# nihaomiao/WACV23_TSNet

Hardware: AMD Instinct MI355X
Metric: retargeted frames/sec at bs=4, 256x256, n_source=3; max-abs delta vs ref (higher is better)
Workload: dtype f32 (convolutions: fp16 x 2 split of the scaled fp32 operands, 3 exact MFMA products, two-level fp32 accumulate; fp32-class accuracy); 1 GPU; TSNet(label_nc=2,n_blocks=0,n_downsampling=3,n_source=3) forward, fp32, B=4 per GPU, 256x256 (BASELINE.json configs[1]); global_batch=4, parallelism=replicas x1 (batch-sharded, weights broadcast once)

## Files before the change

include/tsnet_abi.h:

```cpp
#ifndef TSNET_ABI_H
#define TSNET_ABI_H

#include <stddef.h>
#include <stdint.h>

#ifdef __cplusplus
extern "C" {
#endif

#define TSNET_ABI_VERSION 5
#define TSNET_MAX_SOURCES 8

enum {
    TSNET_OK = 0,
    TSNET_ERR_ARG = -1,
    TSNET_ERR_WEIGHT = -2,
    TSNET_ERR_HIP = -3,
    TSNET_ERR_NOMEM = -4
};

typedef struct tsnet_engine* tsnet_handle;

typedef struct tsnet_cfg {
    int label_nc;
    int n_blocks;
    int n_downsampling;
    int n_source;
    int ngf;
    int enc_blocks;
    int addcoords;
    int pose_composite;
    float pose_mean[3];
    int height, width;
    int max_batch;
    int operand_mode;
} tsnet_cfg;

int tsnet_abi_version(void);
int tsnet_create(const tsnet_cfg* cfg, tsnet_handle* out);
int tsnet_load_weights(tsnet_handle h, const char* name, const float* data, const int64_t* shape, int rank);
int tsnet_finalize(tsnet_handle h, void* stream);
void tsnet_destroy(tsnet_handle h);
const char* tsnet_last_error(tsnet_handle h);

int tsnet_num_params(tsnet_handle h);
int tsnet_param_info(tsnet_handle h, int index, const char** name, int64_t shape_out[4], int* rank);

int tsnet_packed_weights(tsnet_handle h, void** dev_ptr, size_t* bytes);

int tsnet_forward(tsnet_handle h,
                  const float* const* src_img, const float* const* src_lbl, const float* const* src_bbox,
                  const float* tar_lbl, const float* tar_bbox,
                  float* out_rgb, float* out_flow, int B, void* stream);

int tsnet_set_source_divisors(tsnet_handle h, const float* div, int n);

int tsnet_set_sources(tsnet_handle h, const float* const* src_img, const float* const* src_lbl,
                      const float* const* src_bbox, int B, void* stream);
int tsnet_forward_target(tsnet_handle h, const float* tar_lbl, const float* tar_bbox,
                         float* out_rgb, float* out_flow, int B, void* stream);

int tsnet_train_extras(tsnet_handle h, const float* const* src_img, const float* tar_img, int B,
                       float* warp_src_img, float* losses, void* stream);

int tsnet_stage_ptr(tsnet_handle h, const char* name, const float** dev_ptr, size_t* count);

double tsnet_forward_macs(tsnet_handle h, int B);

#define TSNET_TIMING_CLASSES 9
enum { TSNET_T_CONV = 0, TSNET_T_STATS = 1, TSNET_T_ELEMWISE = 2, TSNET_T_FLOW = 3, TSNET_T_WARP = 4,
       TSNET_T_PACK = 5, TSNET_T_UPSAMPLE = 6, TSNET_T_OTHER = 7,
       TSNET_T_CONV_RES = 8  };
int tsnet_timing_enable(tsnet_handle h, int on);
int tsnet_timing_read(tsnet_handle h, double ms_out[TSNET_TIMING_CLASSES], int64_t launches_out[TSNET_TIMING_CLASSES], int reset);

int tsnet_op_conv2d(const float* x, int N, int H, int W, int Cin,
                    const float* w_oihw, const float* bias, int Cout, int ksize, int stride, int pad, int pad_mode,
                    const float* in_alpha, const float* in_beta, int in_relu, float bound, int nprod, int kernel, int tile,
                    float* y, void* stream);
int tsnet_op_conv2d_cat(const float* x, const float* x2, int N, int H, int W, int C1, int C2, int x2_nmod,
                        const float* w_oihw, const float* bias, int Cout, int ksize, int stride, int pad, int pad_mode,
                        float bound, int nprod, float* y, void* stream);
int tsnet_op_head(const float* x, int N, int H, int W, int C, const float* in_alpha, const float* in_beta,
                  const float* w_oihw, const float* bias, int composite, const float* bg, float* y, void* stream);
int tsnet_op_instnorm_stats(const float* x, int N, int HW, int C, float* alpha, float* beta, void* stream);
int tsnet_op_norm_act(const float* x, const float* alpha, const float* beta, int relu, const float* resid,
                      int N, int HW, int C, float* y, void* stream);
int tsnet_op_upsample2x(const float* x, const float* alpha, const float* beta, int relu,
                        int N, int H, int W, int C, float* y, void* stream);
int tsnet_op_flow(const float* tar_fea, const float* src_fea, const float* tar_bbox, const float* src_bbox,
                  int B, int h, int w, int C, int H, int W, float* flow, void* stream);
int tsnet_op_flow_k(const float* tar_fea, const float* src_fea, const float* tar_bbox, const float* src_bbox,
                    int B, int K, int h, int w, int C, int H, int W, float* flow, int variant, int repeat, float* ms_out, void* stream);
int tsnet_flow_plan(int B, int h, int w, int C);
int tsnet_op_warp(const float* src_fea, const float* flow, int B, int h, int w, int C, float* out, void* stream);
int tsnet_op_warp_k(const float* src_fea, const float* flow, int B, int K, int h, int w, int C, float* out, int repeat, float* ms_out, void* stream);
const char* tsnet_op_last_error(void);

int tsnet_frame_stats(const float* x, int B, int C, int HW, float div, float* mean, float* std_unbiased, void* stream);
int tsnet_demo_postprocess(const float* rec, int B, int H, int W, const float* gen_mean, const float* gen_std,
                           const float* ref_mean, const float* ref_std, const float* img_mean_over_255,
                           unsigned char* out_rgb, void* stream);

int tsnet_fit_face_curves(const double* keypoints, int F, double* curves);
int tsnet_raster_face(const double* keypoints, const double* curves, int F, int h, int w, int bw, unsigned char* edges, unsigned char* bbox, void* stream);
int tsnet_vl2ch(const float* labels, int B, int HW, int num_classes, float* out, void* stream);

int tsnet_resize_label(const unsigned char* in, int F, int h, int w, int OH, int OW, const double* wts_rows, int lw_rows,
                       const double* wts_cols, int lw_cols, float* out, void* stream);
int tsnet_fit_pose_curves(const double* pts, int F, int flags, double* curves);
int tsnet_raster_pose(const double* pts, const double* curves, int F, int h, int w, int win_x0, int win_y0, int win_x1, int win_y1, int flags,
                      unsigned char* labels, void* stream);
int tsnet_label_bbox(const unsigned char* labels, int F, int h, int w, unsigned char* bbox, void* stream);
int tsnet_resize_pad(const unsigned char* in, int F, int h, int w, const int* ytab, const int* xtab, int oh, int ow,
                     int pad_top, int pad_left, int OH, int OW, int binarise, float* out, void* stream);

int tsnet_bench_conv(int N, int H, int W, int Cin, int Cout, int ksize, int stride, int pad, int pad_mode, int norm,
                     int variant, int iters, float* ms_out, void* stream);

void tsnet_debug_counters(int64_t out[4], int reset);

void tsnet_linspace(int n, float* out);
void tsnet_coord_table(int H, int W, float* out);

int tsnet_bicubic_taps(int n_in, int n_out);
int tsnet_bicubic_table(int n_in, int n_out, int* first, int* count, int* coef);
int tsnet_prepare_frames(const unsigned char* frames, int F, int h, int w, int x0, int y0, int x1, int y1,
                         const int* xfirst, const int* xcount, const int* xcoef, int xtaps,
                         const int* yfirst, const int* ycount, const int* ycoef, int ytaps,
                         int oh, int ow, int pad_top, int pad_left, int OH, int OW, const float* mean_bgr, float* out, void* stream);

#ifdef __cplusplus
}
#endif
#endif
```

wacv23_tsnet_amd/_lib.py:

```python
from __future__ import annotations

import ctypes as C
import os

import torch

_HERE = os.path.dirname(os.path.abspath(__file__))
LIB_PATH = os.path.join(_HERE, "lib", "libtsnet_hip.so")
MAX_SOURCES = 8
TIMING_CLASSES = 9
TIMING_NAMES = ("conv", "stats", "elementwise", "flow", "warp", "pack", "upsample", "other", "conv_res")

ABI_SYMBOLS = (
    "tsnet_abi_version", "tsnet_create", "tsnet_load_weights", "tsnet_finalize", "tsnet_destroy",
    "tsnet_last_error", "tsnet_num_params", "tsnet_param_info", "tsnet_packed_weights",
    "tsnet_forward", "tsnet_set_source_divisors", "tsnet_set_sources", "tsnet_forward_target", "tsnet_train_extras", "tsnet_stage_ptr",
    "tsnet_forward_macs", "tsnet_timing_enable", "tsnet_timing_read",
    "tsnet_op_conv2d", "tsnet_op_conv2d_cat", "tsnet_op_head", "tsnet_op_instnorm_stats", "tsnet_op_norm_act", "tsnet_op_upsample2x",
    "tsnet_op_flow", "tsnet_op_flow_k", "tsnet_flow_plan", "tsnet_op_warp", "tsnet_op_warp_k", "tsnet_op_last_error", "tsnet_frame_stats", "tsnet_demo_postprocess", "tsnet_fit_face_curves", "tsnet_raster_face", "tsnet_vl2ch", "tsnet_fit_pose_curves", "tsnet_raster_pose", "tsnet_label_bbox", "tsnet_resize_pad", "tsnet_resize_label", "tsnet_bench_conv", "tsnet_debug_counters", "tsnet_linspace", "tsnet_coord_table",
    "tsnet_bicubic_taps", "tsnet_bicubic_table", "tsnet_prepare_frames",
)


class TsnetCfg(C.Structure):
    _fields_ = [
        ("label_nc", C.c_int), ("n_blocks", C.c_int), ("n_downsampling", C.c_int), ("n_source", C.c_int),
        ("ngf", C.c_int), ("enc_blocks", C.c_int), ("addcoords", C.c_int), ("pose_composite", C.c_int),
        ("pose_mean", C.c_float * 3), ("height", C.c_int), ("width", C.c_int), ("max_batch", C.c_int), ("operand_mode", C.c_int),
    ]


_fp = C.POINTER(C.c_float)
_vp = C.c_void_p


def bind(lib: C.CDLL) -> C.CDLL:
    lib.tsnet_abi_version.restype = C.c_int
    lib.tsnet_create.argtypes = [C.POINTER(TsnetCfg), C.POINTER(_vp)]
    lib.tsnet_load_weights.argtypes = [_vp, C.c_char_p, _vp, C.POINTER(C.c_int64), C.c_int]
    lib.tsnet_finalize.argtypes = [_vp, _vp]
    lib.tsnet_destroy.argtypes = [_vp]
    lib.tsnet_destroy.restype = None
    lib.tsnet_last_error.argtypes = [_vp]
    lib.tsnet_last_error.restype = C.c_char_p
    lib.tsnet_num_params.argtypes = [_vp]
    lib.tsnet_param_info.argtypes = [_vp, C.c_int, C.POINTER(C.c_char_p), C.POINTER(C.c_int64), C.POINTER(C.c_int)]
    lib.tsnet_packed_weights.argtypes = [_vp, C.POINTER(_vp), C.POINTER(C.c_size_t)]
    pp = C.POINTER(_vp)
    lib.tsnet_forward.argtypes = [_vp, pp, pp, pp, _vp, _vp, _vp, _vp, C.c_int, _vp]
    lib.tsnet_set_source_divisors.argtypes = [_vp, _fp, C.c_int]
    lib.tsnet_set_sources.argtypes = [_vp, pp, pp, pp, C.c_int, _vp]
    lib.tsnet_forward_target.argtypes = [_vp, _vp, _vp, _vp, _vp, C.c_int, _vp]
    lib.tsnet_train_extras.argtypes = [_vp, pp, _vp, C.c_int, _vp, _vp, _vp]
    lib.tsnet_stage_ptr.argtypes = [_vp, C.c_char_p, C.POINTER(_vp), C.POINTER(C.c_size_t)]
    lib.tsnet_forward_macs.argtypes = [_vp, C.c_int]
    lib.tsnet_forward_macs.restype = C.c_double
    lib.tsnet_timing_enable.argtypes = [_vp, C.c_int]
    lib.tsnet_timing_read.argtypes = [_vp, C.POINTER(C.c_double), C.POINTER(C.c_int64), C.c_int]
    lib.tsnet_op_conv2d.argtypes = [_vp, C.c_int, C.c_int, C.c_int, C.c_int, _vp, _vp, C.c_int, C.c_int, C.c_int,
                                    C.c_int, C.c_int, _vp, _vp, C.c_int, C.c_float, C.c_int, C.c_int, C.c_int, _vp, _vp]
    lib.tsnet_op_conv2d_cat.argtypes = [_vp, _vp] + [C.c_int] * 6 + [_vp, _vp] + [C.c_int] * 5 + [C.c_float, C.c_int, _vp, _vp]
    lib.tsnet_op_head.argtypes = [_vp, C.c_int, C.c_int, C.c_int, C.c_int, _vp, _vp, _vp, _vp, C.c_int, _fp, _vp, _vp]
    lib.tsnet_op_instnorm_stats.argtypes = [_vp, C.c_int, C.c_int, C.c_int, _vp, _vp, _vp]
    lib.tsnet_op_norm_act.argtypes = [_vp, _vp, _vp, C.c_int, _vp, C.c_int, C.c_int, C.c_int, _vp, _vp]
    lib.tsnet_op_upsample2x.argtypes = [_vp, _vp, _vp, C.c_int, C.c_int, C.c_int, C.c_int, C.c_int, _vp, _vp]
    lib.tsnet_resize_label.argtypes = [_vp, C.c_int, C.c_int, C.c_int, C.c_int, C.c_int, _vp, C.c_int, _vp, C.c_int, _vp, _vp]
    lib.tsnet_op_flow.argtypes = [_vp, _vp, _vp, _vp, C.c_int, C.c_int, C.c_int, C.c_int, C.c_int, C.c_int, _vp, _vp]
    lib.tsnet_op_flow_k.argtypes = [_vp, _vp, _vp, _vp] + [C.c_int] * 7 + [_vp, C.c_int, C.c_int, _fp, _vp]
    lib.tsnet_flow_plan.argtypes = [C.c_int] * 4
    lib.tsnet_op_warp.argtypes = [_vp, _vp, C.c_int, C.c_int, C.c_int, C.c_int, _vp, _vp]
    if hasattr(lib, "tsnet_op_warp_k"):
        lib.tsnet_op_warp_k.argtypes = [_vp, _vp] + [C.c_int] * 5 + [_vp, C.c_int, _fp, _vp]
    lib.tsnet_op_last_error.restype = C.c_char_p
    lib.tsnet_frame_stats.argtypes = [_vp, C.c_int, C.c_int, C.c_int, C.c_float, _vp, _vp, _vp]
    lib.tsnet_demo_postprocess.argtypes = [_vp, C.c_int, C.c_int, C.c_int, _vp, _vp, _vp, _vp, _fp, _vp, _vp]
    lib.tsnet_fit_face_curves.argtypes = [_vp, C.c_int, _vp]
    lib.tsnet_fit_pose_curves.argtypes = [_vp, C.c_int, C.c_int, _vp]
    lib.tsnet_raster_face.argtypes = [_vp, _vp, C.c_int, C.c_int, C.c_int, C.c_int, _vp, _vp, _vp]
    lib.tsnet_vl2ch.argtypes = [_vp, C.c_int, C.c_int, C.c_int, _vp, _vp]
    lib.tsnet_raster_pose.argtypes = [_vp, _vp] + [C.c_int] * 8 + [_vp, _vp]
    lib.tsnet_label_bbox.argtypes = [_vp, C.c_int, C.c_int, C.c_int, _vp, _vp]
    lib.tsnet_resize_pad.argtypes = [_vp, C.c_int, C.c_int, C.c_int, _vp, _vp] + [C.c_int] * 7 + [_vp, _vp]
    lib.tsnet_bench_conv.argtypes = [C.c_int] * 12 + [_fp, _vp]
    lib.tsnet_debug_counters.argtypes = [C.POINTER(C.c_int64), C.c_int]
    lib.tsnet_debug_counters.restype = None
    lib.tsnet_linspace.argtypes = [C.c_int, _fp]
    lib.tsnet_linspace.restype = None
    lib.tsnet_coord_table.argtypes = [C.c_int, C.c_int, _fp]
    lib.tsnet_coord_table.restype = None
    if hasattr(lib, "tsnet_prepare_frames"):
        lib.tsnet_bicubic_taps.argtypes = [C.c_int, C.c_int]
        lib.tsnet_bicubic_table.argtypes = [C.c_int, C.c_int, _vp, _vp, _vp]
        lib.tsnet_prepare_frames.argtypes = [_vp] + [C.c_int] * 7 + [_vp, _vp, _vp, C.c_int, _vp, _vp, _vp, C.c_int] + [C.c_int] * 6 + [_fp, _vp, _vp]
    return lib


_cached = None


def load_tools() -> C.CDLL:
    from . import build as _b
    if not os.path.exists(_b.OUT_TOOLS):
        raise RuntimeError(f"{_b.OUT_TOOLS} is missing: run `python -m wacv23_tsnet_amd.build --tools`")
    return bind(C.CDLL(_b.OUT_TOOLS))


def load() -> C.CDLL:
    global _cached
    if _cached is not None:
        return _cached
    if not os.path.exists(LIB_PATH):
        raise RuntimeError(
            f"{LIB_PATH} is missing: the HIP extension is not built. Run "
            "`python -c 'import __graft_entry__ as g; g.build()'` (needs hipcc). "
            "There is no CPU fallback for the TS-Net forward path.")
    try:
        _cached = bind(C.CDLL(LIB_PATH))
    except OSError as e:
        raise RuntimeError(f"failed to load {LIB_PATH}: {e}") from e
    if _cached.tsnet_abi_version() != 5:
        raise RuntimeError("libtsnet_hip.so ABI version mismatch; rebuild")
    return _cached
```

wacv23_tsnet_amd/csrc/conv_common.hpp:

```cpp
#pragma once
#include <hip/hip_runtime.h>

namespace tsnet {

typedef float f32x16 __attribute__((ext_vector_type(16)));
struct alignas(16) F4 { float v[4]; };

constexpr unsigned kOOB = 0x80000000u;
constexpr int kPatchCols = 32;
constexpr int kPatchRows = 4;

#ifndef TSNET_BUF_LOAD16
typedef __amdgpu_buffer_rsrc_t tsnet_brsrc_t;
__device__ __forceinline__ tsnet_brsrc_t tsnet_make_brsrc(const void* p, unsigned bytes) {
    return __builtin_amdgcn_make_buffer_rsrc(const_cast<void*>(p), 0, (int)bytes, 0x00020000);
}
#define TSNET_BUF_LOAD16(rsrc, voff, soff) __builtin_bit_cast(F4, __builtin_amdgcn_raw_buffer_load_b128((rsrc), (int)(voff), (int)(soff), 0))
#endif
#ifndef TSNET_BUF_LOAD8
struct alignas(8) F2 { float v[2]; };
#define TSNET_BUF_LOAD8(rsrc, voff, soff) __builtin_bit_cast(F2, __builtin_amdgcn_raw_buffer_load_b64((rsrc), (int)(voff), (int)(soff), 0))
#endif
#ifndef TSNET_UNIFORM
#define TSNET_UNIFORM(x) __builtin_amdgcn_readfirstlane(x)
// ... 42 lines not shown
        "v_fma_mixhi_f16 %2, %5, %8, -%0 op_sel:[0,0,1] op_sel_hi:[0,0,1]\n\t"                                     \
        "v_fma_mixhi_f16 %3, %7, %8, -%1 op_sel:[0,0,1] op_sel_hi:[0,0,1]"                                          \
        : "=&v"(h0), "=&v"(h1), "=&v"(l0), "=&v"(l1)                                                               \
        : "v"(a0), "v"(b0), "v"(a1), "v"(b1), "v"(s))
#endif
#ifndef TSNET_FAST_EXP
#define TSNET_FAST_EXP(x) __expf(x)
#endif
#ifndef TSNET_SETPRIO
#define TSNET_SETPRIO(n) __builtin_amdgcn_s_setprio(n)
#endif
#ifndef TSNET_OPAQUE_V
#define TSNET_OPAQUE_V(x) asm volatile("" : "+v"(x))
#endif

__device__ __forceinline__ int xcd_item(int bid, int nitems) {
    const int q = nitems >> 3, r = nitems & 7, xcd = bid & 7, loc = bid >> 3;
    return (xcd < r ? xcd * (q + 1) : r * (q + 1) + (xcd - r) * q) + loc;
}

__device__ __forceinline__ void tile_of_block(int bid, int tiles_m, int tiles_n, int gn, int& tile_m, int& tile_n) {
    if (gn > 0) {
        const int xcd = bid & 7, loc = bid >> 3;
        const int tn = tiles_n / gn, tm = tiles_m / (8 / gn);
        tile_m = (xcd / gn) * tm + loc / tn;
        tile_n = (xcd % gn) * tn + loc % tn;
    } else {
        const int item = xcd_item(bid, tiles_m * tiles_n);
        tile_m = item / tiles_n;
        tile_n = item - tile_m * tiles_n;
    }
}

__device__ __forceinline__ unsigned short bf16_rne(float f) {
    const unsigned u = __builtin_bit_cast(unsigned, f);
    return (unsigned short)((u + 0x7FFFu + ((u >> 16) & 1u)) >> 16);
}
#ifndef TSNET_CVT_PK_BF16
__device__ __forceinline__ unsigned tsnet_cvt_pk_bf16(float a, float b) {
    unsigned r;
    asm("v_cvt_pk_bf16_f32 %0, %1, %2" : "=v"(r) : "v"(a), "v"(b));
    return r;
}
#define TSNET_CVT_PK_BF16(a, b) tsnet_cvt_pk_bf16((a), (b))
#endif

__device__ __forceinline__ void tsnet_publish_amax(unsigned* slot, float m) {
    __shared__ float wave_max[16];
#pragma unroll
    for (int off = 32; off > 0; off >>= 1) { const float o = __shfl_xor(m, off); m = o > m ? o : m; }
    __syncthreads();
    if ((threadIdx.x & 63) == 0) wave_max[threadIdx.x >> 6] = m;
    __syncthreads();
    if (threadIdx.x == 0) {
        const int nw = (int)((blockDim.x + 63) >> 6);
        for (int i = 1; i < nw; ++i) m = wave_max[i] > m ? wave_max[i] : m;
        __hip_atomic_fetch_max(slot, __builtin_bit_cast(unsigned, m), __ATOMIC_RELAXED, __HIP_MEMORY_SCOPE_AGENT);
    }
}

struct ConvArgs {
    const float* x;
    const float* x2;
    const float* in_alpha;
    const float* in_beta;
    int in_relu;
    float in_scale, in_unscale;
    const unsigned* in_amax; float in_bound_add;
    const unsigned short* w;
    const float* w_unscale;
    const float* bias;
    float* y;
    double* stat_part;
    const float* addend; int add_nmod;
    int N, H, W, Cin, cin_log2, Csplit, x2_nmod;
    int Ho, Wo, Cout, Npad;
    int stride, pad, reflect, taps, nchunks, M;
    int tiles_m, tiles_n, tpi;
    int xcd_gn;
    float* fin_alpha; float* fin_beta; int* fin_counter; int fin_S; float fin_eps;
    unsigned* amax_out;
    int x_bf16, y_bf16;
    int w1_chunk, w1_tab2;
};

__device__ __forceinline__ void bf16x8_widen(const F4& p, F4 (&o)[2]) {
#pragma unroll
    for (int e = 0; e < 4; ++e) {
        const unsigned w = __builtin_bit_cast(unsigned, p.v[e]);
        o[e >> 1].v[(e & 1) * 2] = __builtin_bit_cast(float, w << 16);
        o[e >> 1].v[(e & 1) * 2 + 1] = __builtin_bit_cast(float, w & 0xFFFF0000u);
    }
}

__device__ __forceinline__ void load_x_octet(const tsnet_brsrc_t& rs, bool xb16, unsigned voff, unsigned soff, F4 (&o)[2]) {
    if (xb16) {
        const F4 p = TSNET_BUF_LOAD16(rs, voff >> 1, soff >> 1);
        bf16x8_widen(p, o);
    } else {
        o[0] = TSNET_BUF_LOAD16(rs, voff, soff);
        o[1] = TSNET_BUF_LOAD16(rs, voff, soff + 16u);
    }
}

__device__ __forceinline__ void h2_device_scale(const unsigned* amax, float add, float& scale, float& unscale) {
    const float bound = __builtin_bit_cast(float, __hip_atomic_load(amax, __ATOMIC_RELAXED, __HIP_MEMORY_SCOPE_AGENT)) + add;
    int e = 0;
    (void)frexpf(bound, &e);
    int sa = 15 - e;
    sa = sa > 24 ? 24 : (sa < -24 ? -24 : sa);
    scale = ldexpf(1.0f, sa);
    unscale = ldexpf(1.0f, -sa);
}

__device__ __forceinline__ void split_h2(float v, unsigned& hi, unsigned& lo) {
    const _Float16 h = (_Float16)v;
    const _Float16 l = (_Float16)(v - (float)h);
    hi = (unsigned)__builtin_bit_cast(unsigned short, h);
    lo = (unsigned)__builtin_bit_cast(unsigned short, l);
}

__device__ __forceinline__ void split_h2_octet(const F4& x0, const F4& x1, F4& H, F4& L) {
    unsigned hw[4], lw[4];
    TSNET_SPLIT_2PAIRS(x0.v[0], x0.v[1], x0.v[2], x0.v[3], hw[0], lw[0], hw[1], lw[1]);
    TSNET_SPLIT_2PAIRS(x1.v[0], x1.v[1], x1.v[2], x1.v[3], hw[2], lw[2], hw[3], lw[3]);
#pragma unroll
    for (int e = 0; e < 4; ++e) { H.v[e] = __builtin_bit_cast(float, hw[e]); L.v[e] = __builtin_bit_cast(float, lw[e]); }
}

__device__ __forceinline__ void bf16_octet(const F4& x0, const F4& x1, F4& H) {
    unsigned hw[4];
#pragma unroll
    for (int e = 0; e < 2; ++e) {
        hw[e] = TSNET_CVT_PK_BF16(x0.v[2 * e], x0.v[2 * e + 1]);
        hw[2 + e] = TSNET_CVT_PK_BF16(x1.v[2 * e], x1.v[2 * e + 1]);
    }
#pragma unroll
    for (int e = 0; e < 4; ++e) H.v[e] = __builtin_bit_cast(float, hw[e]);
}

template <bool AFFINE, bool KEEP = true>
__device__ __forceinline__ void transform_octet(const F4 (&sx)[2], const float* ta, int Cin, float in_scale, float relu_floor, float keep, F4 (&t)[2]) {
    if (AFFINE) {
#pragma unroll
        for (int q = 0; q < 2; ++q) {
            const F4 al = *reinterpret_cast<const F4*>(ta + q * 4), be = *reinterpret_cast<const F4*>(ta + Cin + q * 4);
#pragma unroll
            for (int e = 0; e < 4; ++e) {
                const float v = __builtin_fmaxf(__builtin_fmaf(sx[q].v[e], al.v[e], be.v[e]), relu_floor);
                t[q].v[e] = KEEP ? v * keep : v;
            }
        }
    } else {
#pragma unroll
        for (int q = 0; q < 2; ++q)
#pragma unroll
            for (int e = 0; e < 4; ++e) t[q].v[e] = __builtin_fmaxf(sx[q].v[e] * in_scale, relu_floor);
    }
}

template <int BN, int WARPS_M, int WARPS_N, int MT, int NTL, int STAT_WAVE = 0, typename MOf>
__device__ __forceinline__ void conv_epilogue(const ConvArgs& a, f32x16 (&tot)[MT][NTL], unsigned char* smem_raw, int tid, int wave, int n0,
                                              size_t stat_tile, MOf m_of, const bool active = true) {
    constexpr int WM = MT * 32, WN = NTL * 32;
    const int lane = tid & 63, li = lane & 31, lh = lane >> 5;
    const int wm0 = (wave / WARPS_N) * WM, wn0 = (wave % WARPS_N) * WN;
    const int hw = a.Ho * a.Wo;
    double csum[NTL], csq[NTL];
#pragma unroll
    for (int j = 0; j < NTL; ++j) { csum[j] = 0.0; csq[j] = 0.0; }
    float vmax = 0.f;
#pragma unroll
    for (int i = 0; i < MT; ++i) {
#pragma unroll
        for (int j = 0; j < NTL; ++j) {
            const int n = n0 + wn0 + j * 32 + li;
            const bool nok = n < a.Cout;
            const float bv = (a.bias && nok) ? a.bias[n] : 0.f;
#pragma unroll
            for (int r = 0; r < 16; ++r) {
                const int m = m_of(wm0 + i * 32 + (r & 3) + 8 * (r >> 2) + 4 * lh);
                const bool mok = active && m >= 0;
                float v = tot[i][j][r] + bv;
                if (a.addend && nok && mok) {
                    const int img = m / hw;
                    v += a.addend[((size_t)(img % a.add_nmod) * hw + (m - img * hw)) * a.Cout + n];
                }
                tot[i][j][r] = v;
                if (a.stat_part && mok) { csum[j] += (double)v; csq[j] += (double)v * (double)v; }
                if (nok && mok) vmax = __builtin_fmaxf(vmax, __builtin_fabsf(v));
            }
        }
    }
    if (a.amax_out) tsnet_publish_amax(a.amax_out + stat_tile / (size_t)a.tpi, vmax);
    if (a.stat_part) {
        __syncthreads();
        double* red = reinterpret_cast<double*>(smem_raw);
#pragma unroll
        for (int j = 0; j < NTL; ++j) {
            const double s2 = csum[j] + __shfl_xor(csum[j], 32);
            const double q2 = csq[j] + __shfl_xor(csq[j], 32);
            if (lh == 0 && active) {
                double* o = red + ((size_t)(wave / WARPS_N) * BN + wn0 + j * 32 + li) * 2;
                o[0] = s2; o[1] = q2;
            }
        }
        __syncthreads();
        const int stid = tid - 64 * STAT_WAVE;
        if (stid >= 0 && stid < BN && n0 + stid < a.Cout) {
            double s = 0.0, q = 0.0;
#pragma unroll
            for (int wmi = 0; wmi < WARPS_M; ++wmi) { s += red[((size_t)wmi * BN + stid) * 2]; q += red[((size_t)wmi * BN + stid) * 2 + 1]; }
            double* o = a.stat_part + (stat_tile * a.Cout + n0 + stid) * 2;
            if (a.fin_counter) {
                __hip_atomic_store(o, s, __ATOMIC_RELAXED, __HIP_MEMORY_SCOPE_AGENT);
                __hip_atomic_store(o + 1, q, __ATOMIC_RELAXED, __HIP_MEMORY_SCOPE_AGENT);
            } else {
                o[0] = s; o[1] = q;
            }
        }
        if (a.fin_counter) {
            const int S = a.fin_S;
            const int img = (int)(stat_tile / (size_t)S);
            const int ntn = (a.Npad + 31) / 32;
            int* counter = a.fin_counter + (size_t)img * ntn + n0 / 32;
            const bool mine = stid >= 0 && stid < BN && n0 + stid < a.Cout;
            auto fold = [&](const double* p0, int cnt, size_t step, double& sm, double& sq) __attribute__((always_inline)) {
                double gs[4] = {0, 0, 0, 0}, gq[4] = {0, 0, 0, 0};
                for (int t0 = 0; t0 < cnt; t0 += 8) {
                    double v[8], w[8];
#pragma unroll
                    for (int u = 0; u < 8; ++u) {
                        const double* p = p0 + (size_t)(t0 + u < cnt ? t0 + u : cnt - 1) * step;
                        v[u] = __hip_atomic_load(p, __ATOMIC_RELAXED, __HIP_MEMORY_SCOPE_AGENT);
                        w[u] = __hip_atomic_load(p + 1, __ATOMIC_RELAXED, __HIP_MEMORY_SCOPE_AGENT);
                    }
#pragma unroll
                    for (int u = 0; u < 8; ++u) {
                        const bool in = t0 + u < cnt;
                        gs[u & 3] += in ? v[u] : 0.0;
                        gq[u & 3] += in ? w[u] : 0.0;
                    }
                }
                sm = gs[0]; sq = gq[0];
#pragma unroll
                for (int k = 1; k < 4; ++k) { sm += gs[k]; sq += gq[k]; }
            };
            auto write_ab = [&](double sm, double sq) __attribute__((always_inline)) {
                const double mean = sm / hw;
                double var = sq / hw - mean * mean;
                if (var < 0) var = 0;
                const float al = 1.0f / sqrtf((float)var + a.fin_eps);
                a.fin_alpha[(size_t)img * a.Cout + n0 + stid] = al;
                a.fin_beta[(size_t)img * a.Cout + n0 + stid] = -((float)mean) * al;
            };
            auto finalize = [&]() __attribute__((always_inline)) {
                if (mine) {
                    double sm, sq;
                    fold(a.stat_part + (((size_t)img * S) * a.Cout + n0 + stid) * 2, S, (size_t)a.Cout * 2, sm, sq);
                    write_ab(sm, sq);
                }
                if (stid == 0) __hip_atomic_store(counter, 0, __ATOMIC_RELAXED, __HIP_MEMORY_SCOPE_AGENT);
            };
            if (BN <= 64) {
                if (stid >= 0 && stid < 64) {
                    auto arrive = [&](int* c) __attribute__((always_inline)) {
                        TSNET_DRAIN_VMEM();
                        float arrived = 0.f;
                        if (lane == 0) arrived = (float)__hip_atomic_fetch_add(c, 1, __ATOMIC_RELAXED, __HIP_MEMORY_SCOPE_AGENT);
#pragma unroll
                        for (int off = 32; off > 0; off >>= 1) arrived += __shfl_xor(arrived, off);
                        return (int)arrived;
                    };
                    if (arrive(counter) == S - 1) finalize();
                }
            } else {
                int* flag = reinterpret_cast<int*>(smem_raw + 8192);
                auto arrive = [&](int* c) __attribute__((always_inline)) {
                    TSNET_DRAIN_VMEM();
                    __syncthreads();
                    if (stid == 0) *flag = __hip_atomic_fetch_add(c, 1, __ATOMIC_RELAXED, __HIP_MEMORY_SCOPE_AGENT);
                    __syncthreads();
                    return *flag;
                };
                if (arrive(counter) == S - 1) finalize();
            }
        }
    }
    unsigned short* const y16 = reinterpret_cast<unsigned short*>(a.y);
#pragma unroll
    for (int i = 0; i < MT; ++i) {
#pragma unroll
        for (int j = 0; j < NTL; ++j) {
            const int n = n0 + wn0 + j * 32 + li;
            if (n >= a.Cout) continue;
#pragma unroll
            for (int r = 0; r < 16; ++r) {
                const int m = m_of(wm0 + i * 32 + (r & 3) + 8 * (r >> 2) + 4 * lh);
                if (!(active && m >= 0)) continue;
                if (a.y_bf16) y16[(size_t)m * a.Cout + n] = bf16_rne(tot[i][j][r]);
                else a.y[(size_t)m * a.Cout + n] = tot[i][j][r];
            }
        }
    }
}

}
```

wacv23_tsnet_amd/csrc/conv_plan.hpp:

```cpp
#pragma once
#include <cstddef>
#include <stdexcept>
#include <string>

namespace tsnet {

constexpr int kPlanTileRows = 4, kPlanTileCols = 32;
constexpr size_t kFinCounterInts = 65536;
constexpr int kFinMaxTiles = 32;

enum class ConvFamily { H2R, G64, H2, H2S, H2S32, H2D, W1 };
enum class ConvKernel { Own = 0, General = 1, Patch = 2 };
enum class ConvSched { Plain = 0, Deep = 1, TwoGroups = 2 };

struct ConvShape {
    int ks = 1, stride = 1, pad = 0, reflect = 0;
    int cin = 0;
    int cout = 0, npad = 0, kpad = 0;
    int form = 0;
    int N = 0, H = 0, W = 0;
    int csplit = 0;
    bool transform = false;
    int nprod = 3;
    bool fin_counter = false;
    int ho() const { return (H + 2 * pad - ks) / stride + 1; }
    int wo() const { return (W + 2 * pad - ks) / stride + 1; }
};

struct ConvRequest {
    ConvKernel kernel = ConvKernel::Own;
    int rows = 0;
    int width = 0;
    bool alt = false;
    ConvSched sched = ConvSched::Plain;
    int chunk = 0;
    int chunk_cap = 3;
    int abl = 0, opt = 0;
    int xcd_gn = -1;
};

struct ConvPlan {
    ConvFamily family = ConvFamily::H2R;
    int rows = 0;
    int width = 0;
    bool side_by_side = false;
    ConvSched sched = ConvSched::Plain;
    int w1_chunk = 1, w1_tab2 = 0;
    int xcd_gn = 0;
    int tpi = 0, tiles_m = 0, tiles_n = 0;
    bool fin = false;
};

inline ConvRequest decode_tile_code(int kernel, int tile) {
    ConvRequest r;
    if (kernel == 3) {
        if (tile < 0 || tile > 3) throw std::invalid_argument("conv: the Winograd form takes 0 to 3 tiles per workgroup");
        r.chunk = tile;
        return r;
    }
    if (kernel < 0 || kernel > 2) throw std::invalid_argument("conv: kernel must be 0 (the layer's own), 1 (general), 2 (patch) or 3 (Winograd form)");
    r.kernel = static_cast<ConvKernel>(kernel);
    switch (tile) {
        case 0: break;
        case 32: case 64: case 128: r.width = tile; break;
        case 2128: r.rows = 2; r.width = 128; break;
        case 3064: case 3128: r.alt = true; r.width = tile - 3000; break;
        case 12128: r.rows = 2; r.width = 128; r.sched = ConvSched::Deep; break;
        case 20032: case 20064: r.rows = 4; r.width = tile - 20000; r.sched = ConvSched::TwoGroups; break;
        default: throw std::invalid_argument("conv: unknown tile code " + std::to_string(tile));
    }
    return r;
}

struct BenchVariant { ConvRequest req; int nprod = 3, form = 0; bool cold = false; };
inline BenchVariant decode_bench_variant(int variant) {
    const int v = variant < 0 ? 0 : variant;
    BenchVariant b;
    b.form = (v & 32768) ? 1 : 0;
    b.req = decode_tile_code(b.form ? 3 : ((v & 4096) ? 1 : ((v & 16384) ? 2 : 0)), v & 4095);
    b.nprod = (v & 8192) ? 1 : 3;
    b.cold = (v & (1 << 21)) != 0;
    b.req.abl = (v >> 16) & 31;
    b.req.opt = ((v >> 24) & 15) | ((v & (1 << 23)) ? 16 : 0) | ((v & (1 << 22)) ? 32 : 0);
    const int gx = (v >> 28) & 7;
    if (gx > 5) throw std::invalid_argument("bench_conv: XCD grid code 0 to 5");
    b.req.xcd_gn = gx == 0 ? -1 : (gx == 1 ? 0 : 1 << (gx - 2));
    return b;
}

struct HeadRequest { bool composite = false; int rows = 0; };
inline HeadRequest decode_head_code(int code) {
    if (code < 0 || (code & 0xFE)) throw std::invalid_argument("head: composite is bit 0, the tile rows bits 8 and up");
    HeadRequest r;
    r.composite = code & 1;
    r.rows = code >> 8;
    if (r.rows != 0 && r.rows != 8 && r.rows != 16 && r.rows != 32) throw std::invalid_argument("head: tile rows 8, 16 or 32");
    return r;
}

inline size_t w1_lds_bytes_host(int Cin, int tables) {
    return 3 * (size_t)(2 * (4 * 2 * 2 * (96 * 16 + 64) + 32)) + (size_t)tables * 2 * ((Cin + 31) / 32 * 32) * 4;
}
inline bool w1_eligible(int ks, int stride, int pad, int cin, int H, int W) {
    return ks == 3 && stride == 1 && pad == 1 && cin >= 16 && (cin & 15) == 0 && H >= 4 && W >= 32 && H % kPlanTileRows == 0 && W % kPlanTileCols == 0 &&
           w1_lds_bytes_host(cin, 1) + 256 <= 160 * 1024;
}

inline ConvFamily conv_class(const ConvShape& s, int rows, bool eligible_only) {
    const int Ho = s.ho(), Wo = s.wo();
    const bool bf16 = s.nprod == 1;
    const bool s1 = s.ks == 3 && s.stride == 1 && s.pad == 1 && s.cin >= 16 && (s.cin & 15) == 0 && s.H >= 2 && s.W >= 2;
    if (s.csplit || Ho <= 0 || Wo <= 0 || Wo % kPlanTileCols) return ConvFamily::H2R;
    const bool s2 = s.ks == 3 && s.stride == 2 && s.pad == 1 && !s.reflect && s.cin >= (eligible_only ? 16 : 128) && (s.cin & 15) == 0 && s.H == 2 * Ho && s.W == 2 * Wo;
    if (rows == 2 && Ho % 2 == 0) {
        if (s1) return ConvFamily::H2;
        if (s2) return ConvFamily::H2D;
    }
    if (Ho % kPlanTileRows) return ConvFamily::H2R;
    if (s1) return ConvFamily::H2;
    if (s.ks == 7 && s.stride == 1 && s.pad == 3 && s.reflect && s.cin == 8 && !s.transform && s.H >= 4 && s.W >= 4) return ConvFamily::H2S;
    if (s.ks == 7 && s.stride == 1 && s.pad == 3 && s.reflect && s.cin == 32 && !s.transform && s.H >= 4 && s.W >= 4) return ConvFamily::H2S32;
    if (s2 && (eligible_only || !bf16)) return ConvFamily::H2D;
    return ConvFamily::H2R;
}

inline bool wide_pays(const ConvShape& s, long tm, double gain, int cus) {
    const double c64 = (double)((tm * ((s.cout + 63) / 64) + cus - 1) / cus) * 64.0;
    const double c128 = (double)((tm * ((s.cout + 127) / 128) + cus - 1) / cus) * 128.0 / gain;
    return s.npad % 128 == 0 && s.cout > 64 && c128 < c64;
}

inline int xcd_grid(const ConvShape& s, int requested, int tiles_m, int tiles_n, const char* who) {
    int gn = requested < 0 ? (((double)s.kpad * s.npad * 4 > 16e6) ? 4 : 0) : requested;
    if (gn && ((gn != 1 && gn != 2 && gn != 4 && gn != 8) || tiles_n % gn || tiles_m % (8 / gn))) {
        if (requested >= 0) throw std::invalid_argument(std::string(who) + ": the XCD grid does not divide the tile matrix");
        gn = 0;
    }
    return gn;
}

inline void plan_w1_chunk(const ConvShape& s, const ConvRequest& r, int cus, ConvPlan& p) {
    const int n = p.tiles_m * p.tiles_n, npp = ((s.cin >> 4) + 1) / 2;
    const int rows = p.xcd_gn ? p.tiles_m / (8 / p.xcd_gn) : (p.tiles_m % 8 ? 0 : p.tiles_m / 8);
    const bool tab2 = !s.transform || w1_lds_bytes_host(s.cin, 2) + 256 <= 160 * 1024;
    auto fits = [&](int cc) { return cc == 1 || (s.nprod != 1 && npp >= 4 && rows > 0 && rows % cc == 0 && (tab2 || p.tpi % cc == 0)); };
    int cc = 1;
    if (r.chunk) {
        if (!fits(r.chunk)) throw std::invalid_argument("conv(w1): this chunk size does not fit the layer");
        cc = r.chunk;
    } else {
        for (int t : {3, 2}) if (fits(t) && n % (cus * t) == 0) { cc = t; break; }
        if (cc > r.chunk_cap) cc = 1;
    }
    p.w1_chunk = cc; p.w1_tab2 = (s.transform && tab2 && cc > 1) ? 1 : 0;
}

inline ConvPlan plan_conv(const ConvShape& s, const ConvRequest& r, int cus) {
    const bool bf16 = s.nprod == 1;
    const int Ho = s.ho(), hw = Ho * s.wo();
    ConvPlan p;
    if (s.form == 1) {
        if (s.csplit || !w1_eligible(s.ks, s.stride, s.pad, s.cin, s.H, s.W))
            throw std::invalid_argument("conv(w1): the layer is packed in the Winograd form, which needs a single source and whole 4 x 32 tiles");
        if (s.nprod == 4) throw std::invalid_argument("conv(w1): 1 or 3 products");
        p.family = ConvFamily::W1;
    } else if (r.kernel == ConvKernel::General) {
        p.family = ConvFamily::H2R;
    } else {
        p.family = conv_class(s, r.rows == 2 ? 2 : kPlanTileRows, r.kernel == ConvKernel::Patch);
        if (r.kernel == ConvKernel::Patch && p.family == ConvFamily::H2R) throw std::invalid_argument("conv: this layer / frame size has no patch kernel");
    }
    auto set_tiles = [&](int rows_per_tile_m, int bn) {
        p.tpi = (hw + rows_per_tile_m - 1) / rows_per_tile_m;
        p.tiles_m = s.N * p.tpi; p.tiles_n = (s.cout + bn - 1) / bn;
        p.fin = s.fin_counter && p.tpi <= kFinMaxTiles && (size_t)s.N * ((s.npad + 31) / 32) <= kFinCounterInts;
    };
    switch (p.family) {
    case ConvFamily::W1:
        if (r.opt) throw std::invalid_argument("conv(w1): no experiment variants");
        p.rows = kPlanTileRows; p.width = 64;
        set_tiles(kPlanTileRows * kPlanTileCols, 64);
        p.xcd_gn = xcd_grid(s, r.xcd_gn, p.tiles_m, p.tiles_n, "conv(w1)");
        plan_w1_chunk(s, r, cus, p);
        break;
    case ConvFamily::H2: {
        int pr = r.rows ? r.rows : kPlanTileRows, bn = r.width;
        if (bn == 0) {
            const long tm = (long)s.N * (hw / 128);
            bn = wide_pays(s, tm, s.transform ? 1.03 : 1.10, cus) ? 128 : 64;
            if (bf16 && s.npad % 128 == 0 && s.cout > 64 && tm * ((s.cout + 127) / 128) >= cus) bn = 128;
        }
        p.side_by_side = r.alt || (!r.width && bf16 && pr == 4 && bn == 128);
        if (p.side_by_side && (!bf16 || bn != 128)) throw std::invalid_argument("conv(h2): the 1 x 4 wave grid is the bf16 4 x 128 tile's");
        if ((pr != 2 && pr != 4) || Ho % pr) throw std::invalid_argument("conv(h2): the output height must be a multiple of the tile's rows (2 or 4)");
        if (s.npad % bn) throw std::invalid_argument("conv(h2): the tile width must divide the padded output width");
        p.rows = pr; p.width = bn; p.sched = r.sched;
        set_tiles(pr * kPlanTileCols, bn);
        p.xcd_gn = xcd_grid(s, r.xcd_gn, p.tiles_m, p.tiles_n, "conv(h2)");
        break;
    }
    case ConvFamily::H2S:
    case ConvFamily::H2S32:
        p.rows = kPlanTileRows; p.width = 64;
        set_tiles(128, 64);
        break;
    case ConvFamily::H2D: {
        if (r.sched == ConvSched::TwoGroups) throw std::invalid_argument("conv(h2d): the stride-2 tiles have no two-K-group form (1xxxx: the deep schedule of the 2 x 128 tile)");
        if (r.alt) throw std::invalid_argument("conv(h2d): tiles have two or four output rows");
        int pr = r.rows ? r.rows : kPlanTileRows, bn = r.width;
        if (bn == 0) {
            bn = 64;
            if (s.npad % 128 == 0 && s.cout > 64 && Ho % 2 == 0) { pr = 2; bn = 128; }
        }
        if (s.npad % bn) throw std::invalid_argument("conv(h2d): the tile width must divide the padded output width");
        if (Ho % pr) throw std::invalid_argument("conv(h2d): the output height must be a multiple of the tile's rows");
        p.rows = pr; p.width = bn;
        set_tiles(pr * kPlanTileCols, bn);
        const bool deep = r.width ? r.sched == ConvSched::Deep : (pr == 2 && bn == 128 && s.nprod == 3 && (long)p.tiles_m * p.tiles_n <= 2L * cus);
        p.sched = deep ? ConvSched::Deep : ConvSched::Plain;
        break;
    }
    case ConvFamily::H2R:
    case ConvFamily::G64: {
        if (r.abl || r.opt) throw std::invalid_argument("conv: experiment variants exist for the 3x3 / stride-1 patch kernel only");
        if (r.rows || r.sched != ConvSched::Plain || r.width == 32) throw std::invalid_argument("conv(h2r): the tile width must be 64 or 128");
        const bool g64_ok = (s.ks == 1 || s.ks == 3) && (s.cin & 63) == 0 && (!s.csplit || (s.csplit & 63) == 0) && s.npad % 128 == 0 && s.cout > 64 &&
                            (s.nprod == 1 || s.nprod == 3);
        if (r.alt || (!r.width && g64_ok)) {
            if (!g64_ok) throw std::invalid_argument("conv(g64): needs a 1 x 1 / 3 x 3 layer, input channels in multiples of 64 and more than 64 output channels");
            p.family = ConvFamily::G64;
            p.rows = r.width ? r.width : 64; p.width = 128;
            set_tiles(p.rows, 128);
        } else {
            const long tm = (long)s.N * ((hw + 127) / 128);
            const int bn = r.width ? r.width : ((s.ks == 3 && s.cin >= 16 && wide_pays(s, tm, 1.15, cus)) ? 128 : 64);
            if (s.npad % bn) throw std::invalid_argument("conv(h2r): the tile width must divide the padded output width");
            p.family = ConvFamily::H2R;
            p.rows = 128; p.width = bn;
            set_tiles(128, bn);
        }
        break;
    }
    }
    return p;
}

inline int head_rows(int B, int tiles_x, int hh, int cus) {
    return (long)B * tiles_x * ((hh + 31) / 32) >= cus ? 32 : ((long)B * tiles_x * ((hh + 15) / 16) >= cus ? 16 : 8);
}

}
```

wacv23_tsnet_amd/csrc/conv_w1.hpp:

```cpp
#pragma once
#include <type_traits>

#include "conv_common.hpp"

namespace tsnet {

constexpr int kW1Prod = 6;
constexpr int kW1Waves = 8 + kW1Prod;
constexpr int kW1Reg = 96 * 16 + 64;
constexpr int kW1Stage(int npl) { return 2 * (4 * npl * 2 * kW1Reg + 32); }
constexpr int w1_lds_bytes(int Cin, int npl = 2, int tables = 1) {
    const int v = 3 * kW1Stage(npl), ex = 4 * 64 * 64 * 4 + 2048;
    return (v > ex ? v : ex) + tables * 2 * ((Cin + 31) / 32 * 32) * 4;
}

#ifdef TSNET_TOOLS
constexpr int kW1ProfSlots = 16, kW1ProfTiles = 1024;
static __device__ unsigned long long g_w1_prof[kW1ProfTiles * kW1Waves * kW1ProfSlots];
#define TSNET_W1_STAMP(slot)                                                                                                   \
    do {                                                                                                                        \
        if ((OPT & 512) && (threadIdx.x & 63) == 0 && blockIdx.x < kW1ProfTiles)                                                \
            g_w1_prof[((size_t)blockIdx.x * kW1Waves + (threadIdx.x >> 6)) * kW1ProfSlots + (slot)] = __builtin_amdgcn_s_memrealtime(); \
    } while (0)
#define TSNET_W1_LOOP_BARRIER(acc_)                                                        \
// ... 28 lines not shown
#pragma unroll
        for (int q = 0; q < 4; ++q)
#pragma unroll
            for (int e = 0; e < 4; ++e) {
                const float v = __builtin_fmaxf(__builtin_fmaf(b[q].v[e], al.v[e], be.v[e]), relu_floor);
                d[q].v[e] = (ZPAD_KEEP && pad[q]) ? 0.f : v;
            }
    } else {
#pragma unroll
        for (int q = 0; q < 4; ++q)
#pragma unroll
            for (int e = 0; e < 4; ++e) d[q].v[e] = LATE_SCALE ? b[q].v[e] : (NO_RELU ? b[q].v[e] * scale : __builtin_fmaxf(b[q].v[e] * scale, relu_floor));
    }
#pragma unroll
    for (int p = 0; p < 4; ++p) {
        float v[4];
#pragma unroll
        for (int e = 0; e < 4; ++e) {
            const float d0 = d[0].v[e], d1 = d[1].v[e], d2 = d[2].v[e], d3 = d[3].v[e];
            v[e] = p == 0 ? d0 - d2 : (p == 1 ? d1 + d2 : (p == 2 ? d2 - d1 : d1 - d3));
        }
        if (NPROD == 1) {
            U2 h;
            h.x = TSNET_CVT_PK_BF16(v[0], v[1]);
            h.y = TSNET_CVT_PK_BF16(v[2], v[3]);
            *reinterpret_cast<U2*>(dst + p * POSB) = h;
        } else {
            U2 h, l;
            if (LATE_SCALE) TSNET_SPLIT_2PAIRS_SCALED(v[0], v[1], v[2], v[3], scale, h.x, l.x, h.y, l.y);
            else TSNET_SPLIT_2PAIRS(v[0], v[1], v[2], v[3], h.x, l.x, h.y, l.y);
            *reinterpret_cast<U2*>(dst + p * POSB) = h;
            *reinterpret_cast<U2*>(dst + p * POSB + PLANE_V) = l;
        }
    }
}

template <int NPROD, int NPL>
__device__ __forceinline__ void w1_step_products(f32x16 (&acc)[2], const F4 (&a0)[NPL], const F4 (&a1)[NPL], const F4 (&bw)[NPL], const bool fresh) {
    auto product = [&](int pa, int pb, bool fr) __attribute__((always_inline)) {
#pragma unroll
        for (int i = 0; i < 2; ++i) {
            f32x16 c = acc[i];
            if (fr) {
#pragma unroll
                for (int r = 0; r < 16; ++r) c[r] = 0.f;
            }
            const F4& A = i ? a1[pa] : a0[pa];
            if (NPROD == 1) acc[i] = TSNET_MFMA_BF16(A, bw[pb], c);
            else acc[i] = TSNET_MFMA_F16(A, bw[pb], c);
        }
    };
    if (NPROD == 1) {
        product(0, 0, fresh);
    } else {
        product(NPL - 1, 0, fresh);
        product(0, NPL - 1, false);
        product(0, 0, false);
    }
}

__device__ __forceinline__ void w1_output_transform(const float* m, const int pstride, const int lh, f32x16& out) {
#pragma unroll
    for (int r2 = 0; r2 < 8; ++r2) {
        const int x = ((2 * r2) & 3) + 8 * ((2 * r2) >> 2) + 4 * lh;
        const float* q = m + (size_t)(x >> 1) * 64;
        const float m0 = q[0], m1 = q[pstride], m2 = q[2 * pstride], m3 = q[3 * pstride];
        out[2 * r2] = (m0 + m1) + m2;
        out[2 * r2 + 1] = (m1 - m2) - m3;
    }
}

struct W1Tile {
    int img, oy0, ox0, n0, tin;
    float in_scale, in_unscale;
};

template <int NPROD, bool AFFINE, int OPT = 0>
__device__ __forceinline__ void w1_chunk(const ConvArgs& a, unsigned char* smem_raw, const int wg, const int nrun) {
    static_assert(NPROD == 1 || NPROD == 3, "one (bf16 operands) or three products");
    constexpr int NPL = NPROD == 1 ? 1 : 2;
    constexpr bool ONE_LEVEL = NPROD == 1;
    constexpr bool ZPAD_KEEP = (OPT & 1) != 0;
    constexpr bool NO_RELU = (OPT & 2) != 0;
    constexpr int BD = 3;
    constexpr int REG = kW1Reg;
    constexpr int PLANE_V = 2 * REG, POSB = NPL * PLANE_V, SLABB = 4 * POSB + 32, STAGE = 2 * SLABB;
    static_assert(STAGE == kW1Stage(NPL), "stage size");
    static_assert(NPL == 1 || STAGE >= 4 * 32 * 64 * 4 + 4096, "a stage holds half the output exchange and the epilogue's reductions (one plane: chunks of one tile only)");
    constexpr int OFF_END = 3 * STAGE, OFF_EX_END = 4 * 64 * 64 * 4 + 2048;
    constexpr int OFF_TAB = OFF_END > OFF_EX_END ? OFF_END : OFF_EX_END;

    const int tid = threadIdx.x;
    const int lane = tid & 63;
    const int wave = TSNET_UNIFORM(tid >> 6);
    TSNET_W1_STAMP(0);
    const int pos = wave >> 1, nt = wave & 1;
    const int wn0 = nt * 32;
    const int li = lane & 31, lh = lane >> 5;

    const int tcols = a.Wo / kPatchCols, tper = (a.Ho / kPatchRows) * tcols;
    const int ncc = a.Cin >> 4;
    const int npp = (ncc + 1) >> 1;
    const int cp32 = (a.Cin + 31) & ~31;
    auto tile_at = [&](int j) __attribute__((always_inline)) {
        W1Tile t;
        int tile_m, tile_n;
        if (nrun == 1) {
            tile_of_block(wg, a.tiles_m, a.tiles_n, a.xcd_gn, tile_m, tile_n);
        } else {
            const int xcd = wg & 7, loc = wg >> 3;
            const int gn = a.xcd_gn > 0 ? a.xcd_gn : 1;
            const int tn = a.tiles_n / gn, tm = a.xcd_gn > 0 ? a.tiles_m / (8 / gn) : a.tiles_m / 8;
            tile_m = (a.xcd_gn > 0 ? xcd / gn : xcd) * tm + (loc / tn) * nrun + j;
            tile_n = (a.xcd_gn > 0 ? xcd % gn : 0) * tn + loc % tn;
        }
        t.img = tile_m / tper; t.tin = tile_m - t.img * tper;
        t.oy0 = (t.tin / tcols) * kPatchRows; t.ox0 = (t.tin % tcols) * kPatchCols;
        t.n0 = tile_n * 64;
        t.in_scale = a.in_scale; t.in_unscale = a.in_unscale;
        if (NPROD != 1 && a.in_amax) {
            h2_device_scale(a.in_amax + t.img, a.in_bound_add, t.in_scale, t.in_unscale);
            t.in_scale *= 0.5f; t.in_unscale *= 2.0f;
        }
        return t;
    };
    W1Tile T = tile_at(0);

    const size_t planew = (size_t)((a.nchunks + 1) / 2 * 2) * a.Npad * 16;
    const tsnet_brsrc_t rsx = tsnet_make_brsrc(a.x, (unsigned)((size_t)a.N * a.H * a.W * a.Cin * 4));
    tsnet_brsrc_t rsw[NPL];
#pragma unroll
    for (int p = 0; p < NPL; ++p) rsw[p] = tsnet_make_brsrc(a.w + p * planew, (unsigned)(planew * 2));

    float* const tab0 = reinterpret_cast<float*>(smem_raw + OFF_TAB);
    auto tab_fill = [&](float* tb, const W1Tile& t, int first, int stride) __attribute__((always_inline)) {
        for (int c = first; c < cp32; c += stride) {
            const bool ok = c < a.Cin;
            tb[c] = ok ? a.in_alpha[(size_t)t.img * a.Cin + c] * t.in_scale : 0.f;
            tb[cp32 + c] = ok ? a.in_beta[(size_t)t.img * a.Cin + c] * t.in_scale : 0.f;
        }
    };
    struct TabRegs { float a0, b0, a1, b1; };
    auto tab_request = [&](const W1Tile& t) __attribute__((always_inline)) {
        const int c0 = tid, c1 = tid + 64 * kW1Waves;
        TabRegs r;
        r.a0 = c0 < a.Cin ? a.in_alpha[(size_t)t.img * a.Cin + c0] : 0.f; r.b0 = c0 < a.Cin ? a.in_beta[(size_t)t.img * a.Cin + c0] : 0.f;
        r.a1 = c1 < a.Cin ? a.in_alpha[(size_t)t.img * a.Cin + c1] : 0.f; r.b1 = c1 < a.Cin ? a.in_beta[(size_t)t.img * a.Cin + c1] : 0.f;
        return r;
    };
    auto tab_store = [&](float* tb, const W1Tile& t, const TabRegs& r) __attribute__((always_inline)) {
        const int c0 = tid, c1 = tid + 64 * kW1Waves;
        if (c0 < cp32) { tb[c0] = r.a0 * t.in_scale; tb[cp32 + c0] = r.b0 * t.in_scale; }
        if (c1 < cp32) { tb[c1] = r.a1 * t.in_scale; tb[cp32 + c1] = r.b1 * t.in_scale; }
    };
    f32x16 tot[2];
#pragma unroll
    for (int i = 0; i < 2; ++i)
#pragma unroll
        for (int r = 0; r < 16; ++r) tot[i][r] = 0.f;
    unsigned long long bar_wait = 0;
    const bool consumer = wave < 8;
    const int mq = consumer ? wave >> 1 : 0;

    auto epilogue = [&](const W1Tile& t, const int st_free, const bool two_pass) __attribute__((always_inline)) {
        const float unscale = a.w_unscale ? t.in_unscale * a.w_unscale[0] : t.in_unscale;
        __syncthreads();
        int tid_e = tid;
        TSNET_OPAQUE_V(tid_e);
        const int li = tid_e & 31, lh = (tid_e >> 5) & 1;
        f32x16 out[1][1];
        unsigned char* const ebase = two_pass ? smem_raw + st_free : smem_raw;
        float* const ex = reinterpret_cast<float*>(ebase);
        auto transform = [&](const float* m, const int pstride) __attribute__((always_inline)) { w1_output_transform(m, pstride, lh, out[0][0]); };
        if (!two_pass) {
            if (consumer) {
#pragma unroll
                for (int i = 0; i < 2; ++i)
#pragma unroll
                    for (int r = 0; r < 16; ++r) {
                        const int pair = i * 32 + (r & 3) + 8 * (r >> 2) + 4 * lh;
                        ex[(pos * 64 + pair) * 64 + wn0 + li] = tot[i][r] * unscale;
                    }
            }
            __syncthreads();
            if (consumer) transform(ex + (size_t)(mq * 16) * 64 + wn0 + li, 64 * 64);
            __syncthreads();
        } else {
#pragma unroll
            for (int h = 0; h < 2; ++h) {
                if (consumer) {
#pragma unroll
                    for (int r = 0; r < 16; ++r) {
                        const int pair = (r & 3) + 8 * (r >> 2) + 4 * lh;
                        ex[(pos * 32 + pair) * 64 + wn0 + li] = tot[h][r] * unscale;
                    }
                }
                __syncthreads();
                if (consumer && (mq >> 1) == h) transform(ex + (size_t)((mq & 1) * 16) * 64 + wn0 + li, 32 * 64);
                __syncthreads();
            }
        }
        const int m_img = t.img * a.Ho * a.Wo;
        conv_epilogue<64, 4, 2, 1, 1, 8>(a, out, ebase, tid_e, consumer ? wave : nt, t.n0, (size_t)t.img * tper + t.tin,
                                      [&](int l) { return m_img + (t.oy0 + (l >> 5)) * a.Wo + t.ox0 + (l & 31); }, consumer);
    };

    if (wave >= 8) {
        constexpr int NIT = 12 / kW1Prod;
        static_assert(NIT * kW1Prod == 12 && (NIT & 1) == 0, "an even number of items per producer (the fetch buffers alternate)");
        const int pw = wave - 8, quad = lane & 7;
        const int psl = quad >> 2, poct = (quad >> 1) & 1, psub = quad & 1;
        struct Offs { unsigned vP[NIT][4]; };
        int ldst[NIT];
#pragma unroll
        for (int it = 0; it < NIT; ++it) {
            const int item = NIT * pw + it;
            ldst[it] = psl * SLABB + poct * REG + ((item >> 1) * 16 + (item & 1) * 8 + (lane >> 3)) * 16 + psub * 8;
        }
        auto offsets = [&](const W1Tile& t, const bool real, Offs& o) __attribute__((always_inline)) {
#pragma unroll
            for (int it = 0; it < NIT; ++it) {
                const int item = NIT * pw + it, prow = item >> 1, ppair = (item & 1) * 8 + (lane >> 3);
                int iy = t.oy0 - 1 + prow;
                bool rok = real;
                if (a.reflect) {
                    iy = iy < 0 ? -iy : iy;
                    iy = iy >= a.H ? 2 * (a.H - 1) - iy : iy;
                } else {
                    rok = rok && iy >= 0 && iy < a.H;
                }
#pragma unroll
                for (int q = 0; q < 4; ++q) {
                    int ix = t.ox0 - 1 + 2 * ppair + q;
                    bool ok = rok;
                    if (a.reflect) {
                        ix = ix < 0 ? -ix : ix;
                        ix = ix >= a.W ? 2 * (a.W - 1) - ix : ix;
                    } else {
                        ok = ok && ix >= 0 && ix < a.W;
                    }
                    o.vP[it][q] = ok ? (unsigned)(((t.img * a.H * a.W + iy * a.W + ix) * a.Cin + quad * 4) * 4) : kOOB;
                }
            }
        };
        Offs cur, nxt;
        W1Tile Tn = T;
        bool has_next = nrun > 1;
        offsets(T, true, cur);
        offsets(T, false, nxt);
        unsigned curT[NIT][4];
        auto tail_of = [&](const Offs& o) __attribute__((always_inline)) {
            const bool cok = (npp - 1) * 32 + quad * 4 < a.Cin;
#pragma unroll
            for (int it = 0; it < NIT; ++it)
#pragma unroll
                for (int q = 0; q < 4; ++q) curT[it][q] = cok ? o.vP[it][q] : kOOB;
        };
        tail_of(cur);
        const float* tab_cur = tab0;
        const float* tab_nxt = tab0;
        const float relu_floor = a.in_relu ? 0.f : -__builtin_inff();
        F4 sx[2][4];
        using SrcCur = std::integral_constant<int, 0>;
        using SrcTail = std::integral_constant<int, 1>;
        using SrcNxt = std::integral_constant<int, 2>;
        auto v_fetch = [&](auto SRC, int pe, int it, F4 (&b)[4]) __attribute__((always_inline)) {
            constexpr int src = decltype(SRC)::value;
#pragma unroll
            for (int q = 0; q < 4; ++q)
                b[q] = TSNET_BUF_LOAD16(rsx, src == 2 ? nxt.vP[it][q] : (src == 1 ? curT[it][q] : cur.vP[it][q]), (unsigned)(pe * 128));
        };
        auto v_put = [&](auto SRC, int pe, int it, int st, const F4 (&b)[4]) __attribute__((always_inline)) {
            constexpr bool nx = decltype(SRC)::value == 2;
            const int c0 = pe * 32 + quad * 4;
            bool pad[4];
#pragma unroll
            for (int q = 0; q < 4; ++q) pad[q] = ZPAD_KEEP && (nx ? nxt.vP[it][q] : cur.vP[it][q]) == kOOB;
            w1_put_item<NPROD, AFFINE, ZPAD_KEEP, NO_RELU, POSB, PLANE_V>(b, pad, (nx ? tab_nxt : tab_cur) + c0, cp32, nx ? Tn.in_scale : T.in_scale, relu_floor,
                                                                        smem_raw + st + ldst[it]);
        };
        auto fetch_any = [&](int pq, int it, F4 (&b)[4]) __attribute__((always_inline)) {
            if (pq >= npp) v_fetch(SrcNxt{}, pq - npp, it, b);
            else if (pq == npp - 1) v_fetch(SrcTail{}, pq, it, b);
            else v_fetch(SrcCur{}, pq, it, b);
        };
        auto put_any = [&](int pq, int it, int st, const F4 (&b)[4]) __attribute__((always_inline)) {
            if (pq >= npp) v_put(SrcNxt{}, pq - npp, it, st, b);
            else v_put(SrcCur{}, pq, it, st, b);
        };
        static_assert(NIT == 2, "the prologue and the period loop are written for two items per producer");
        {
            F4 sp[2][4];
            TabRegs tr{};
            if (AFFINE) tr = tab_request(T);
            fetch_any(0, 0, sx[0]); fetch_any(0, 1, sx[1]); fetch_any(1, 0, sp[0]); fetch_any(1, 1, sp[1]);
            if (AFFINE) {
                tab_store(tab0, T, tr);
                __syncthreads();
            }
            if (has_next) { Tn = tile_at(1); offsets(Tn, true, nxt); }
            put_any(0, 0, 0, sx[0]);
            fetch_any(2, 0, sx[0]);
            put_any(0, 1, 0, sx[1]);
            if (1 < npp || has_next) { put_any(1, 0, STAGE, sp[0]); put_any(1, 1, STAGE, sp[1]); }
        }
        TSNET_W1_STAMP(1);
        __syncthreads();
        TSNET_W1_STAMP(2);
        int st_wr = 2 * STAGE;
        auto iter = [&](auto L1, auto L2, auto PUT, int pe1, int pe2, int pep, bool put_ok) __attribute__((always_inline)) {
            if (!(OPT & 128)) TSNET_W1_LOOP_BARRIER(bar_wait);
            if (!(OPT & 16)) {
                v_fetch(L1, pe1, 1, sx[1]);
                if (put_ok) v_put(PUT, pep, 0, st_wr, sx[0]);
                v_fetch(L2, pe2, 0, sx[0]);
                if (put_ok) v_put(PUT, pep, 1, st_wr, sx[1]);
            }
            st_wr = st_wr == 2 * STAGE ? 0 : st_wr + STAGE;
        };
        for (int j = 0; j < nrun; ++j) {
// ... 150 lines not shown
```

wacv23_tsnet_amd/csrc/conv_w1_launch.cpp:

```cpp
#include <stdexcept>

#include "conv_w1.hpp"
#include "conv_w1_one.hpp"
#include "kernels.hpp"

namespace tsnet {

namespace {

template <int NPROD, bool AFFINE, int OPT>
void go_w1_one(const ConvArgs& a, hipStream_t s) {
    const size_t lds = (size_t)w1_lds_bytes(a.Cin, NPROD == 1 ? 1 : 2, 1);
    ensure_dynamic_lds(reinterpret_cast<const void*>(conv_w1_one_kernel<NPROD, AFFINE, OPT>), lds);
    hipLaunchKernelGGL((conv_w1_one_kernel<NPROD, AFFINE, OPT>), dim3(a.tiles_m * a.tiles_n), dim3(64 * kW1Waves), lds, s, a);
}

template <int NPROD, bool AFFINE, int OPT>
void go_w1_k(const ConvArgs& a, size_t lds, hipStream_t s) {
    ensure_dynamic_lds(reinterpret_cast<const void*>(conv_w1_kernel<NPROD, AFFINE, OPT>), lds);
    const int c = a.w1_chunk > 1 ? a.w1_chunk : 1;
    if (c > 1 && (a.tiles_m % ((a.xcd_gn > 0 ? 8 / a.xcd_gn : 8) * c) || (a.xcd_gn > 0 && a.tiles_n % a.xcd_gn)))
        throw std::invalid_argument("conv(w1): the chunk size must divide every XCD's rows of the tile matrix");
    hipLaunchKernelGGL((conv_w1_kernel<NPROD, AFFINE, OPT>), dim3(a.tiles_m * a.tiles_n / c), dim3(64 * kW1Waves), lds, s, a);
}

template <int NPROD>
void go_w1(const ConvArgs& a, hipStream_t s) {
    const size_t lds = (size_t)w1_lds_bytes(a.Cin, NPROD == 1 ? 1 : 2, a.w1_tab2 ? 2 : 1);
    if (NPROD == 1 && a.w1_chunk > 1) throw std::invalid_argument("conv(w1): chunks of several tiles need the two-plane stages");
    if (a.w1_chunk <= 1) {
        if (!a.in_alpha && !a.in_relu) go_w1_one<NPROD, false, 2>(a, s);
        else if (!a.in_alpha) go_w1_one<NPROD, false, 0>(a, s);
        else if (a.reflect) go_w1_one<NPROD, true, 0>(a, s);
        else go_w1_one<NPROD, true, 1>(a, s);
        return;
    }
    if constexpr (NPROD == 3) {
        if (!a.in_alpha && !a.in_relu) go_w1_k<NPROD, false, 2>(a, lds, s);
        else if (!a.in_alpha) go_w1_k<NPROD, false, 0>(a, lds, s);
        else if (a.reflect) go_w1_k<NPROD, true, 0>(a, lds, s);
        else go_w1_k<NPROD, true, 1>(a, lds, s);
    }
}

}

void launch_conv_w1(const ConvArgs& a, int nprod, int abl, hipStream_t s) {
    if (a.Cin > 2 * 64 * kW1Waves) throw std::invalid_argument("conv(w1): the prologue's table request covers two channels per thread");
    if (abl) {
#ifdef TSNET_TOOLS
        const size_t lds = (size_t)w1_lds_bytes(a.Cin, 2, a.w1_tab2 ? 2 : 1);
        if (abl == 31 && nprod == 3 && a.in_alpha) { go_w1_k<3, true, 512>(a, lds, s); return; }
        if (nprod != 3 || a.in_alpha) throw std::invalid_argument("conv(w1): ablations are built for three products on a raw input");
#define TSNET_W1_ABL(A_) if (abl == A_) { go_w1_k<3, false, ((A_) << 4) | 2>(a, lds, s); return; }
        if (abl == 30) { go_w1_k<3, false, 512 | 2>(a, lds, s); return; }
        TSNET_W1_ABL(1) TSNET_W1_ABL(2) TSNET_W1_ABL(4) TSNET_W1_ABL(3) TSNET_W1_ABL(7) TSNET_W1_ABL(8) TSNET_W1_ABL(15) TSNET_W1_ABL(16) TSNET_W1_ABL(17)
#undef TSNET_W1_ABL
        throw std::invalid_argument("conv(w1): this ablation is not instantiated");
#else
        throw std::invalid_argument("conv(w1): ablation variants are only built into the tools library");
#endif
    }
    if (nprod == 3) go_w1<3>(a, s);
    else if (nprod == 1) go_w1<1>(a, s);
    else throw std::invalid_argument("conv(w1): 1 (bf16 operands) or 3 products");
}

}

#ifdef TSNET_TOOLS
extern "C" int tsnet_w1_prof_read(unsigned long long* out, int ntiles) {
    using namespace tsnet;
    if (!out || ntiles < 1 || ntiles > kW1ProfTiles) return -1;
    if (hipDeviceSynchronize() != hipSuccess) return -2;
    return hipMemcpyFromSymbol(out, HIP_SYMBOL(g_w1_prof), (size_t)ntiles * kW1Waves * kW1ProfSlots * 8, 0, hipMemcpyDeviceToHost) == hipSuccess ? 0 : -3;
}
#endif
```

wacv23_tsnet_amd/csrc/conv_w1_one.hpp:

```cpp
#pragma once
#include "conv_w1.hpp"

namespace tsnet {

template <int NPROD, bool AFFINE, int OPT = 0>
__device__ __forceinline__ void w1_tile_one(const ConvArgs& a, unsigned char* smem_raw, const int tile_m, const int n0) {
    static_assert(NPROD == 1 || NPROD == 3, "one (bf16 operands) or three products");
    constexpr int NPL = NPROD == 1 ? 1 : 2;
    constexpr bool ONE_LEVEL = NPROD == 1;
    constexpr bool ZPAD_KEEP = (OPT & 1) != 0;
    constexpr bool NO_RELU = (OPT & 2) != 0;
    constexpr int BD = 3;
    constexpr int REG = kW1Reg;
    constexpr int PLANE_V = 2 * REG, POSB = NPL * PLANE_V, SLABB = 4 * POSB + 32, STAGE = 2 * SLABB;
    static_assert(STAGE == kW1Stage(NPL), "stage size");
    constexpr int OFF_END = 3 * STAGE, OFF_EX_END = 4 * 64 * 64 * 4 + 2048;
    constexpr int OFF_TAB = OFF_END > OFF_EX_END ? OFF_END : OFF_EX_END;

    const int tid = threadIdx.x;
    const int lane = tid & 63;
    const int wave = TSNET_UNIFORM(tid >> 6);
    const int pos = wave >> 1, nt = wave & 1;
    const int wn0 = nt * 32;
    const int li = lane & 31, lh = lane >> 5;

    const int tcols = a.Wo / kPatchCols, tper = (a.Ho / kPatchRows) * tcols;
    const int img = tile_m / tper, tin = tile_m - img * tper;
    const int oy0 = (tin / tcols) * kPatchRows, ox0 = (tin % tcols) * kPatchCols;
    const int ncc = a.Cin >> 4;
    const int npp = (ncc + 1) >> 1;
    float in_scale = a.in_scale, in_unscale = a.in_unscale;
    if (NPROD != 1 && a.in_amax) {
        h2_device_scale(a.in_amax + img, a.in_bound_add, in_scale, in_unscale);
        in_scale *= 0.5f; in_unscale *= 2.0f;
    }

    const size_t planew = (size_t)((a.nchunks + 1) / 2 * 2) * a.Npad * 16;
    const tsnet_brsrc_t rsx = tsnet_make_brsrc(a.x, (unsigned)((size_t)a.N * a.H * a.W * a.Cin * 4));
    tsnet_brsrc_t rsw[NPL];
#pragma unroll
    for (int p = 0; p < NPL; ++p) rsw[p] = tsnet_make_brsrc(a.w + p * planew, (unsigned)(planew * 2));

    const int cp32 = (a.Cin + 31) & ~31;
    float* tab = reinterpret_cast<float*>(smem_raw + OFF_TAB);
    if (AFFINE) {
        for (int c = tid; c < cp32; c += 64 * kW1Waves) {
            const bool ok = c < a.Cin;
            tab[c] = ok ? a.in_alpha[(size_t)img * a.Cin + c] * in_scale : 0.f;
            tab[cp32 + c] = ok ? a.in_beta[(size_t)img * a.Cin + c] * in_scale : 0.f;
        }
        __syncthreads();
    }
    f32x16 tot[2];
#pragma unroll
    for (int i = 0; i < 2; ++i)
#pragma unroll
        for (int r = 0; r < 16; ++r) tot[i][r] = 0.f;

    if (wave >= 8) {
        constexpr int NIT = 12 / kW1Prod;
        static_assert(NIT * kW1Prod == 12 && (NIT & 1) == 0, "an even number of items per producer (the fetch buffers alternate)");
        const int pw = wave - 8, quad = lane & 7;
        const int psl = quad >> 2, poct = (quad >> 1) & 1, psub = quad & 1;
        unsigned vP[NIT][4];
        int ldst[NIT];
#pragma unroll
        for (int it = 0; it < NIT; ++it) {
            const int item = NIT * pw + it, prow = item >> 1, ppair = (item & 1) * 8 + (lane >> 3);
            int iy = oy0 - 1 + prow;
            bool rok = true;
            if (a.reflect) {
                iy = iy < 0 ? -iy : iy;
                iy = iy >= a.H ? 2 * (a.H - 1) - iy : iy;
            } else {
                rok = iy >= 0 && iy < a.H;
            }
#pragma unroll
            for (int q = 0; q < 4; ++q) {
                int ix = ox0 - 1 + 2 * ppair + q;
                bool ok = rok;
                if (a.reflect) {
                    ix = ix < 0 ? -ix : ix;
                    ix = ix >= a.W ? 2 * (a.W - 1) - ix : ix;
                } else {
                    ok = ok && ix >= 0 && ix < a.W;
                }
                vP[it][q] = ok ? (unsigned)(((img * a.H * a.W + iy * a.W + ix) * a.Cin + quad * 4) * 4) : kOOB;
            }
            ldst[it] = psl * SLABB + poct * REG + (prow * 16 + ppair) * 16 + psub * 8;
        }
        const float relu_floor = a.in_relu ? 0.f : -__builtin_inff();
        F4 sx[2][4];
        auto v_load = [&](int pq, int it, int buf) __attribute__((always_inline)) {
            const bool cok = pq * 32 + quad * 4 < a.Cin;
#pragma unroll
            for (int q = 0; q < 4; ++q) sx[buf][q] = TSNET_BUF_LOAD16(rsx, cok ? vP[it][q] : kOOB, (unsigned)(pq * 128));
        };
        auto v_item = [&](int pq, int it, int st, int buf) __attribute__((always_inline)) {
            const int c0 = pq * 32 + quad * 4;
            bool pad[4];
#pragma unroll
            for (int q = 0; q < 4; ++q) pad[q] = ZPAD_KEEP && vP[it][q] == kOOB;
            w1_put_item<NPROD, AFFINE, ZPAD_KEEP, NO_RELU, POSB, PLANE_V>(sx[buf], pad, tab + (c0 < cp32 ? c0 : 0) , cp32, in_scale,
                                                                        relu_floor, smem_raw + st + ldst[it]);
        };
        v_load(0, 0, 0);
#pragma unroll
        for (int u = 0; u < 2 * NIT; ++u) {
            v_load((u + 1) / NIT, (u + 1) % NIT, (u + 1) & 1);
            v_item(u / NIT, u % NIT, (u / NIT) * STAGE, u & 1);
        }
        __syncthreads();
        int st_wr = 2 * STAGE;
        for (int pp = 0; pp < npp; ++pp) {
            if (!(OPT & 128)) __syncthreads();
            if (!(OPT & 16)) {
#pragma unroll
                for (int it = 0; it < NIT; ++it) {
                    v_load(it == NIT - 1 ? pp + 3 : pp + 2, it == NIT - 1 ? 0 : it + 1, (it & 1) ^ 1);
                    v_item(pp + 2, it, st_wr, it & 1);
                }
            }
            st_wr = st_wr == 2 * STAGE ? 0 : st_wr + STAGE;
        }
    } else {
        TSNET_SETPRIO(2);
        const unsigned vB = (unsigned)((wn0 + li) * 32 + (lh ^ ((li >> 3) & 1)) * 16);
        F4 af[2][5][NPL], bf[BD][NPL];
        auto load_b = [&](int set, int cc, int ky) __attribute__((always_inline)) {
            const int kc = (ky * 4 + pos) * ncc + cc;
            const unsigned vo = cc < ncc ? vB : kOOB;
#pragma unroll
            for (int p = 0; p < NPL; ++p) bf[set][p] = TSNET_BUF_LOAD16(rsw[p], vo, (unsigned)((kc * a.Npad + n0) * 32));
        };
        const unsigned char* abase = smem_raw + pos * POSB + lh * REG + li * 16;
        auto load_f = [&](int sl, int f, int st) __attribute__((always_inline)) {
#pragma unroll
            for (int p = 0; p < NPL; ++p) af[sl][f][p] = *reinterpret_cast<const F4*>(abase + st + sl * SLABB + p * PLANE_V + f * 256);
        };
        f32x16 acc[2];
#pragma unroll
        for (int i = 0; i < 2; ++i)
#pragma unroll
            for (int r = 0; r < 16; ++r) acc[i][r] = 0.f;
        auto period = [&](int pp, int st_cur, int st_nxt) __attribute__((always_inline)) {
            if (!(OPT & 128)) __syncthreads();
#pragma unroll
            for (int t = 0; t < 6; ++t) {
                const int sl = t / 3, ky = t % 3;
                if (!(OPT & 32)) load_b((t + BD - 1) % BD, 2 * pp + (t + BD - 1) / 3, (t + BD - 1) % 3);
                if (!(OPT & 64)) {
                    if (ky == 0) { load_f(sl, 1, st_cur); load_f(sl, 3, st_cur); }
                    if (ky == 1) load_f(sl, 4, st_cur);
                    if (t == 2) { load_f(1, 0, st_cur); load_f(1, 2, st_cur); }
                    if (t == 5) { load_f(0, 0, st_nxt); load_f(0, 2, st_nxt); }
                }
                const bool fresh = !ONE_LEVEL && t == 0;
                w1_step_products<NPROD, NPL>(acc, af[sl][ky], af[sl][ky + 2], bf[t % BD], fresh);
                __builtin_amdgcn_sched_barrier(0);
            }
            if (!ONE_LEVEL) {
#pragma unroll
                for (int i = 0; i < 2; ++i)
#pragma unroll
                    for (int r = 0; r < 16; ++r) tot[i][r] += acc[i][r];
            }
        };
#pragma unroll
        for (int i = 0; i < BD - 1; ++i) load_b(i, i / 3, i % 3);
        __syncthreads();
        load_f(0, 0, 0); load_f(0, 2, 0);
        if (OPT & 32) load_b(BD - 1, 1, 2);
        if (OPT & 64) {
#pragma unroll
            for (int sl = 0; sl < 2; ++sl)
#pragma unroll
                for (int f = 0; f < 5; ++f) load_f(sl, f, 0);
        }
        int st0 = 0, st1 = STAGE;
        for (int pp = 0; pp < npp; ++pp) {
            period(pp, st0, st1);
            st0 = st1; st1 = st1 == 2 * STAGE ? 0 : st1 + STAGE;
        }
        if (ONE_LEVEL) { tot[0] = acc[0]; tot[1] = acc[1]; }
        TSNET_SETPRIO(0);
    }

    const float unscale = a.w_unscale ? in_unscale * a.w_unscale[0] : in_unscale;
    __syncthreads();
    float* ex = reinterpret_cast<float*>(smem_raw);
    const bool consumer = wave < 8;
    if (consumer) {
#pragma unroll
        for (int i = 0; i < 2; ++i)
#pragma unroll
            for (int r = 0; r < 16; ++r) {
                const int pair = i * 32 + (r & 3) + 8 * (r >> 2) + 4 * lh;
                ex[(pos * 64 + pair) * 64 + wn0 + li] = tot[i][r] * unscale;
            }
    }
    __syncthreads();
    const int mq = consumer ? wave >> 1 : 0;
    f32x16 out[1][1];
    w1_output_transform(ex + (size_t)(mq * 16) * 64 + wn0 + li, 64 * 64, lh, out[0][0]);
    __syncthreads();
    const int m_img = img * a.Ho * a.Wo;
    conv_epilogue<64, 4, 2, 1, 1>(a, out, smem_raw, tid, consumer ? wave : nt, n0, (size_t)img * tper + tin,
                                  [&](int l) { return m_img + (oy0 + (l >> 5)) * a.Wo + ox0 + (l & 31); }, consumer);
}

template <int NPROD, bool AFFINE, int OPT = 0>
__global__ __launch_bounds__(64 * kW1Waves, 1)
void conv_w1_one_kernel(ConvArgs a) {
    HIP_DYNAMIC_SHARED(__attribute__((aligned(16))) unsigned char, smem_raw)
    int tile_m, tile_n;
    tile_of_block(blockIdx.x, a.tiles_m, a.tiles_n, a.xcd_gn, tile_m, tile_n);
    w1_tile_one<NPROD, AFFINE, OPT>(a, smem_raw, tile_m, tile_n * 64);
}

}
```

wacv23_tsnet_amd/csrc/engine.cpp:

```cpp
#include <hip/hip_runtime.h>

#include <algorithm>
#include <cmath>
#include <cstdio>
#include <cstdlib>
#include <cstring>
#include <map>
#include <memory>
#include <stdexcept>
#include <string>
#include <vector>

#include "../../include/tsnet_abi.h"
#include "conv_plan.hpp"
#include "kernels.hpp"
#include "lmfit.hpp"
#include "flow_warp.hpp"
#include "frames.hpp"
#include "head_conv.hpp"
#include "norm_elementwise.hpp"
#include "pack_weights.hpp"
#include "postproc.hpp"
#include "raster.hpp"
#include "train_extras.hpp"

using namespace tsnet;

namespace {

thread_local std::string g_op_error;
int64_t g_launch_counters[4] = {0, 0, 0, 0};
std::string g_create_error;

#define HIP_TRY(expr)                                                                               \
    do {                                                                                            \
        hipError_t e__ = (expr);                                                                    \
        if (e__ != hipSuccess) {                                                                    \
            char buf__[512];                                                                        \
            snprintf(buf__, sizeof buf__, "%s failed: %s (%s:%d)", #expr, hipGetErrorString(e__), __FILE__, __LINE__); \
            throw std::runtime_error(buf__);                                                        \
        }                                                                                           \
    } while (0)

#ifdef TSNET_TOOLS
int g_tools_knob[8] = {3, 0, 0, 0, 0, 0, 0, 0};
#endif
struct ArgError : std::runtime_error { using std::runtime_error::runtime_error; };
struct WeightError : std::runtime_error { using std::runtime_error::runtime_error; };

inline int round_up(int x, int m) { return (x + m - 1) / m * m; }
static_assert(kPlanTileRows == kPatchRows && kPlanTileCols == kPatchCols, "conv_plan.hpp's patch tile is conv_common.hpp's");
inline int current_device_cus() {
    int dev = 0, v = 0;
    if (hipGetDevice(&dev) != hipSuccess || hipDeviceGetAttribute(&v, hipDeviceAttributeMultiprocessorCount, dev) != hipSuccess || v < 8) v = 256;
    return v;
}
inline int ilog2(int x) { int l = 0; while ((1 << l) < x) ++l; return l; }
inline int next_pow2(int x) { int p = 4; while (p < x) p <<= 1; return p; }

struct Timing {
    bool on = false;
    struct Rec { int cls; hipEvent_t a, b; };
    std::vector<Rec> recs;
    double ms[TSNET_TIMING_CLASSES] = {0};
    int64_t launches[TSNET_TIMING_CLASSES] = {0};
    void begin(int cls, hipStream_t s) {
        if (!on) return;
        Rec r{cls, nullptr, nullptr};
        HIP_TRY(hipEventCreate(&r.a));
        HIP_TRY(hipEventCreate(&r.b));
        HIP_TRY(hipEventRecord(r.a, s));
        recs.push_back(r);
    }
    void end(hipStream_t s) {
        if (!on) return;
        HIP_TRY(hipEventRecord(recs.back().b, s));
    }
    void collect() {
        for (auto& r : recs) {
            HIP_TRY(hipEventSynchronize(r.b));
            float t = 0.f;
            HIP_TRY(hipEventElapsedTime(&t, r.a, r.b));
            ms[r.cls] += t;
            launches[r.cls] += 1;
            (void)hipEventDestroy(r.a);
            (void)hipEventDestroy(r.b);
        }
        recs.clear();
    }
};

struct Ctx {
    hipStream_t stream;
    int cus;
    Timing* timing = nullptr;
    int lane = 0;
    Ctx(hipStream_t s, int cus_, Timing* t = nullptr, int lane_ = 0) : stream(s), cus(cus_), timing(t), lane(lane_) {}
};

struct EventPair {
    hipEvent_t a = nullptr, b = nullptr;
    EventPair() {
        HIP_TRY(hipEventCreate(&a));
        try { HIP_TRY(hipEventCreate(&b)); } catch (...) { (void)hipEventDestroy(a); throw; }
    }
    ~EventPair() { (void)hipEventDestroy(a); (void)hipEventDestroy(b); }
    EventPair(const EventPair&) = delete;
    EventPair& operator=(const EventPair&) = delete;
    float ms() {
        HIP_TRY(hipEventSynchronize(b));
        float t = 0.f;
        HIP_TRY(hipEventElapsedTime(&t, a, b));
        return t;
    }
};

struct SideJoin {
    hipStream_t side, main; hipEvent_t ev; bool done = false;
    ~SideJoin() { if (!done && side && hipEventRecord(ev, side) == hipSuccess) (void)hipStreamWaitEvent(main, ev, 0); }
};

struct TimeScope {
    Ctx& c;
    TimeScope(Ctx& c_, int cls) : c(c_) { if (c.timing) c.timing->begin(cls, c.stream); }
    ~TimeScope() { if (c.timing) { try { c.timing->end(c.stream); } catch (...) {} } }
};

inline void check_launch(const char* what) {
    hipError_t e = hipGetLastError();
    if (e != hipSuccess) throw std::runtime_error(std::string(what) + " launch failed: " + hipGetErrorString(e));
}

inline int ew_grid(size_t total, int block = 256) {
    size_t g = (total + block - 1) / block;
    if (g > 256 * 8) g = 256 * 8;
    if (g < 1) g = 1;
    return (int)g;
}

void launch_finalize_impl(const double* part, float* alpha, float* beta, int N, int C, int S, int HW, hipStream_t s);
inline void launch_finalize(const double* part, float* alpha, float* beta, int N, int C, int S, int HW, hipStream_t s) { launch_finalize_impl(part, alpha, beta, N, C, S, HW, s); }

inline int pack_grid(int hw) {
    int g = (hw + 255) / 256;
    if (g > 128) g = 128;
    return g < 1 ? 1 : g;
}
struct ConvLayer {
    std::string name;
    std::string wparam, bparam;
    int cin_real = 0, cin_pad = 0, cout = 0, ks = 1, stride = 1, pad = 0, reflect = 0;
    int cin_total = 0, cin_off = 0;
    int kpad = 0, npad = 0;
    int form = 0;
    size_t w_off = 0, b_off = 0;
    const unsigned short* wq = nullptr;
    const float* w_unscale = nullptr;
    const float* bias = nullptr;
};

struct DevBufs {
    std::vector<void*> p;
    template <typename T> T* alloc(size_t bytes) { void* q = nullptr; HIP_TRY(hipMalloc(&q, bytes)); p.push_back(q); return static_cast<T*>(q); }
    ~DevBufs() { for (void* q : p) (void)hipFree(q); }
    DevBufs() = default;
    DevBufs(const DevBufs&) = delete;
    DevBufs& operator=(const DevBufs&) = delete;
};

inline size_t stat_part_doubles(size_t N, size_t tpi, size_t Cout) { return N * tpi * Cout * 2; }
constexpr int KPAD_ALIGN = 32;

inline int conv_kpad(int ks, int cin_pad) { return round_up(ks * ks * cin_pad, KPAD_ALIGN); }
inline int conv_kpad_w1(int cin_pad) { return round_up(12 * cin_pad, KPAD_ALIGN); }
inline int conv_npad(int cout) { return cout >= 128 ? round_up(cout, 128) : round_up(cout, 64); }
inline int conv_cin_pad(int cin) { return cin <= 8 ? 8 : round_up(cin, 16); }

struct ConvCall {
    const float* x = nullptr; const float* x2 = nullptr;
    int csplit = 0, x2_nmod = 1;
    const float* alpha = nullptr; const float* beta = nullptr; int relu = 0;
    float bound = 0.f;
    const unsigned* in_amax = nullptr; float bound_add = 0.f;
    int N = 0, H = 0, W = 0;
    float* y = nullptr;
    const float* addend = nullptr; int add_nmod = 1;
    double* stat_part = nullptr; mutable int stat_S = 0;
    float* fin_alpha = nullptr; float* fin_beta = nullptr; int* fin_counter = nullptr;
    unsigned* amax_out = nullptr;
    int x_bf16 = 0, y_bf16 = 0;
    int nprod = 3;
    int tclass = TSNET_T_CONV;
};

inline int h2_scale_log2(float bound) {
    if (!(bound > 0.f) || !std::isfinite(bound)) throw ArgError("conv: the operand bound must be positive and finite");
    int e = 0;
    (void)std::frexp(bound, &e);
    int sa = 15 - e;
    if (sa > 24) sa = 24;
    if (sa < -24) sa = -24;
    return sa;
}

void run_conv(Ctx& ctx, const ConvLayer& L, const ConvCall& c, ConvRequest req = {}) {
    const bool bf16 = c.nprod == 1;
    if (!L.wq) throw ArgError("conv: layer has no packed weights");
    if (L.ks != 1 && L.ks != 3 && L.ks != 7) throw ArgError("conv: kernel size must be 1, 3 or 7");
    if (L.cin_pad != 8 && (L.cin_pad < 16 || (L.cin_pad & 15))) throw ArgError("conv: input channels must be 8 or a multiple of 16 (pad with zeros)");
    ConvArgs g{};
    g.x = c.x; g.x2 = c.x2; g.in_alpha = c.alpha; g.in_beta = c.alpha ? c.beta : nullptr; g.in_relu = c.relu;
    if (c.alpha && !c.beta) throw ArgError("conv: alpha without beta");
    const int sa = (bf16 || c.in_amax) ? 0 : h2_scale_log2(L.form == 1 ? 2.f * c.bound : c.bound);
    g.in_scale = std::ldexp(1.0f, sa); g.in_unscale = std::ldexp(1.0f, -sa);
    g.in_amax = bf16 ? nullptr : c.in_amax; g.in_bound_add = c.bound_add; g.amax_out = c.amax_out;
    g.w = L.wq; g.w_unscale = bf16 ? nullptr : L.w_unscale; g.bias = L.bias; g.y = c.y;
    g.stat_part = c.stat_part; g.addend = c.addend; g.add_nmod = c.add_nmod > 0 ? c.add_nmod : 1;
    g.x_bf16 = c.x_bf16; g.y_bf16 = c.y_bf16;
    if ((c.x_bf16 || c.y_bf16) && !bf16) throw ArgError("conv: bf16 storage goes with bf16 operands");
    if (c.x_bf16 && c.x2) throw ArgError("conv: bf16 storage of a concatenated input is not built");
    g.N = c.N; g.H = c.H; g.W = c.W; g.Cin = L.cin_pad; g.cin_log2 = ilog2(L.cin_pad);
    g.Csplit = c.x2 ? c.csplit : L.cin_pad; g.x2_nmod = c.x2_nmod > 0 ? c.x2_nmod : 1;
    g.Ho = (c.H + 2 * L.pad - L.ks) / L.stride + 1; g.Wo = (c.W + 2 * L.pad - L.ks) / L.stride + 1;
    g.Cout = L.cout; g.Npad = L.npad; g.stride = L.stride; g.pad = L.pad; g.reflect = L.reflect;
    g.taps = L.form == 1 ? 12 : L.ks * L.ks; g.nchunks = (g.taps * g.Cin + 15) / 16; g.M = c.N * g.Ho * g.Wo;
    if (c.N < 1 || g.Ho < 1 || g.Wo < 1) throw ArgError("conv: empty tensor");
    if (L.reflect && (L.pad >= c.H || L.pad >= c.W)) throw ArgError("conv: reflection pad needs pad < input size");
    if (c.x2 && ((g.Csplit & 15) || g.Csplit <= 0 || g.Csplit >= g.Cin)) throw ArgError("conv: channel split must be a multiple of 16 inside the channel range");
    if ((double)c.N * c.H * c.W * g.Csplit * 4 >= 2147483648.0 || (double)g.x2_nmod * c.H * c.W * (g.Cin - g.Csplit) * 4 >= 2147483648.0 ||
        (double)g.M * L.cout >= 2147483647.0 || (double)L.kpad * L.npad * 2 >= 2147483648.0)
        throw ArgError("conv: tensor too large for 32-bit buffer offsets");
    if ((size_t)2 * g.Cin * 4 > 32 * 1024) throw ArgError("conv: too many input channels for the transform table");
#ifdef TSNET_TOOLS
    req.chunk_cap = g_tools_knob[0];
#endif
    ConvShape sh;
    sh.ks = L.ks; sh.stride = L.stride; sh.pad = L.pad; sh.reflect = L.reflect; sh.cin = L.cin_pad; sh.cout = L.cout; sh.npad = L.npad; sh.kpad = L.kpad;
    sh.form = L.form; sh.N = c.N; sh.H = c.H; sh.W = c.W; sh.csplit = c.x2 ? c.csplit : 0; sh.transform = c.alpha != nullptr; sh.nprod = c.nprod;
    sh.fin_counter = c.stat_part && c.fin_counter;
    TimeScope ts(ctx, c.tclass);
    try {
        const ConvPlan p = plan_conv(sh, req, ctx.cus);
        g.tpi = p.tpi; g.tiles_m = p.tiles_m; g.tiles_n = p.tiles_n; g.fin_S = p.tpi; g.xcd_gn = p.xcd_gn;
        g.fin_alpha = c.fin_alpha; g.fin_beta = c.fin_beta; g.fin_eps = 1e-5f; g.fin_counter = p.fin ? c.fin_counter : nullptr;
        g.w1_chunk = p.w1_chunk; g.w1_tab2 = p.w1_tab2;
        const bool res = c.tclass == TSNET_T_CONV_RES;
        switch (p.family) {
        case ConvFamily::W1:
            launch_conv_w1(g, c.nprod, req.abl, ctx.stream);
            ++g_launch_counters[0];
            if (res) g_launch_counters[3] = 4064 + 30000;
            break;
        case ConvFamily::H2: {
            const int opt = req.opt | (p.sched == ConvSched::TwoGroups ? 24 : (p.sched == ConvSched::Deep ? 8 : 0));
            launch_conv_h2(g, p.side_by_side ? 5 : p.rows, p.width, c.nprod, req.abl, opt, ctx.stream);
            ++g_launch_counters[0];
            if (res) g_launch_counters[3] = (p.side_by_side ? 3 : p.rows) * 1000 + p.width + ((opt & 16) ? 20000 : 0);
            break;
        }
        case ConvFamily::H2S: launch_conv_h2s(g, c.nprod, ctx.stream); ++g_launch_counters[0]; break;
        case ConvFamily::H2S32: launch_conv_h2s32(g, c.nprod, ctx.stream); ++g_launch_counters[0]; break;
        case ConvFamily::H2D: launch_conv_h2d(g, p.rows, p.width, c.nprod, p.sched == ConvSched::Deep, ctx.stream); ++g_launch_counters[0]; break;
        case ConvFamily::G64: launch_conv_g64(g, L.ks, p.rows, c.nprod, ctx.stream); ++g_launch_counters[1]; break;
        case ConvFamily::H2R: launch_conv_h2r(g, L.ks, p.width, c.nprod, ctx.stream); ++g_launch_counters[1]; break;
        }
    } catch (const std::invalid_argument& e) { throw ArgError(e.what()); }
    check_launch("conv");
    c.stat_S = !c.stat_part ? 0 : (g.fin_counter ? -1 : g.tpi);
}

void run_stats(Ctx& ctx, const float* x, int N, int HW, int C, double* part, float* alpha, float* beta) {
    if (C & 3) throw ArgError("instnorm: C must be a multiple of 4");
    TimeScope ts(ctx, TSNET_T_STATS);
    const int cq = C / 4, cols = cq < 256 ? cq : 256, R = 256 / cols;
    int S = (HW + R * 8 - 1) / (R * 8);
    if (S > 64) S = 64;
    if (S < 1) S = 1;
    const int rps = (HW + S - 1) / S;
    S = (HW + rps - 1) / rps;
    StatsArgs sa{x, part, HW, C, S, rps};
    hipLaunchKernelGGL(in_stats_partial_kernel, dim3(S, N, (cq + 255) / 256), dim3(256), 0, ctx.stream, sa);
    check_launch("in_stats_partial");
    launch_finalize(part, alpha, beta, N, C, S, HW, ctx.stream);
}

void launch_finalize_impl(const double* part, float* alpha, float* beta, int N, int C, int S, int HW, hipStream_t s) {
    if (S > 8) {
        hipLaunchKernelGGL(in_finalize2_kernel, dim3((C + kFin2Ch - 1) / kFin2Ch, N), dim3(256), 0, s, part, alpha, beta, C, S, HW, 1e-5f);
    } else {
        const int NC = N * C;
        hipLaunchKernelGGL(in_finalize_kernel, dim3((NC + 255) / 256), dim3(256), 0, s, part, alpha, beta, NC, C, S, HW, 1e-5f);
    }
    check_launch("in_finalize");
}

void run_add_stats(Ctx& ctx, const float* x, const float* add, int add_nmod, float* y, int N, int HW, int C, double* part, float* alpha, float* beta) {
    if (C & 3) throw ArgError("add_stats: C must be a multiple of 4");
    TimeScope ts(ctx, TSNET_T_STATS);
    const int cq = C / 4, cols = cq < 256 ? cq : 256, R = 256 / cols;
    int S = (HW + R * 8 - 1) / (R * 8);
    if (S > 64) S = 64;
    if (S < 1) S = 1;
    const int rps = (HW + S - 1) / S;
    S = (HW + rps - 1) / rps;
    AddStatsArgs sa{x, add, y, part, HW, C, S, rps, add_nmod > 0 ? add_nmod : 1};
    hipLaunchKernelGGL(add_stats_partial_kernel, dim3(S, N, (cq + 255) / 256), dim3(256), 0, ctx.stream, sa);
    check_launch("add_stats_partial");
    launch_finalize(part, alpha, beta, N, C, S, HW, ctx.stream);
}

void run_norm_act(Ctx& ctx, const float* x, const float* alpha, const float* beta, int relu, const float* resid,
                  int N, int HW, int C, float* y) {
    if (C & 3) throw ArgError("norm_act: C must be a multiple of 4");
    TimeScope ts(ctx, TSNET_T_ELEMWISE);
    NormActArgs a{x, alpha, beta, resid, y, HW, C, relu, (size_t)N * HW * C / 4};
    if ((double)HW * C / 4 >= 4294967295.0 || N > 65535) throw ArgError("norm_act: tensor too large");
    size_t per_img4 = (size_t)HW * C / 4, gx = (per_img4 + 255) / 256, cap = std::max<size_t>(1, 4096 / (size_t)N);
    if (gx > cap) gx = cap;
    hipLaunchKernelGGL(norm_act_kernel, dim3((unsigned)gx, N), dim3(256), 0, ctx.stream, a);
    check_launch("norm_act");
}

void run_upsample(Ctx& ctx, const float* x, const float* alpha, const float* beta, int relu, int N, int H, int W, int C, float* y, int x_bf16 = 0, int y_bf16 = 0) {
    if (C & 3) throw ArgError("upsample: C must be a multiple of 4");
    TimeScope ts(ctx, TSNET_T_UPSAMPLE);
    UpsampleArgs a{x, alpha, beta, y, N, H, W, C, relu, x_bf16, y_bf16};
    if (2 * H > 65535 || N > 65535) throw ArgError("upsample: tensor too large");
    const size_t row4 = (size_t)2 * W * C / 4;
    hipLaunchKernelGGL(upsample2x_kernel, dim3((unsigned)std::min<size_t>((row4 + 255) / 256, 64), 2 * H, N), dim3(256), 0, ctx.stream, a);
    check_launch("upsample2x");
}

void launch_head(const HeadArgs& ha, int hh, int ww, int B, hipStream_t s, int cus, int force_rows = 0) {
    if (ha.C % (2 * kHead3Ch) != 0) {
        if (force_rows) throw ArgError("head: the narrow head (C not a multiple of 16) has no tile rows to force");
        const int tiles = ((ww + kHeadT - 1) / kHeadT) * ((hh + kHeadT - 1) / kHeadT);
        hipLaunchKernelGGL(head_conv_kernel, dim3(tiles, B), dim3(256), 0, s, ha);
    } else {
        const int tiles_x = (ww + kHead3T - 1) / kHead3T;
        auto go = [&](auto tr) {
            constexpr int TR = decltype(tr)::value;
            const size_t lds = (size_t)(2 * (head3_patch_f4(TR) + kHead3WtsF4) + ha.C / 2) * sizeof(float4);
            ensure_dynamic_lds(reinterpret_cast<const void*>(head_conv3_kernel<TR>), lds);
            hipLaunchKernelGGL(head_conv3_kernel<TR>, dim3(tiles_x * ((hh + TR - 1) / TR), B), dim3(TR * 16), lds, s, ha);
        };
        const int rows = force_rows ? force_rows : head_rows(B, tiles_x, hh, cus);
        if (rows == 32) go(std::integral_constant<int, 32>{});
        else if (rows == 16) go(std::integral_constant<int, 16>{});
        else go(std::integral_constant<int, 8>{});
    }
    check_launch("head_conv");
    ++g_launch_counters[2];
}

void run_l2norm_split(Ctx& ctx, const float* x, unsigned short* q, int N, int P, int C) {
    if (C & 7) throw ArgError("l2norm: C must be a multiple of 8");
    TimeScope ts(ctx, TSNET_T_ELEMWISE);
    const int Ppad = flow_ppad(P);
    hipLaunchKernelGGL(l2norm_split_kernel, dim3((unsigned)(((size_t)N * Ppad + 3) / 4)), dim3(256), 0, ctx.stream, x, q, N, P, Ppad, C, flow_ksteps(C));
    check_launch("l2norm_split");
}

void run_flow(Ctx& ctx, FlowArgs a, int NB, int variant = 0) {
    if (a.C & 7) throw ArgError("flow: C must be a multiple of 8");
    if (variant < 0 || variant > 2) throw ArgError("flow: variant 0, 1 or 2");
    TimeScope ts(ctx, TSNET_T_FLOW);
    const size_t budget = 160 * 1024;
    const int G = (a.part && a.cnt && NB % a.B == 0 && NB / a.B <= 8 && variant != 1) ? flowp_plan(a.B, a.h, a.w, a.C) : 0;
    if (G) {
        a.K = NB / a.B; a.G = G; a.S = flowp_slices(a.h, a.w);
        try {
            launch_flow_p(a, variant, ctx.stream);
        } catch (const std::invalid_argument& e) { throw ArgError(e.what()); }
        check_launch("flow_p");
        return;
    }
    const int NT = flow_lds_bytes(2, a.h, a.w, a.C) <= budget ? 2 : 1;
    const size_t lds = flow_lds_bytes(NT, a.h, a.w, a.C);
    if (lds > budget) throw ArgError("flow: feature width / position count exceed the LDS budget");
    try {
        launch_flow(a, NT, lds, (unsigned)(flow_ppad(a.P) / (32 * NT) * NB), ctx.stream);
    } catch (const std::invalid_argument& e) { throw ArgError(e.what()); }
    check_launch("flow");
}

void run_warp(Ctx& ctx, const float* src, const float* flow, float* out, int B, int K, int h, int w, int C) {
    TimeScope ts(ctx, TSNET_T_WARP);
    WarpArgs a{src, flow, out, B, K, h, w, C};
    hipLaunchKernelGGL(warp_mean_kernel, dim3(ew_grid((size_t)B * h * w * C / 4)), dim3(256), 0, ctx.stream, a);
    check_launch("warp_mean");
}

void pack_layer(const float* stage, const ConvLayer& L, unsigned short* planes_out, int planes, float scale, hipStream_t s) {
    hipLaunchKernelGGL(pack_weights_kernel, dim3(ew_grid((size_t)L.kpad * L.npad)), dim3(256), 0, s, stage, planes_out, scale, planes,
                       L.cout, L.cin_real, L.cin_pad, L.ks, L.form == 1 ? 4 : L.ks, L.kpad, L.npad, L.cin_total > 0 ? L.cin_total : L.cin_real, L.cin_off);
    check_launch("pack_weights");
}

std::vector<float> winograd_x_filters(const std::vector<float>& w) {
    if (w.size() % 9) throw ArgError("winograd filter transform: not a 3 x 3 kernel");
    std::vector<float> u(w.size() / 9 * 12);
    for (size_t i = 0; i < w.size() / 3; ++i) {
        const double g0 = w[3 * i], g1 = w[3 * i + 1], g2 = w[3 * i + 2];
        u[4 * i] = (float)g0;
        u[4 * i + 1] = (float)(0.5 * (g0 + g1 + g2));
        u[4 * i + 2] = (float)(0.5 * (g0 - g1 + g2));
        u[4 * i + 3] = (float)g2;
    }
    return u;
}

void linspace_pm1(int n, float* out) {
    if (n == 1) { out[0] = -1.f; return; }
    const float start = -1.f, end = 1.f;
    const float step = (end - start) / (float)(n - 1);
    const int half = n / 2;
    for (int i = 0; i < n; ++i) out[i] = i < half ? fmaf(step, (float)i, start) : fmaf(-step, (float)(n - i - 1), end);
}

void coord_table(int H, int W, float* out) {
    for (int i = 0; i < H; ++i) {
        volatile float ys = (float)i / (float)(H - 1);
        volatile float yy = 2.f * ys - 1.f;
        for (int j = 0; j < W; ++j) {
            volatile float xs = (float)j / (float)(W - 1);
            volatile float xx = 2.f * xs - 1.f;
            volatile float x2 = xx * xx;
            volatile float y2 = yy * yy;
            volatile float ss = x2 + y2;
            float* o = out + ((size_t)i * W + j) * 3;
            o[0] = xx; o[1] = yy; o[2] = sqrtf(ss);
        }
    }
}

}

struct tsnet_engine {
    tsnet_cfg cfg{};
    std::string err;
    bool finalized = false;
    int cus = 256;
    int C = 0, h = 0, w = 0, P = 0, K = 0, Bmax = 0;
    int cp_img = 0, cp_lbl = 0;
    int np = 3;
    bool st16 = false;

    struct Param { std::string name; std::vector<int64_t> shape; std::vector<float> host; bool loaded = false; };
    std::vector<Param> params;
    std::map<std::string, int> pindex;

    std::vector<ConvLayer> img_enc, lbl_enc;
    ConvLayer fuse_c1_src, fuse_c1_tar;
    ConvLayer fuse_c2, fuse_out, dec_map, dec_head;
    std::vector<ConvLayer> dec_res, dec_up;
    std::vector<ConvLayer*> all_layers;
    float* head_w = nullptr;
    const float* head_bias = nullptr;

    float* wpack = nullptr; size_t wpack_floats = 0;
    float* arena = nullptr; size_t arena_floats = 0;
    float* d_coords = nullptr; float* d_gx = nullptr; float* d_gy = nullptr;
    unsigned* amax = nullptr;
    unsigned* amax_src() const { return amax; }
    unsigned* amax_tar() const { return amax + (size_t)K * Bmax; }
    unsigned* amax_sg() const { return amax + (size_t)(K + 1) * Bmax; }
    unsigned* amax_dec() const { return amax + (size_t)(K + 2) * Bmax; }

    float *x_img = nullptr, *x_lbl = nullptr;
    std::vector<float*> raw_img, raw_lbl;
    float *X = nullptr, *Y1 = nullptr, *Y2 = nullptr;
    float *tar_fea = nullptr, *that = nullptr, *shat = nullptr, *flow = nullptr, *pg = nullptr;
    float *F1 = nullptr, *F2 = nullptr, *zbar = nullptr, *sg = nullptr;
    float* F1s = nullptr;
    float* FT = nullptr;
    float *D = nullptr, *DY1 = nullptr, *DY2 = nullptr;
    std::vector<float*> U, R;
    float* ab[4][2] = {{nullptr}};
    float* ab_side[2][2] = {{nullptr}};
    int ab_rr = 0, ab_side_rr = 0;
    double* part = nullptr;
    double* part_side = nullptr;
    int* fin_counter = nullptr;
    int* fin_counter_side = nullptr;
    int* flow_cnt = nullptr;
    float* flow_part = nullptr;
    hipStream_t side_stream = nullptr;
    hipEvent_t ev_fork = nullptr, ev_join = nullptr, ev_fork2 = nullptr, ev_join2 = nullptr;
    hipEvent_t ev_done = nullptr;
    float* train_ws = nullptr;

    int cached_B = 0;
    float* bbox_copy = nullptr;
    int last_B = 0;
    int cur_B = 0;
    float src_div[TSNET_MAX_SOURCES];

    Timing timing;

    void add_param(const std::string& name, std::vector<int64_t> shape) {
        pindex[name] = (int)params.size();
        Param p; p.name = name; p.shape = std::move(shape);
        params.push_back(std::move(p));
    }
    ConvLayer make_conv(const std::string& name, int cin_real, int cout, int ks, int stride, int pad, int reflect) {
        ConvLayer L; L.name = name; L.cin_real = cin_real; L.cin_pad = conv_cin_pad(cin_real); L.cout = cout; L.ks = ks;
        L.stride = stride; L.pad = pad; L.reflect = reflect;
        L.kpad = conv_kpad(ks, L.cin_pad); L.npad = conv_npad(cout);
        L.wparam = name + ".weight"; L.bparam = name + ".bias"; L.cin_total = cin_real; L.cin_off = 0;
        add_param(L.wparam, {cout, cin_real, ks, ks});
        add_param(L.bparam, {cout});
        return L;
    }
    void build_layers();
    void alloc_all(hipStream_t s);

    std::pair<float*, float*> next_ab(const Ctx& ctx) {
        if (!ctx.lane) { auto r = std::make_pair(ab[ab_rr][0], ab[ab_rr][1]); ab_rr = (ab_rr + 1) & 3; return r; }
        auto r = std::make_pair(ab_side[ab_side_rr][0], ab_side[ab_side_rr][1]); ab_side_rr ^= 1; return r;
    }
    float enc_bound() const { return (float)(cfg.enc_blocks + 1) * std::sqrt((float)P); }
    void conv(Ctx& ctx, const ConvLayer& L, ConvCall& c) { c.nprod = np; run_conv(ctx, L, c); }
    void conv_stats(Ctx& ctx, const ConvLayer& L, ConvCall& c, int N, int HW, float* alpha, float* beta) {
        double* pt = ctx.lane ? part_side : part;
        c.stat_part = pt;
        c.fin_alpha = alpha; c.fin_beta = beta; c.fin_counter = ctx.lane ? fin_counter_side : fin_counter;
        conv(ctx, L, c);
        if (c.stat_S < 0) return;
        TimeScope ts(ctx, TSNET_T_STATS);
        hipLaunchKernelGGL(in_finalize2_kernel, dim3((L.cout + kFin2Ch - 1) / kFin2Ch, N), dim3(256), 0, ctx.stream, pt, alpha, beta, L.cout, c.stat_S, HW, 1e-5f);
        check_launch("in_finalize2");
    }
    void encode(Ctx& ctx, std::vector<ConvLayer>& L, const float* xin, const unsigned* xin_amax, int N, std::vector<float*>& raw, float* out_fea, int nblocks);
    void resblock(Ctx& ctx, const ConvLayer& c1, const ConvLayer& c2, float* Xs, float stream_bound, const unsigned* stream_amax, float amax_add,
                  float* y1, float* y2, int N, int hh, int ww);
    void set_sources(Ctx& ctx, const float* const* src_img, const float* const* src_lbl, const float* const* src_bbox, int B, hipStream_t bbox_stream = nullptr);
    void target_chain(Ctx& ctx, const float* tar_lbl, int B);
    void forward_rest(Ctx& ctx, const float* tar_bbox, float* out_rgb, float* out_flow, int B);
    void forward_target(Ctx& ctx, const float* tar_lbl, const float* tar_bbox, float* out_rgb, float* out_flow, int B) {
        target_chain(ctx, tar_lbl, B);
        forward_rest(ctx, tar_bbox, out_rgb, out_flow, B);
    }
};

void tsnet_engine::build_layers() {
    const tsnet_cfg& c = cfg;
    const int coords = c.addcoords ? 3 : 0;
    auto enc = [&](const std::string& net, int cin, int nblocks, std::vector<ConvLayer>& out) {
        const int cin_real = cin + coords;
        out.push_back(make_conv(net + ".model.1", cin_real, c.ngf, 7, 1, 3, 1));
        int idx = 4, ch = c.ngf;
        for (int i = 0; i < c.n_downsampling; ++i) {
            out.push_back(make_conv(net + ".model." + std::to_string(idx), ch, ch * 2, 3, 2, 1, 0));
            ch *= 2; idx += 3;
        }
        for (int i = 0; i < nblocks; ++i) {
            out.push_back(make_conv(net + ".model." + std::to_string(idx) + ".conv_block.1", ch, ch, 3, 1, 1, 1));
            out.push_back(make_conv(net + ".model." + std::to_string(idx) + ".conv_block.5", ch, ch, 3, 1, 1, 1));
            idx += 1;
        }
        return out[0].cin_pad;
    };
    cp_img = enc("img_enc", 3 + c.label_nc, c.enc_blocks, img_enc);
    cp_lbl = enc("lbl_enc", c.label_nc, 0, lbl_enc);
    const int fc = 2 * C;
    fuse_c1_src = make_conv("fuse_net.model.0.conv_block.1", fc, fc, 3, 1, 1, 1);
    fuse_c1_src.name += "[src]"; fuse_c1_src.cin_real = C; fuse_c1_src.cin_pad = conv_cin_pad(C); fuse_c1_src.cin_off = 0;
    fuse_c1_src.kpad = conv_kpad(3, fuse_c1_src.cin_pad);
    fuse_c1_tar = fuse_c1_src; fuse_c1_tar.name = "fuse_net.model.0.conv_block.1[tar]"; fuse_c1_tar.cin_off = C; fuse_c1_tar.bparam.clear();
    fuse_c2 = make_conv("fuse_net.model.0.conv_block.5", fc, fc, 3, 1, 1, 1);
    fuse_out = make_conv("fuse_net.conv", fc, fc / 2, 1, 1, 0, 0);
    dec_map = make_conv("dec.map_conv", 2 * C, C, 1, 1, 0, 0);
    int n = 0;
    for (int i = 0; i < c.n_blocks; ++i) {
        dec_res.push_back(make_conv("dec.model" + std::to_string(n) + ".0.conv_block.1", C, C, 3, 1, 1, 1));
        dec_res.push_back(make_conv("dec.model" + std::to_string(n) + ".0.conv_block.5", C, C, 3, 1, 1, 1));
        ++n;
    }
    for (int i = 0; i < c.n_downsampling; ++i) {
        const int ci = c.ngf << (c.n_downsampling - i);
        dec_up.push_back(make_conv("dec.model" + std::to_string(n) + ".2", ci, ci / 2, 3, 1, 1, 1));
        ++n;
    }
    dec_head = make_conv("dec.model" + std::to_string(n) + ".1", c.ngf, 3, 7, 1, 3, 1);
    auto to_w1 = [&](ConvLayer& L, int hh, int ww) {
        if (np == 1 || !w1_eligible(L.ks, L.stride, L.pad, L.cin_pad, hh, ww)) return;
        L.form = 1; L.kpad = conv_kpad_w1(L.cin_pad);
    };
    for (size_t i = 1 + c.n_downsampling; i < img_enc.size(); ++i) to_w1(img_enc[i], h, w);
    to_w1(fuse_c1_src, h, w); to_w1(fuse_c1_tar, h, w); to_w1(fuse_c2, h, w);
    for (auto& L : dec_res) to_w1(L, h, w);
    if (!dec_up.empty()) to_w1(dec_up[0], 2 * h, 2 * w);
    if (dec_up.size() > 1) to_w1(dec_up[1], 4 * h, 4 * w);
    for (auto& L : img_enc) all_layers.push_back(&L);
    for (auto& L : lbl_enc) all_layers.push_back(&L);
    all_layers.push_back(&fuse_c1_src); all_layers.push_back(&fuse_c1_tar);
    all_layers.push_back(&fuse_c2); all_layers.push_back(&fuse_out);
    all_layers.push_back(&dec_map);
    for (auto& L : dec_res) all_layers.push_back(&L);
    for (auto& L : dec_up) all_layers.push_back(&L);
}

void tsnet_engine::alloc_all(hipStream_t s) {
    const int planes = np == 1 ? 1 : 2;
    size_t off = 0;
    for (ConvLayer* L : all_layers) { L->b_off = off; off += (size_t)round_up(L->cout, 4); }
    dec_head.b_off = off; off += 4;
    off = (off + 63) / 64 * 64;
    const size_t head_off = off;
    off += (size_t)49 * cfg.ngf * 4 + 64;
    off = (off + 63) / 64 * 64;
    const size_t tab_off = off;
    off += round_up((int)all_layers.size(), 64);
    off = (off + 63) / 64 * 64;
    const size_t planes_off = off;
    size_t o16 = 0;
    for (ConvLayer* L : all_layers) { L->w_off = o16; o16 += (size_t)planes * L->kpad * L->npad; o16 = (o16 + 127) / 128 * 128; }
    off += (o16 + 1) / 2;
    wpack_floats = off;
    HIP_TRY(hipMalloc((void**)&wpack, wpack_floats * sizeof(float)));
    HIP_TRY(hipMemsetAsync(wpack, 0, wpack_floats * sizeof(float), s));
    size_t max_w = 0;
    for (ConvLayer* L : all_layers) max_w = std::max(max_w, (size_t)L->cout * L->cin_total * L->ks * (L->form == 1 ? 4 : L->ks));
    max_w = std::max(max_w, (size_t)3 * cfg.ngf * 49);
    float* stage = nullptr;
    HIP_TRY(hipMalloc((void**)&stage, max_w * sizeof(float)));
    unsigned short* planes_base = reinterpret_cast<unsigned short*>(wpack + planes_off);
    for (size_t i = 0; i < all_layers.size(); ++i) {
        ConvLayer* L = all_layers[i];
        const Param& pw = params[pindex[L->wparam]];
        std::vector<float> wino;
        if (L->form == 1) wino = winograd_x_filters(pw.host);
        const std::vector<float>& wsrc = L->form == 1 ? wino : pw.host;
        float mx = 0.f;
        for (float v : wsrc) { const float av = std::fabs(v); if (av > mx) mx = av; }
        if (!std::isfinite(mx)) throw WeightError("parameter '" + L->wparam + "' holds a non-finite value");
        const int sw = (np != 1 && mx > 0.f) ? h2_scale_log2(mx) : 0;
        const float unscale = std::ldexp(1.0f, -sw);
        HIP_TRY(hipMemcpyAsync(stage, wsrc.data(), wsrc.size() * sizeof(float), hipMemcpyHostToDevice, s));
        HIP_TRY(hipMemcpyAsync(wpack + tab_off + i, &unscale, sizeof(float), hipMemcpyHostToDevice, s));
        pack_layer(stage, *L, planes_base + L->w_off, planes, std::ldexp(1.0f, sw), s);
        if (!L->bparam.empty()) {
            const Param& pb = params[pindex[L->bparam]];
            HIP_TRY(hipMemcpyAsync(wpack + L->b_off, pb.host.data(), pb.host.size() * sizeof(float), hipMemcpyHostToDevice, s));
        }
        HIP_TRY(hipStreamSynchronize(s));
        L->wq = planes_base + L->w_off;
        L->w_unscale = np == 1 ? nullptr : wpack + tab_off + i;
        L->bias = L->bparam.empty() ? nullptr : wpack + L->b_off;
    }
    {
        const Param& pw = params[pindex[dec_head.wparam]];
        const Param& pb = params[pindex[dec_head.bparam]];
        HIP_TRY(hipMemcpyAsync(stage, pw.host.data(), pw.host.size() * sizeof(float), hipMemcpyHostToDevice, s));
        HIP_TRY(hipMemcpyAsync(wpack + dec_head.b_off, pb.host.data(), pb.host.size() * sizeof(float), hipMemcpyHostToDevice, s));
        head_w = wpack + head_off;
        head_bias = wpack + dec_head.b_off;
        hipLaunchKernelGGL(pack_head_weights_kernel, dim3(64), dim3(256), 0, s, stage, head_w, cfg.ngf);
        check_launch("pack_head_weights");
        HIP_TRY(hipStreamSynchronize(s));
    }
    HIP_TRY(hipFree(stage));
    for (auto& p : params) { std::vector<float>().swap(p.host); }

    const int H = cfg.height, W = cfg.width;
    {
        std::vector<float> t((size_t)H * W * 3), gx(w), gy(h);
        coord_table(H, W, t.data());
        linspace_pm1(w, gx.data());
        linspace_pm1(h, gy.data());
        HIP_TRY(hipMalloc((void**)&d_coords, t.size() * sizeof(float)));
        HIP_TRY(hipMalloc((void**)&d_gx, w * sizeof(float)));
        HIP_TRY(hipMalloc((void**)&d_gy, h * sizeof(float)));
        HIP_TRY(hipMemcpy(d_coords, t.data(), t.size() * sizeof(float), hipMemcpyHostToDevice));
        HIP_TRY(hipMemcpy(d_gx, gx.data(), w * sizeof(float), hipMemcpyHostToDevice));
        HIP_TRY(hipMemcpy(d_gy, gy.data(), h * sizeof(float), hipMemcpyHostToDevice));
    }

    const size_t NB = (size_t)K * Bmax, B = Bmax;
    std::vector<std::pair<float**, size_t>> req;
    auto want = [&](float** p, size_t n) { req.emplace_back(p, (n + 63) & ~(size_t)63); };
    want(&x_img, NB * H * W * cp_img);
    want(&x_lbl, B * H * W * cp_lbl);
    raw_img.assign(cfg.n_downsampling + 1, nullptr);
    raw_lbl.assign(cfg.n_downsampling + 1, nullptr);
    for (int l = 0; l <= cfg.n_downsampling; ++l) {
        const size_t e = (size_t)(H >> l) * (W >> l) * (cfg.ngf << l);
        want(&raw_img[l], NB * e);
        want(&raw_lbl[l], B * e);
    }
    const size_t fe = (size_t)P * C;
    want(&X, NB * fe); want(&Y1, NB * fe); want(&Y2, NB * fe);
    want(&tar_fea, B * fe); want(&that, (flow_plane_halves((int)B, P, C) + 1) / 2); want(&shat, (flow_plane_halves((int)NB, P, C) + 1) / 2); want(&flow, NB * P * 2); want(&pg, B * fe);
    want(&F1, NB * fe * 2); want(&F2, NB * fe * 2); want(&F1s, NB * fe * 2); want(&zbar, B * fe * 2); want(&sg, B * fe); want(&FT, B * fe * 2);
    want(&D, B * fe); want(&DY1, B * fe); want(&DY2, B * fe);
    U.assign(cfg.n_downsampling, nullptr); R.assign(cfg.n_downsampling, nullptr);
    for (int i = 0; i < cfg.n_downsampling; ++i) {
        const size_t sp = (size_t)(h << (i + 1)) * (w << (i + 1));
        want(&U[i], B * sp * (C >> i));
        want(&R[i], B * sp * (C >> (i + 1)));
    }
    for (int i = 0; i < 4; ++i) { want(&ab[i][0], NB * 2 * C); want(&ab[i][1], NB * 2 * C); }
    for (int i = 0; i < 2; ++i) { want(&ab_side[i][0], NB * 2 * C); want(&ab_side[i][1], NB * 2 * C); }
    want(&bbox_copy, NB * H * W);
    if (P >= 2048 && P % 64 == 0) want(&flow_part, 2 * flowp_part_words((int)NB, P, flowp_slices(h, w)));
    size_t part_doubles = NB * 64 * 2 * C * 2;
    for (int l = 0; l <= cfg.n_downsampling; ++l) {
        const size_t hw = (size_t)(H >> l) * (W >> l), tpi = (hw + 63) / 64;
        part_doubles = std::max(part_doubles, stat_part_doubles(NB, tpi, (size_t)std::max(cfg.ngf << l, 2 * C)));
    }
    float *part_f = nullptr, *part_side_f = nullptr;
    want(&part_f, 2 * part_doubles); want(&part_side_f, 2 * part_doubles);
    size_t total = 0;
    for (auto& r : req) total += r.second;
    arena_floats = total;
    HIP_TRY(hipMalloc((void**)&arena, total * sizeof(float)));
    size_t o = 0;
    for (auto& r : req) { *r.first = arena + o; o += r.second; }
    part = reinterpret_cast<double*>(part_f);
    part_side = reinterpret_cast<double*>(part_side_f);
    HIP_TRY(hipMalloc((void**)&amax, (size_t)(K + 3) * Bmax * sizeof(unsigned)));
    HIP_TRY(hipMemsetAsync(amax, 0, (size_t)(K + 3) * Bmax * sizeof(unsigned), s));
    HIP_TRY(hipMalloc((void**)&fin_counter, (2 * kFinCounterInts + 256) * sizeof(int)));
    HIP_TRY(hipMemsetAsync(fin_counter, 0, (2 * kFinCounterInts + 256) * sizeof(int), s));
    fin_counter_side = fin_counter + kFinCounterInts;
    flow_cnt = fin_counter + 2 * kFinCounterInts;
    HIP_TRY(hipStreamCreateWithFlags(&side_stream, hipStreamNonBlocking));
    HIP_TRY(hipEventCreateWithFlags(&ev_fork, hipEventDisableTiming));
    HIP_TRY(hipEventCreateWithFlags(&ev_join, hipEventDisableTiming));
    HIP_TRY(hipEventCreateWithFlags(&ev_fork2, hipEventDisableTiming));
    HIP_TRY(hipEventCreateWithFlags(&ev_join2, hipEventDisableTiming));
    HIP_TRY(hipEventCreateWithFlags(&ev_done, hipEventDisableTiming));
}

void tsnet_engine::resblock(Ctx& ctx, const ConvLayer& c1, const ConvLayer& c2, float* Xs, float stream_bound, const unsigned* stream_amax,
                            float amax_add, float* y1, float* y2, int N, int hh, int ww) {
    const int Cc = c1.cout, HW = hh * ww;
    auto s1 = next_ab(ctx);
    ConvCall a; a.x = Xs; a.bound = stream_bound; a.in_amax = stream_amax; a.bound_add = amax_add;
    a.N = N; a.H = hh; a.W = ww; a.y = y1; a.tclass = TSNET_T_CONV_RES;
    conv_stats(ctx, c1, a, N, HW, s1.first, s1.second);
    ConvCall b; b.x = y1; b.alpha = s1.first; b.beta = s1.second; b.relu = 1; b.bound = std::sqrt((float)HW);
    b.N = N; b.H = hh; b.W = ww; b.y = y2; b.tclass = TSNET_T_CONV_RES;
    auto s2 = next_ab(ctx);
    conv_stats(ctx, c2, b, N, HW, s2.first, s2.second);
    run_norm_act(ctx, y2, s2.first, s2.second, 0, Xs, N, HW, Cc, Xs);
}

void tsnet_engine::encode(Ctx& ctx, std::vector<ConvLayer>& L, const float* xin, const unsigned* xin_amax, int N, std::vector<float*>& raw,
                          float* out_fea, int nblocks) {
    int hh = cfg.height, ww = cfg.width;
    auto st = next_ab(ctx);
    {
        ConvCall a; a.x = xin; a.in_amax = xin_amax; a.bound = 1.f; a.N = N; a.H = hh; a.W = ww; a.y = raw[0];
        a.y_bf16 = st16;
        conv_stats(ctx, L[0], a, N, hh * ww, st.first, st.second);
    }
    for (int l = 1; l <= cfg.n_downsampling; ++l) {
        auto prev = st;
        st = next_ab(ctx);
        ConvCall d; d.x = raw[l - 1]; d.alpha = prev.first; d.beta = prev.second; d.relu = 1; d.bound = std::sqrt((float)(hh * ww));
        d.N = N; d.H = hh; d.W = ww; d.y = raw[l];
        d.x_bf16 = st16; d.y_bf16 = st16 && l < cfg.n_downsampling;
        hh /= 2; ww /= 2;
        conv_stats(ctx, L[l], d, N, hh * ww, st.first, st.second);
    }
    run_norm_act(ctx, raw[cfg.n_downsampling], st.first, st.second, 1, nullptr, N, hh * ww, C, out_fea);
    const float bound = (float)(nblocks + 1) * std::sqrt((float)(hh * ww));
    for (int i = 0; i < nblocks; ++i)
        resblock(ctx, L[cfg.n_downsampling + 1 + 2 * i], L[cfg.n_downsampling + 2 + 2 * i], out_fea, bound, nullptr, 0.f, Y1, Y2, N, hh, ww);
}

void tsnet_engine::set_sources(Ctx& ctx, const float* const* src_img, const float* const* src_lbl, const float* const* src_bbox, int B, hipStream_t bbox_stream) {
    cur_B = B;
    const int H = cfg.height, W = cfg.width;
    {
        TimeScope ts(ctx, TSNET_T_PACK);
        PackArgs p{};
        for (int s = 0; s < K; ++s) { p.img[s] = src_img[s]; p.lbl[s] = src_lbl[s]; p.img_div[s] = src_div[s]; }
        p.coords = cfg.addcoords ? d_coords : nullptr;
        p.out = x_img; p.S = K; p.B = B; p.H = H; p.W = W; p.L = cfg.label_nc; p.nimg = 3; p.Cp = cp_img;
        HIP_TRY(hipMemsetAsync(amax_src(), 0, (size_t)K * B * sizeof(unsigned), ctx.stream));
        p.amax_out = amax_src();
        hipLaunchKernelGGL(pack_input_kernel, dim3(pack_grid(H * W), K * B), dim3(256), 0, ctx.stream, p);
// ... 5 lines not shown
    encode(ctx, img_enc, x_img, amax_src(), K * B, raw_img, X, cfg.enc_blocks);
    run_l2norm_split(ctx, X, reinterpret_cast<unsigned short*>(shat), K * B, P, C);
    ConvCall a; a.x = X; a.bound = enc_bound(); a.N = K * B; a.H = h; a.W = w; a.y = F1s;
    conv(ctx, fuse_c1_src, a);
    cached_B = B;
}

void tsnet_engine::target_chain(Ctx& ctx, const float* tar_lbl, int B) {
    cur_B = B;
    const int H = cfg.height, W = cfg.width;
    {
        TimeScope ts(ctx, TSNET_T_PACK);
        PackArgs p{};
        p.img[0] = nullptr; p.lbl[0] = tar_lbl;
        p.coords = cfg.addcoords ? d_coords : nullptr;
        p.out = x_lbl; p.S = 1; p.B = B; p.H = H; p.W = W; p.L = cfg.label_nc; p.nimg = 0; p.Cp = cp_lbl;
        HIP_TRY(hipMemsetAsync(amax_tar(), 0, (size_t)3 * Bmax * sizeof(unsigned), ctx.stream));
        p.amax_out = amax_tar();
        hipLaunchKernelGGL(pack_input_kernel, dim3(pack_grid(H * W), B), dim3(256), 0, ctx.stream, p);
        check_launch("pack_input(lbl)");
    }
    encode(ctx, lbl_enc, x_lbl, amax_tar(), B, raw_lbl, tar_fea, 0);
    run_l2norm_split(ctx, tar_fea, reinterpret_cast<unsigned short*>(that), B, P, C);
    ConvCall t; t.x = tar_fea; t.bound = std::sqrt((float)P); t.N = B; t.H = h; t.W = w; t.y = FT;
    conv(ctx, fuse_c1_tar, t);
}

void tsnet_engine::forward_rest(Ctx& ctx, const float* tar_bbox, float* out_rgb, float* out_flow, int B) {
    cur_B = B;
    const int H = cfg.height, W = cfg.width, NB = K * B;
    const bool fork = side_stream && !ctx.timing && ctx.lane == 0;
    Ctx cside(side_stream, cus, nullptr, 1);
    Ctx& cx = fork ? cside : ctx;
    SideJoin join2{fork ? side_stream : nullptr, ctx.stream, ev_join2};
    if (fork) {
        HIP_TRY(hipEventRecord(ev_fork2, ctx.stream));
        HIP_TRY(hipStreamWaitEvent(side_stream, ev_fork2, 0));
    }
    FlowArgs fa{};
    fa.tq = reinterpret_cast<const unsigned short*>(that); fa.sq = reinterpret_cast<const unsigned short*>(shat); fa.tar_bbox = tar_bbox;
    for (int s = 0; s < K; ++s) fa.src_bbox[s] = bbox_copy + (size_t)s * Bmax * H * W;
    fa.gx = d_gx; fa.gy = d_gy; fa.flow = flow;
    fa.part = reinterpret_cast<unsigned long long*>(flow_part); fa.cnt = flow_cnt;
    fa.B = B; fa.P = P; fa.C = C; fa.h = h; fa.w = w; fa.H = H; fa.W = W; fa.sy = H / h; fa.sx = W / w;
    run_flow(cx, fa, NB);
    if (out_flow)
        HIP_TRY(hipMemcpyAsync(out_flow, flow, (size_t)NB * P * 2 * sizeof(float), hipMemcpyDeviceToDevice, cx.stream));
    run_warp(cx, X, flow, pg, B, K, h, w, C);
    if (fork) HIP_TRY(hipEventRecord(ev_join2, side_stream));

    const float sqP = std::sqrt((float)P);
    {
        auto s1 = next_ab(ctx);
        auto s2 = next_ab(ctx);
        run_add_stats(ctx, F1s, FT, B, F1, NB, P, 2 * C, part, s1.first, s1.second);
        ConvCall b; b.x = F1; b.alpha = s1.first; b.beta = s1.second; b.relu = 1; b.bound = sqP;
        b.N = NB; b.H = h; b.W = w; b.y = F2;
        conv_stats(ctx, fuse_c2, b, NB, P, s2.first, s2.second);
        {
            TimeScope ts(ctx, TSNET_T_ELEMWISE);
            FuseTailArgs t2{X, tar_fea, F2, s2.first, s2.second, zbar, B, K, P, C};
            hipLaunchKernelGGL(fuse_resid_mean_kernel, dim3(ew_grid((size_t)B * P * 2 * C / 4)), dim3(256), 0, ctx.stream, t2);
            check_launch("fuse_resid_mean");
        }
        ConvCall c; c.x = zbar; c.bound = enc_bound() + sqP; c.N = B; c.H = h; c.W = w; c.y = sg;
        c.amax_out = amax_sg();
        conv(ctx, fuse_out, c);
    }

    if (fork) HIP_TRY(hipStreamWaitEvent(ctx.stream, ev_join2, 0));
    join2.done = true;
    {
        ConvCall a; a.x = pg; a.x2 = sg; a.csplit = C; a.x2_nmod = B; a.N = B; a.H = h; a.W = w; a.y = D;
        a.in_amax = amax_sg(); a.bound_add = enc_bound();
        a.amax_out = amax_dec();
        conv(ctx, dec_map, a);
    }
    for (int i = 0; i < cfg.n_blocks; ++i)
        resblock(ctx, dec_res[2 * i], dec_res[2 * i + 1], D, 0.f, amax_dec(), (float)i * sqP, DY1, DY2, B, h, w);
    const float* cur = D; const float* cal = nullptr; const float* cbe = nullptr;
    int hh = h, ww = w, cc = C;
    for (int i = 0; i < cfg.n_downsampling; ++i) {
        const float in_bound = std::sqrt((float)(hh * ww));
        run_upsample(ctx, cur, cal, cbe, cal ? 1 : 0, B, hh, ww, cc, U[i], st16 && i > 0, st16);
        hh *= 2; ww *= 2;
        cc /= 2;
        auto st = next_ab(ctx);
        ConvCall a; a.x = U[i]; a.bound = in_bound; a.N = B; a.H = hh; a.W = ww; a.y = R[i];
        a.x_bf16 = st16; a.y_bf16 = st16;
        if (!cal) { a.in_amax = amax_dec(); a.bound_add = (float)cfg.n_blocks * sqP; }
        conv_stats(ctx, dec_up[i], a, B, hh * ww, st.first, st.second);
        cur = R[i]; cal = st.first; cbe = st.second;
    }
    {
        TimeScope ts(ctx, TSNET_T_CONV);
        HeadArgs ha{};
        ha.x = cur; ha.alpha = cal; ha.beta = cbe; ha.w = head_w; ha.bias = head_bias; ha.y = out_rgb;
        ha.N = B; ha.H = hh; ha.W = ww; ha.C = cc; ha.x_bf16 = st16 && cfg.n_downsampling > 0;
        ha.composite = cfg.pose_composite; ha.fore_x0 = 64; ha.fore_x1 = 192;
        for (int c = 0; c < 3; ++c) ha.bg[c] = (-cfg.pose_mean[c]) / 255.0f;
        launch_head(ha, hh, ww, B, ctx.stream, ctx.cus);
    }
    last_B = B;
    HIP_TRY(hipEventRecord(ev_done, ctx.stream));
}

#define API_BEGIN(h)                        \
    if (!(h)) return TSNET_ERR_ARG;         \
    try {
#define API_END(h)                                                              \
    } catch (const ArgError& e) { (h)->err = e.what(); return TSNET_ERR_ARG; }   \
      catch (const WeightError& e) { (h)->err = e.what(); return TSNET_ERR_WEIGHT; } \
      catch (const std::bad_alloc&) { (h)->err = "out of host memory"; return TSNET_ERR_NOMEM; } \
      catch (const std::exception& e) { (h)->err = e.what(); return TSNET_ERR_HIP; } \
    return TSNET_OK;

extern "C" {

int tsnet_abi_version(void) { return TSNET_ABI_VERSION; }

int tsnet_create(const tsnet_cfg* cfg, tsnet_handle* out) {
    if (!cfg || !out) { g_create_error = "null argument"; return TSNET_ERR_ARG; }
    *out = nullptr;
    auto bad = [&](const char* m) { g_create_error = m; return TSNET_ERR_ARG; };
    if (cfg->n_source < 1 || cfg->n_source > TSNET_MAX_SOURCES) return bad("n_source must be in 1..8");
    if (cfg->label_nc < 1) return bad("label_nc must be >= 1");
    if (cfg->n_downsampling < 1 || cfg->n_downsampling > 5) return bad("n_downsampling must be in 1..5");
    if (cfg->ngf < 8 || (cfg->ngf & (cfg->ngf - 1))) return bad("ngf must be a power of two >= 8");
    if (cfg->n_blocks < 0 || cfg->enc_blocks < 0) return bad("block counts must be >= 0");
    const int ds = 1 << cfg->n_downsampling;
    if (cfg->height < ds * 2 || cfg->width < ds * 2 || cfg->height % ds || cfg->width % ds)
        return bad("height/width must be multiples of 2^n_downsampling (and at least twice that)");
    if (cfg->max_batch < 1) return bad("max_batch must be >= 1");
    if (cfg->pose_composite && (cfg->height != 256 || cfg->width != 256))
        return bad("pose composite is defined for 256x256 frames only (TSNet_pose.py:277-280)");
    if (cfg->operand_mode < 0 || cfg->operand_mode > 2) return bad("operand_mode must be 0 (fp32-class), 1 (bf16 operands) or 2 (bf16 operands + bf16 storage)");
    try {
        tsnet_engine* e = new tsnet_engine();
        e->cfg = *cfg;
        e->K = cfg->n_source; e->Bmax = cfg->max_batch;
        for (int s = 0; s < TSNET_MAX_SOURCES; ++s) e->src_div[s] = 255.0f;
        e->C = cfg->ngf << cfg->n_downsampling;
        e->h = cfg->height / ds; e->w = cfg->width / ds; e->P = e->h * e->w;
        e->np = cfg->operand_mode != 0 ? 1 : 3;
        e->st16 = cfg->operand_mode == 2;
        e->build_layers();
        *out = e;
    } catch (const std::exception& ex) { g_create_error = ex.what(); return TSNET_ERR_NOMEM; }
    return TSNET_OK;
}

const char* tsnet_last_error(tsnet_handle h) { return h ? h->err.c_str() : g_create_error.c_str(); }

int tsnet_num_params(tsnet_handle h) { return h ? (int)h->params.size() : TSNET_ERR_ARG; }

int tsnet_param_info(tsnet_handle h, int index, const char** name, int64_t shape_out[4], int* rank) {
    API_BEGIN(h)
    if (index < 0 || index >= (int)h->params.size()) throw ArgError("param index out of range");
    const auto& p = h->params[index];
    if (name) *name = p.name.c_str();
    if (rank) *rank = (int)p.shape.size();
    if (shape_out) for (size_t i = 0; i < 4; ++i) shape_out[i] = i < p.shape.size() ? p.shape[i] : 1;
    API_END(h)
}

int tsnet_load_weights(tsnet_handle h, const char* name, const float* data, const int64_t* shape, int rank) {
    API_BEGIN(h)
    if (h->finalized) throw ArgError("load_weights after finalize");
    if (!name || !data || !shape) throw ArgError("null argument");
    auto it = h->pindex.find(name);
    if (it == h->pindex.end()) throw WeightError(std::string("unknown parameter '") + name + "'");
    auto& p = h->params[it->second];
// ... 158 lines not shown

int tsnet_stage_ptr(tsnet_handle h, const char* name, const float** dev_ptr, size_t* count) {
    API_BEGIN(h)
    if (!h->finalized || h->last_B < 1) throw ArgError("stage_ptr before a forward");
    const size_t fe = (size_t)h->P * h->C, B = h->last_B;
    std::string n = name ? name : "";
    const float* p = nullptr; size_t c = 0;
    if (n == "src_fea") { p = h->X; c = (size_t)h->K * B * fe; }
    else if (n == "tar_fea") { p = h->tar_fea; c = B * fe; }
    else if (n == "pg") { p = h->pg; c = B * fe; }
    else if (n == "sg") { p = h->sg; c = B * fe; }
    else if (n == "dec_map") { p = h->D; c = B * fe; }
    else if (n.rfind("dec_up", 0) == 0 && n.size() == 7 && n[6] >= '0' && n[6] < '0' + h->cfg.n_downsampling) {
        const int i = n[6] - '0';
        p = h->R[i]; c = B * ((size_t)(h->h << (i + 1)) * (h->w << (i + 1)) * (h->C >> (i + 1)));
        if (h->st16) {
            HIP_TRY(hipStreamWaitEvent(h->side_stream, h->ev_done, 0));
            hipLaunchKernelGGL(bf16_widen_kernel, dim3(ew_grid(c)), dim3(256), 0, h->side_stream, reinterpret_cast<const unsigned short*>(h->R[i]), h->U[i], c);
            check_launch("bf16_widen");
            HIP_TRY(hipStreamSynchronize(h->side_stream));
            p = h->U[i];
        }
    }
    else throw ArgError("unknown stage '" + n + "'");
    if (dev_ptr) *dev_ptr = p;
    if (count) *count = c;
    API_END(h)
}

double tsnet_forward_macs(tsnet_handle h, int B) {
    if (!h) return 0.0;
    const tsnet_cfg& c = h->cfg;
    const double H = c.height, W = c.width, P = h->P, C = h->C, K = h->K;
    auto enc = [&](double cin, int nres) {
        double t = H * W * c.ngf * cin * 49;
        for (int i = 0; i < c.n_downsampling; ++i) {
            const double ho = H / (2 << i), wo = W / (2 << i), ci = c.ngf << i;
            t += ho * wo * (2 * ci) * ci * 9;
        }
        return t + nres * 2.0 * P * C * C * 9;
    };
    const double coords = c.addcoords ? 3 : 0;
    const double fuse = 2.0 * P * (2 * C) * (2 * C) * 9 + P * C * (2 * C);
    double dec = P * C * (2 * C) + c.n_blocks * 2.0 * P * C * C * 9;
    for (int i = 0; i < c.n_downsampling; ++i) {
        const double sp = P * (double)(1 << (2 * (i + 1))), ci = C / (1 << i);
        dec += sp * (ci / 2) * ci * 9;
    }
    dec += H * W * 3 * c.ngf * 49;
    const double corr = K * P * P * C + K * P * P * 2;
    return B * (K * enc(3 + c.label_nc + coords, c.enc_blocks) + enc(c.label_nc + coords, 0) + K * fuse + dec + corr);
}

int tsnet_timing_enable(tsnet_handle h, int on) {
    API_BEGIN(h)
    h->timing.on = on != 0;
    API_END(h)
}

int tsnet_timing_read(tsnet_handle h, double ms_out[TSNET_TIMING_CLASSES], int64_t launches_out[TSNET_TIMING_CLASSES], int reset) {
    API_BEGIN(h)
    h->timing.collect();
    for (int i = 0; i < TSNET_TIMING_CLASSES; ++i) {
        if (ms_out) ms_out[i] = h->timing.ms[i];
        if (launches_out) launches_out[i] = h->timing.launches[i];
        if (reset) { h->timing.ms[i] = 0; h->timing.launches[i] = 0; }
    }
    API_END(h)
}

const char* tsnet_op_last_error(void) { return g_op_error.c_str(); }

#define OP_BEGIN try {
#define OP_END                                                                   \
    } catch (const ArgError& e) { g_op_error = e.what(); return TSNET_ERR_ARG; }  \
      catch (const std::exception& e) { g_op_error = e.what(); return TSNET_ERR_HIP; } \
    return TSNET_OK;

namespace {
struct OpLayer {
    ConvLayer L;
    DevBufs mem;
    float* wd = nullptr; float* bd = nullptr; float* un = nullptr; unsigned short* wq = nullptr;
    OpLayer(const float* w_oihw, const float* bias, int Cin, int Cout, int ks, int stride, int pad, int reflect, int nprod, hipStream_t s, int form = 0) {
        L.name = "op"; L.cin_real = Cin; L.cin_pad = conv_cin_pad(Cin); L.cin_total = Cin; L.cout = Cout; L.ks = ks; L.stride = stride; L.pad = pad;
        L.reflect = reflect; L.form = form; L.kpad = form == 1 ? conv_kpad_w1(L.cin_pad) : conv_kpad(ks, L.cin_pad); L.npad = conv_npad(Cout);
        if (L.cin_pad != Cin) throw ArgError("conv2d op: Cin must be 8 or a multiple of 16 (pad channels with zeros)");
        if (form == 1 && (ks != 3 || stride != 1 || pad != 1)) throw ArgError("conv2d op: the Winograd form is for 3 x 3 / stride 1 / pad 1");
        size_t wn = (size_t)Cout * Cin * ks * ks;
        std::vector<float> hw(wn);
        HIP_TRY(hipMemcpy(hw.data(), w_oihw, wn * sizeof(float), hipMemcpyDefault));
        if (form == 1) { hw = winograd_x_filters(hw); wn = hw.size(); }
        float mx = 0.f;
        for (float v : hw) mx = std::max(mx, std::fabs(v));
        const int planes = nprod == 1 ? 1 : 2;
        const int sw = (nprod != 1 && mx > 0.f) ? h2_scale_log2(mx) : 0;
        wd = mem.alloc<float>(wn * sizeof(float));
        wq = mem.alloc<unsigned short>((size_t)L.kpad * L.npad * 2 * planes);
        un = mem.alloc<float>(sizeof(float));
        HIP_TRY(hipMemcpy(wd, hw.data(), wn * sizeof(float), hipMemcpyHostToDevice));
        const float unscale = std::ldexp(1.0f, -sw);
        HIP_TRY(hipMemcpy(un, &unscale, sizeof(float), hipMemcpyHostToDevice));
        pack_layer(wd, L, wq, planes, std::ldexp(1.0f, sw), s);
        if (bias) {
            bd = mem.alloc<float>(Cout * sizeof(float));
            HIP_TRY(hipMemcpy(bd, bias, Cout * sizeof(float), hipMemcpyDefault));
        }
        L.wq = wq; L.w_unscale = nprod == 1 ? nullptr : un; L.bias = bd;
    }
    OpLayer(const OpLayer&) = delete;
    OpLayer& operator=(const OpLayer&) = delete;
};
}

int tsnet_op_conv2d(const float* x, int N, int H, int W, int Cin, const float* w_oihw, const float* bias, int Cout,
                    int ksize, int stride, int pad, int pad_mode, const float* in_alpha, const float* in_beta, int in_relu,
                    float bound, int nprod, int kernel, int tile, float* y, void* stream) {
    OP_BEGIN
    if (!x || !w_oihw || !y) throw ArgError("null tensor");
    if (nprod != 1 && nprod != 3 && nprod != 4) throw ArgError("conv2d op: 1 (bf16 operands), 3 or 4 products");
    hipStream_t s = (hipStream_t)stream;
    Ctx ctx(s, current_device_cus());
    ConvRequest req;
    try { req = decode_tile_code(kernel, tile); } catch (const std::invalid_argument& e) { throw ArgError(e.what()); }
    OpLayer op(w_oihw, bias, Cin, Cout, ksize, stride, pad, pad_mode, nprod, s, kernel == 3 ? 1 : 0);
    ConvCall c; c.x = x; c.alpha = in_alpha; c.beta = in_beta; c.relu = in_relu; c.bound = bound; c.N = N; c.H = H; c.W = W; c.y = y; c.nprod = nprod;
    run_conv(ctx, op.L, c, req);
    HIP_TRY(hipStreamSynchronize(s));
    OP_END
}

int tsnet_op_conv2d_cat(const float* x, const float* x2, int N, int H, int W, int C1, int C2, int x2_nmod, const float* w_oihw, const float* bias, int Cout,
                        int ksize, int stride, int pad, int pad_mode, float bound, int nprod, float* y, void* stream) {
    OP_BEGIN
    if (!x || !x2 || !w_oihw || !y) throw ArgError("null tensor");
    hipStream_t s = (hipStream_t)stream;
    Ctx ctx(s, current_device_cus());
    OpLayer op(w_oihw, bias, C1 + C2, Cout, ksize, stride, pad, pad_mode, nprod, s);
    ConvCall c; c.x = x; c.x2 = x2; c.csplit = C1; c.x2_nmod = x2_nmod; c.bound = bound; c.N = N; c.H = H; c.W = W; c.y = y; c.nprod = nprod;
    run_conv(ctx, op.L, c);
    HIP_TRY(hipStreamSynchronize(s));
    OP_END
}

int tsnet_op_head(const float* x, int N, int H, int W, int C, const float* in_alpha, const float* in_beta, const float* w_oihw, const float* bias,
                  int composite, const float* bg, float* y, void* stream) {
    OP_BEGIN
    if (!x || !w_oihw || !bias || !y) throw ArgError("null tensor");
    if (C < 4 || (C & 3)) throw ArgError("head op: C must be a multiple of 4");
    if (in_alpha && !in_beta) throw ArgError("head op: alpha without beta");
    HeadRequest hr;
    try { hr = decode_head_code(composite); } catch (const std::invalid_argument& e) { throw ArgError(e.what()); }
    hipStream_t s = (hipStream_t)stream;
    const size_t wn = (size_t)3 * C * 49;
    DevBufs mem;
    float* wd = mem.alloc<float>(wn * sizeof(float));
    float* tab = mem.alloc<float>(((size_t)49 * C * 4 + 64) * sizeof(float));
    float* bd = mem.alloc<float>(4 * sizeof(float));
    HIP_TRY(hipMemsetAsync(tab, 0, ((size_t)49 * C * 4 + 64) * sizeof(float), s));
    HIP_TRY(hipMemcpy(wd, w_oihw, wn * sizeof(float), hipMemcpyDefault));
    HIP_TRY(hipMemcpy(bd, bias, 3 * sizeof(float), hipMemcpyDefault));
    hipLaunchKernelGGL(pack_head_weights_kernel, dim3(64), dim3(256), 0, s, wd, tab, C);
    check_launch("pack_head_weights");
    HeadArgs ha{};
    ha.x = x; ha.alpha = in_alpha; ha.beta = in_alpha ? in_beta : nullptr; ha.w = tab; ha.bias = bd; ha.y = y;
    ha.N = N; ha.H = H; ha.W = W; ha.C = C;
    ha.composite = hr.composite; ha.fore_x0 = 64; ha.fore_x1 = 192;
    for (int c = 0; c < 3; ++c) ha.bg[c] = bg ? bg[c] : 0.f;
    launch_head(ha, H, W, N, s, current_device_cus(), hr.rows);
    HIP_TRY(hipStreamSynchronize(s));
    OP_END
}

int tsnet_op_instnorm_stats(const float* x, int N, int HW, int C, float* alpha, float* beta, void* stream) {
    OP_BEGIN
    if (!x || !alpha || !beta) throw ArgError("null tensor");
    Ctx ctx((hipStream_t)stream, current_device_cus());
    DevBufs mem;
    double* part = mem.alloc<double>((size_t)N * 64 * C * 2 * sizeof(double));
    run_stats(ctx, x, N, HW, C, part, alpha, beta);
    HIP_TRY(hipStreamSynchronize(ctx.stream));
    OP_END
}

int tsnet_op_norm_act(const float* x, const float* alpha, const float* beta, int relu, const float* resid,
                      int N, int HW, int C, float* y, void* stream) {
    OP_BEGIN
    if (!x || !y) throw ArgError("null tensor");
    Ctx ctx((hipStream_t)stream, current_device_cus());
    run_norm_act(ctx, x, alpha, beta, relu, resid, N, HW, C, y);
    OP_END
}

int tsnet_op_upsample2x(const float* x, const float* alpha, const float* beta, int relu, int N, int H, int W, int C, float* y, void* stream) {
    OP_BEGIN
    if (!x || !y) throw ArgError("null tensor");
    Ctx ctx((hipStream_t)stream, current_device_cus());
    run_upsample(ctx, x, alpha, beta, relu, N, H, W, C, y);
    OP_END
}

static void op_flow_impl(const float* tar_fea, const float* src_fea, const float* tar_bbox, const float* src_bbox,
                         int B, int K, int h, int w, int C, int H, int W, float* flow, int variant, int repeat, float* ms_out, hipStream_t stream) {
    if (!tar_fea || !src_fea || !tar_bbox || !src_bbox || !flow) throw ArgError("null tensor");
    if (B < 1 || K < 1 || K > 8) throw ArgError("flow op: 1 <= K <= 8 sources, B >= 1");
    if (H % h || W % w) throw ArgError("flow op: bbox size must be a multiple of the feature size");
    Ctx ctx(stream, current_device_cus());
    const int P = h * w, NB = K * B;
    DevBufs bufs;
    auto* that = bufs.alloc<unsigned short>(flow_plane_halves(B, P, C) * 2);
    auto* shat = bufs.alloc<unsigned short>(flow_plane_halves(NB, P, C) * 2);
    auto* gx = bufs.alloc<float>(w * sizeof(float));
    auto* gy = bufs.alloc<float>(h * sizeof(float));
    std::vector<float> hx(w), hy(h);
    linspace_pm1(w, hx.data()); linspace_pm1(h, hy.data());
    HIP_TRY(hipMemcpy(gx, hx.data(), w * sizeof(float), hipMemcpyHostToDevice));
    HIP_TRY(hipMemcpy(gy, hy.data(), h * sizeof(float), hipMemcpyHostToDevice));
    FlowArgs fa{};
    const int G = flowp_plan(B, h, w, C);
    if (G) {
        fa.part = bufs.alloc<unsigned long long>(flowp_part_words(NB, P, flowp_slices(h, w)) * 8);
        fa.cnt = bufs.alloc<int>((size_t)B * (P / 64) * sizeof(int));
        HIP_TRY(hipMemsetAsync(fa.cnt, 0, (size_t)B * (P / 64) * sizeof(int), ctx.stream));
    }
    run_l2norm_split(ctx, tar_fea, that, B, P, C);
    run_l2norm_split(ctx, src_fea, shat, NB, P, C);
    fa.tq = that; fa.sq = shat; fa.tar_bbox = tar_bbox; fa.gx = gx; fa.gy = gy; fa.flow = flow;
    for (int k = 0; k < K; ++k) fa.src_bbox[k] = src_bbox + (size_t)k * B * H * W;
    fa.B = B; fa.P = P; fa.C = C; fa.h = h; fa.w = w; fa.H = H; fa.W = W; fa.sy = H / h; fa.sx = W / w;
    std::unique_ptr<EventPair> ev(ms_out ? new EventPair : nullptr);
    run_flow(ctx, fa, NB, variant);
    if (ev) HIP_TRY(hipEventRecord(ev->a, ctx.stream));
    for (int r = 1; r < repeat; ++r) run_flow(ctx, fa, NB, variant);
    if (ev) HIP_TRY(hipEventRecord(ev->b, ctx.stream));
    HIP_TRY(hipStreamSynchronize(ctx.stream));
    if (ms_out) *ms_out = repeat > 1 ? ev->ms() / (float)(repeat - 1) : 0.f;
}

int tsnet_op_flow(const float* tar_fea, const float* src_fea, const float* tar_bbox, const float* src_bbox,
                  int B, int h, int w, int C, int H, int W, float* flow, void* stream) {
    OP_BEGIN
    op_flow_impl(tar_fea, src_fea, tar_bbox, src_bbox, B, 1, h, w, C, H, W, flow, 0, 1, nullptr, (hipStream_t)stream);
    OP_END
}

int tsnet_op_flow_k(const float* tar_fea, const float* src_fea, const float* tar_bbox, const float* src_bbox,
                    int B, int K, int h, int w, int C, int H, int W, float* flow, int variant, int repeat, float* ms_out, void* stream) {
    OP_BEGIN
    op_flow_impl(tar_fea, src_fea, tar_bbox, src_bbox, B, K, h, w, C, H, W, flow, variant, repeat, ms_out, (hipStream_t)stream);
    OP_END
}

int tsnet_flow_plan(int B, int h, int w, int C) { return (B < 1 || h < 1 || w < 1 || C < 8 || (C & 7)) ? -1 : flowp_plan(B, h, w, C); }

int tsnet_op_warp(const float* src_fea, const float* flow, int B, int h, int w, int C, float* out, void* stream) {
    OP_BEGIN
    if (!src_fea || !flow || !out) throw ArgError("null tensor");
    if (C & 3) throw ArgError("warp op: C must be a multiple of 4");
    Ctx ctx((hipStream_t)stream, current_device_cus());
    run_warp(ctx, src_fea, flow, out, B, 1, h, w, C);
    OP_END
}

int tsnet_op_warp_k(const float* src_fea, const float* flow, int B, int K, int h, int w, int C, float* out, int repeat, float* ms_out, void* stream) {
    OP_BEGIN
    if (!src_fea || !flow || !out) throw ArgError("null tensor");
    if (C & 3) throw ArgError("warp op: C must be a multiple of 4");
    if (B < 1 || K < 1 || K > TSNET_MAX_SOURCES || h < 1 || w < 1) throw ArgError("warp op: bad shape");
    Ctx ctx((hipStream_t)stream, current_device_cus());
    if (ms_out) *ms_out = 0.f;
    run_warp(ctx, src_fea, flow, out, B, K, h, w, C);
    if (repeat > 1) {
        EventPair ev;
        HIP_TRY(hipEventRecord(ev.a, ctx.stream));
        for (int i = 1; i < repeat; ++i) run_warp(ctx, src_fea, flow, out, B, K, h, w, C);
        HIP_TRY(hipEventRecord(ev.b, ctx.stream));
        const float t = ev.ms();
        if (ms_out) *ms_out = t / (float)(repeat - 1);
    }
    OP_END
}
// ... 256 lines not shown
```

Measured before the change: 800.6 frames/s.

## Fold bilinear 2x upsample into following conv via phase-composed Winograd filters

Composes the bilinear 2x upsample with the following 3x3 conv into four phase filters run as one Winograd conv on the low-resolution map, with clamp padding. A separate ring kernel computes boundary corrections that account for the reflect padding at full resolution. The epilogue writes the results depth-to-space. This removes the upsampled intermediate tensor and its memory traffic, and cuts conv MACs, in exchange for 4x the output columns, a ring-correction kernel and more epilogue index math.

```diff
diff --git a/include/tsnet_abi.h b/include/tsnet_abi.h
--- a/include/tsnet_abi.h
+++ b/include/tsnet_abi.h
@@ -88,6 +88,9 @@
                       int N, int HW, int C, float* y, void* stream);
 int tsnet_op_upsample2x(const float* x, const float* alpha, const float* beta, int relu,
                         int N, int H, int W, int C, float* y, void* stream);
+int tsnet_op_upconv(const float* x, int N, int H, int W, int Cin, const float* w_oihw, const float* bias, int Cout,
+                    const float* in_alpha, const float* in_beta, int in_relu, float bound, int mode, int chunk,
+                    float* y, float* alpha_out, float* beta_out, int repeat, float* ms_out, void* stream);
 int tsnet_op_flow(const float* tar_fea, const float* src_fea, const float* tar_bbox, const float* src_bbox,
                   int B, int h, int w, int C, int H, int W, float* flow, void* stream);
 int tsnet_op_flow_k(const float* tar_fea, const float* src_fea, const float* tar_bbox, const float* src_bbox,
diff --git a/wacv23_tsnet_amd/_lib.py b/wacv23_tsnet_amd/_lib.py
--- a/wacv23_tsnet_amd/_lib.py
+++ b/wacv23_tsnet_amd/_lib.py
@@ -16,7 +16,7 @@
     "tsnet_last_error", "tsnet_num_params", "tsnet_param_info", "tsnet_packed_weights",
     "tsnet_forward", "tsnet_set_source_divisors", "tsnet_set_sources", "tsnet_forward_target", "tsnet_train_extras", "tsnet_stage_ptr",
     "tsnet_forward_macs", "tsnet_timing_enable", "tsnet_timing_read",
-    "tsnet_op_conv2d", "tsnet_op_conv2d_cat", "tsnet_op_head", "tsnet_op_instnorm_stats", "tsnet_op_norm_act", "tsnet_op_upsample2x",
+    "tsnet_op_conv2d", "tsnet_op_conv2d_cat", "tsnet_op_head", "tsnet_op_instnorm_stats", "tsnet_op_norm_act", "tsnet_op_upsample2x", "tsnet_op_upconv",
     "tsnet_op_flow", "tsnet_op_flow_k", "tsnet_flow_plan", "tsnet_op_warp", "tsnet_op_warp_k", "tsnet_op_last_error", "tsnet_frame_stats", "tsnet_demo_postprocess", "tsnet_fit_face_curves", "tsnet_raster_face", "tsnet_vl2ch", "tsnet_fit_pose_curves", "tsnet_raster_pose", "tsnet_label_bbox", "tsnet_resize_pad", "tsnet_resize_label", "tsnet_bench_conv", "tsnet_debug_counters", "tsnet_linspace", "tsnet_coord_table",
     "tsnet_bicubic_taps", "tsnet_bicubic_table", "tsnet_prepare_frames",
 )
@@ -64,6 +64,8 @@
     lib.tsnet_op_instnorm_stats.argtypes = [_vp, C.c_int, C.c_int, C.c_int, _vp, _vp, _vp]
     lib.tsnet_op_norm_act.argtypes = [_vp, _vp, _vp, C.c_int, _vp, C.c_int, C.c_int, C.c_int, _vp, _vp]
     lib.tsnet_op_upsample2x.argtypes = [_vp, _vp, _vp, C.c_int, C.c_int, C.c_int, C.c_int, C.c_int, _vp, _vp]
+    if hasattr(lib, "tsnet_op_upconv"):
+        lib.tsnet_op_upconv.argtypes = [_vp] + [C.c_int] * 4 + [_vp, _vp, C.c_int, _vp, _vp, C.c_int, C.c_float, C.c_int, C.c_int, _vp, _vp, _vp, C.c_int, _fp, _vp]
     lib.tsnet_resize_label.argtypes = [_vp, C.c_int, C.c_int, C.c_int, C.c_int, C.c_int, _vp, C.c_int, _vp, C.c_int, _vp, _vp]
     lib.tsnet_op_flow.argtypes = [_vp, _vp, _vp, _vp, C.c_int, C.c_int, C.c_int, C.c_int, C.c_int, C.c_int, _vp, _vp]
     lib.tsnet_op_flow_k.argtypes = [_vp, _vp, _vp, _vp] + [C.c_int] * 7 + [_vp, C.c_int, C.c_int, _fp, _vp]
diff --git a/wacv23_tsnet_amd/csrc/conv_common.hpp b/wacv23_tsnet_amd/csrc/conv_common.hpp
--- a/wacv23_tsnet_amd/csrc/conv_common.hpp
+++ b/wacv23_tsnet_amd/csrc/conv_common.hpp
@@ -148,7 +148,18 @@
     unsigned* amax_out;
     int x_bf16, y_bf16;
     int w1_chunk, w1_tab2;
+    int d2s;
+    const float* ring;
 };
+
+__host__ __device__ __forceinline__ int ring_pixels(int H2, int W2) { return 2 * W2 + 2 * (H2 - 2); }
+__device__ __forceinline__ int ring_index(int Y, int X, int H2, int W2) {
+    if (Y == 0) return X;
+    if (Y == H2 - 1) return W2 + X;
+    if (X == 0) return 2 * W2 + Y - 1;
+    if (X == W2 - 1) return 2 * W2 + (H2 - 2) + Y - 1;
+    return -1;
+}
 
 __device__ __forceinline__ void bf16x8_widen(const F4& p, F4 (&o)[2]) {
 #pragma unroll
@@ -225,13 +236,30 @@
     }
 }
 
-template <int BN, int WARPS_M, int WARPS_N, int MT, int NTL, int STAT_WAVE = 0, typename MOf>
+template <int BN, int WARPS_M, int WARPS_N, int MT, int NTL, int STAT_WAVE = 0, bool D2S = false, typename MOf>
 __device__ __forceinline__ void conv_epilogue(const ConvArgs& a, f32x16 (&tot)[MT][NTL], unsigned char* smem_raw, int tid, int wave, int n0,
                                               size_t stat_tile, MOf m_of, const bool active = true) {
     constexpr int WM = MT * 32, WN = NTL * 32;
     const int lane = tid & 63, li = lane & 31, lh = lane >> 5;
     const int wm0 = (wave / WARPS_N) * WM, wn0 = (wave % WARPS_N) * WN;
     const int hw = a.Ho * a.Wo;
+    const int cr = D2S ? a.d2s : 0;
+    struct Pos { int m, img, oy, ox; };
+    auto d2s_split = [&](int m) __attribute__((always_inline)) {
+        Pos p; p.m = m; p.img = m / hw;
+        const int rem = m - p.img * hw;
+        p.oy = rem / a.Wo; p.ox = rem - p.oy * a.Wo;
+        return p;
+    };
+    auto d2s_elem = [&](const Pos& b, int m, int ph, int c, int& ring_at) __attribute__((always_inline)) {
+        Pos p = b;
+        p.ox += m - b.m;
+        if (p.ox < 0 || p.ox >= a.Wo) p = d2s_split(m);
+        const int Y = 2 * p.oy + (ph >> 1), X = 2 * p.ox + (ph & 1), H2 = 2 * a.Ho, W2 = 2 * a.Wo;
+        const int ri = ring_index(Y, X, H2, W2);
+        ring_at = ri < 0 ? -1 : (p.img * ring_pixels(H2, W2) + ri) * cr + c;
+        return ((size_t)(p.img * H2 + Y) * W2 + X) * cr + c;
+    };
     double csum[NTL], csq[NTL];
 #pragma unroll
     for (int j = 0; j < NTL; ++j) { csum[j] = 0.0; csq[j] = 0.0; }
@@ -242,12 +270,21 @@
         for (int j = 0; j < NTL; ++j) {
             const int n = n0 + wn0 + j * 32 + li;
             const bool nok = n < a.Cout;
-            const float bv = (a.bias && nok) ? a.bias[n] : 0.f;
+            const int ph = cr ? n / cr : 0, nc = n - ph * cr;
+            const float bv = (a.bias && nok) ? a.bias[nc] : 0.f;
+            Pos base{};
+            const bool ringed = D2S && a.ring && nok && active;
+            if (ringed) { const int m0 = m_of(wm0 + i * 32 + 4 * lh); base = d2s_split(m0 < 0 ? 0 : m0); }
 #pragma unroll
             for (int r = 0; r < 16; ++r) {
                 const int m = m_of(wm0 + i * 32 + (r & 3) + 8 * (r >> 2) + 4 * lh);
                 const bool mok = active && m >= 0;
                 float v = tot[i][j][r] + bv;
+                if (ringed && mok) {
+                    int ring_at;
+                    (void)d2s_elem(base, m, ph, nc, ring_at);
+                    if (ring_at >= 0) v += a.ring[ring_at];
+                }
                 if (a.addend && nok && mok) {
                     const int img = m / hw;
                     v += a.addend[((size_t)(img % a.add_nmod) * hw + (m - img * hw)) * a.Cout + n];
@@ -360,10 +397,18 @@
         for (int j = 0; j < NTL; ++j) {
             const int n = n0 + wn0 + j * 32 + li;
             if (n >= a.Cout) continue;
+            const int ph = cr ? n / cr : 0, nc = n - ph * cr;
+            Pos base{};
+            if (D2S && cr && active) { const int m0 = m_of(wm0 + i * 32 + 4 * lh); base = d2s_split(m0 < 0 ? 0 : m0); }
 #pragma unroll
             for (int r = 0; r < 16; ++r) {
                 const int m = m_of(wm0 + i * 32 + (r & 3) + 8 * (r >> 2) + 4 * lh);
                 if (!(active && m >= 0)) continue;
+                if (D2S && cr) {
+                    int ring_at;
+                    a.y[d2s_elem(base, m, ph, nc, ring_at)] = tot[i][j][r];
+                    continue;
+                }
                 if (a.y_bf16) y16[(size_t)m * a.Cout + n] = bf16_rne(tot[i][j][r]);
                 else a.y[(size_t)m * a.Cout + n] = tot[i][j][r];
             }
diff --git a/wacv23_tsnet_amd/csrc/conv_plan.hpp b/wacv23_tsnet_amd/csrc/conv_plan.hpp
--- a/wacv23_tsnet_amd/csrc/conv_plan.hpp
+++ b/wacv23_tsnet_amd/csrc/conv_plan.hpp
@@ -25,6 +25,7 @@
     bool fin_counter = false;
     int ho() const { return (H + 2 * pad - ks) / stride + 1; }
     int wo() const { return (W + 2 * pad - ks) / stride + 1; }
+    bool folded_up() const { return reflect == 2; }
 };
 
 struct ConvRequest {
@@ -159,6 +160,8 @@
     const bool bf16 = s.nprod == 1;
     const int Ho = s.ho(), hw = Ho * s.wo();
     ConvPlan p;
+    if (s.folded_up() && (s.form != 1 || s.cout % 4))
+        throw std::invalid_argument("conv: clamp padding is the folded upsample's: the Winograd form on 4 x C phase columns");
     if (s.form == 1) {
         if (s.csplit || !w1_eligible(s.ks, s.stride, s.pad, s.cin, s.H, s.W))
             throw std::invalid_argument("conv(w1): the layer is packed in the Winograd form, which needs a single source and whole 4 x 32 tiles");
@@ -173,7 +176,7 @@
     auto set_tiles = [&](int rows_per_tile_m, int bn) {
         p.tpi = (hw + rows_per_tile_m - 1) / rows_per_tile_m;
         p.tiles_m = s.N * p.tpi; p.tiles_n = (s.cout + bn - 1) / bn;
-        p.fin = s.fin_counter && p.tpi <= kFinMaxTiles && (size_t)s.N * ((s.npad + 31) / 32) <= kFinCounterInts;
+        p.fin = !s.folded_up() && s.fin_counter && p.tpi <= kFinMaxTiles && (size_t)s.N * ((s.npad + 31) / 32) <= kFinCounterInts;
     };
     switch (p.family) {
     case ConvFamily::W1:
diff --git a/wacv23_tsnet_amd/csrc/conv_w1.hpp b/wacv23_tsnet_amd/csrc/conv_w1.hpp
--- a/wacv23_tsnet_amd/csrc/conv_w1.hpp
+++ b/wacv23_tsnet_amd/csrc/conv_w1.hpp
@@ -134,6 +134,7 @@
     constexpr bool ONE_LEVEL = NPROD == 1;
     constexpr bool ZPAD_KEEP = (OPT & 1) != 0;
     constexpr bool NO_RELU = (OPT & 2) != 0;
+    constexpr bool D2S = (OPT & 4) != 0;
     constexpr int BD = 3;
     constexpr int REG = kW1Reg;
     constexpr int PLANE_V = 2 * REG, POSB = NPL * PLANE_V, SLABB = 4 * POSB + 32, STAGE = 2 * SLABB;
@@ -253,7 +254,7 @@
             }
         }
         const int m_img = t.img * a.Ho * a.Wo;
-        conv_epilogue<64, 4, 2, 1, 1, 8>(a, out, ebase, tid_e, consumer ? wave : nt, t.n0, (size_t)t.img * tper + t.tin,
+        conv_epilogue<64, 4, 2, 1, 1, 8, D2S>(a, out, ebase, tid_e, consumer ? wave : nt, t.n0, (size_t)t.img * tper + t.tin,
                                       [&](int l) { return m_img + (t.oy0 + (l >> 5)) * a.Wo + t.ox0 + (l & 31); }, consumer);
     };
 
@@ -269,6 +270,7 @@
             const int item = NIT * pw + it;
             ldst[it] = psl * SLABB + poct * REG + ((item >> 1) * 16 + (item & 1) * 8 + (lane >> 3)) * 16 + psub * 8;
         }
+        const bool clamp = a.reflect == 2;
         auto offsets = [&](const W1Tile& t, const bool real, Offs& o) __attribute__((always_inline)) {
 #pragma unroll
             for (int it = 0; it < NIT; ++it) {
@@ -276,8 +278,8 @@
                 int iy = t.oy0 - 1 + prow;
                 bool rok = real;
                 if (a.reflect) {
-                    iy = iy < 0 ? -iy : iy;
-                    iy = iy >= a.H ? 2 * (a.H - 1) - iy : iy;
+                    iy = iy < 0 ? (clamp ? 0 : -iy) : iy;
+                    iy = iy >= a.H ? (clamp ? a.H - 1 : 2 * (a.H - 1) - iy) : iy;
                 } else {
                     rok = rok && iy >= 0 && iy < a.H;
                 }
@@ -286,8 +288,8 @@
                     int ix = t.ox0 - 1 + 2 * ppair + q;
                     bool ok = rok;
                     if (a.reflect) {
-                        ix = ix < 0 ? -ix : ix;
-                        ix = ix >= a.W ? 2 * (a.W - 1) - ix : ix;
+                        ix = ix < 0 ? (clamp ? 0 : -ix) : ix;
+                        ix = ix >= a.W ? (clamp ? a.W - 1 : 2 * (a.W - 1) - ix) : ix;
                     } else {
                         ok = ok && ix >= 0 && ix < a.W;
                     }
diff --git a/wacv23_tsnet_amd/csrc/conv_w1_launch.cpp b/wacv23_tsnet_amd/csrc/conv_w1_launch.cpp
--- a/wacv23_tsnet_amd/csrc/conv_w1_launch.cpp
+++ b/wacv23_tsnet_amd/csrc/conv_w1_launch.cpp
@@ -28,6 +28,17 @@
 void go_w1(const ConvArgs& a, hipStream_t s) {
     const size_t lds = (size_t)w1_lds_bytes(a.Cin, NPROD == 1 ? 1 : 2, a.w1_tab2 ? 2 : 1);
     if (NPROD == 1 && a.w1_chunk > 1) throw std::invalid_argument("conv(w1): chunks of several tiles need the two-plane stages");
+    if (a.d2s) {
+        if constexpr (NPROD == 3) {
+            if (a.reflect != 2 || a.Cout != 4 * a.d2s || (a.in_alpha == nullptr) != (a.in_relu == 0))
+                throw std::invalid_argument("conv(w1): a folded upsample pads by clamping and reads a raw input or IN + ReLU");
+            if (a.w1_chunk <= 1) { if (a.in_alpha) go_w1_one<3, true, 4>(a, s); else go_w1_one<3, false, 2 | 4>(a, s); }
+            else { if (a.in_alpha) go_w1_k<3, true, 4>(a, lds, s); else go_w1_k<3, false, 2 | 4>(a, lds, s); }
+            return;
+        }
+        throw std::invalid_argument("conv(w1): a folded upsample takes fp16 x 2 operands");
+    }
+    if (a.reflect == 2) throw std::invalid_argument("conv(w1): clamp padding is the folded upsample's");
     if (a.w1_chunk <= 1) {
         if (!a.in_alpha && !a.in_relu) go_w1_one<NPROD, false, 2>(a, s);
         else if (!a.in_alpha) go_w1_one<NPROD, false, 0>(a, s);
diff --git a/wacv23_tsnet_amd/csrc/conv_w1_one.hpp b/wacv23_tsnet_amd/csrc/conv_w1_one.hpp
--- a/wacv23_tsnet_amd/csrc/conv_w1_one.hpp
+++ b/wacv23_tsnet_amd/csrc/conv_w1_one.hpp
@@ -64,14 +64,15 @@
         const int psl = quad >> 2, poct = (quad >> 1) & 1, psub = quad & 1;
         unsigned vP[NIT][4];
         int ldst[NIT];
+        const bool clamp = a.reflect == 2;
 #pragma unroll
         for (int it = 0; it < NIT; ++it) {
             const int item = NIT * pw + it, prow = item >> 1, ppair = (item & 1) * 8 + (lane >> 3);
             int iy = oy0 - 1 + prow;
             bool rok = true;
             if (a.reflect) {
-                iy = iy < 0 ? -iy : iy;
-                iy = iy >= a.H ? 2 * (a.H - 1) - iy : iy;
+                iy = iy < 0 ? (clamp ? 0 : -iy) : iy;
+                iy = iy >= a.H ? (clamp ? a.H - 1 : 2 * (a.H - 1) - iy) : iy;
             } else {
                 rok = iy >= 0 && iy < a.H;
             }
@@ -80,8 +81,8 @@
                 int ix = ox0 - 1 + 2 * ppair + q;
                 bool ok = rok;
                 if (a.reflect) {
-                    ix = ix < 0 ? -ix : ix;
-                    ix = ix >= a.W ? 2 * (a.W - 1) - ix : ix;
+                    ix = ix < 0 ? (clamp ? 0 : -ix) : ix;
+                    ix = ix >= a.W ? (clamp ? a.W - 1 : 2 * (a.W - 1) - ix) : ix;
                 } else {
                     ok = ok && ix >= 0 && ix < a.W;
                 }
@@ -205,7 +206,7 @@
     w1_output_transform(ex + (size_t)(mq * 16) * 64 + wn0 + li, 64 * 64, lh, out[0][0]);
     __syncthreads();
     const int m_img = img * a.Ho * a.Wo;
-    conv_epilogue<64, 4, 2, 1, 1>(a, out, smem_raw, tid, consumer ? wave : nt, n0, (size_t)img * tper + tin,
+    conv_epilogue<64, 4, 2, 1, 1, 0, (OPT & 4) != 0>(a, out, smem_raw, tid, consumer ? wave : nt, n0, (size_t)img * tper + tin,
                                   [&](int l) { return m_img + (oy0 + (l >> 5)) * a.Wo + ox0 + (l & 31); }, consumer);
 }
 
diff --git a/wacv23_tsnet_amd/csrc/engine.cpp b/wacv23_tsnet_amd/csrc/engine.cpp
--- a/wacv23_tsnet_amd/csrc/engine.cpp
+++ b/wacv23_tsnet_amd/csrc/engine.cpp
@@ -23,6 +23,7 @@
 #include "postproc.hpp"
 #include "raster.hpp"
 #include "train_extras.hpp"
+#include "upconv_ring.hpp"
 
 using namespace tsnet;
 
@@ -157,6 +158,9 @@
     const unsigned short* wq = nullptr;
     const float* w_unscale = nullptr;
     const float* bias = nullptr;
+    int d2s = 0;
+    size_t ring_off = 0;
+    const float* ring_w = nullptr;
 };
 
 struct DevBufs {
@@ -169,6 +173,7 @@
 };
 
 inline size_t stat_part_doubles(size_t N, size_t tpi, size_t Cout) { return N * tpi * Cout * 2; }
+constexpr size_t kFoldMaxPlaneBytes = 8u << 20;
 constexpr int KPAD_ALIGN = 32;
 
 inline int conv_kpad(int ks, int cin_pad) { return round_up(ks * ks * cin_pad, KPAD_ALIGN); }
@@ -185,6 +190,7 @@
     int N = 0, H = 0, W = 0;
     float* y = nullptr;
     const float* addend = nullptr; int add_nmod = 1;
+    const float* ring = nullptr;
     double* stat_part = nullptr; mutable int stat_S = 0;
     float* fin_alpha = nullptr; float* fin_beta = nullptr; int* fin_counter = nullptr;
     unsigned* amax_out = nullptr;
@@ -217,6 +223,10 @@
     g.w = L.wq; g.w_unscale = bf16 ? nullptr : L.w_unscale; g.bias = L.bias; g.y = c.y;
     g.stat_part = c.stat_part; g.addend = c.addend; g.add_nmod = c.add_nmod > 0 ? c.add_nmod : 1;
     g.x_bf16 = c.x_bf16; g.y_bf16 = c.y_bf16;
+    g.d2s = L.d2s; g.ring = c.ring;
+    if (L.d2s && (bf16 || c.addend || c.x2 || c.amax_out)) throw ArgError("conv: a folded upsample takes fp16 x 2 operands of one tensor, no addend, no published maximum");
+    if (c.ring && !L.d2s) throw ArgError("conv: ring corrections belong to a folded upsample");
+    if ((L.d2s != 0) != (L.reflect == 2) || (L.d2s && L.cout != 4 * L.d2s)) throw ArgError("conv: clamp padding and the 4 x C phase columns go with a folded upsample");
     if ((c.x_bf16 || c.y_bf16) && !bf16) throw ArgError("conv: bf16 storage goes with bf16 operands");
     if (c.x_bf16 && c.x2) throw ArgError("conv: bf16 storage of a concatenated input is not built");
     g.N = c.N; g.H = c.H; g.W = c.W; g.Cin = L.cin_pad; g.cin_log2 = ilog2(L.cin_pad);
@@ -331,6 +341,16 @@
     check_launch("upsample2x");
 }
 
+void run_up_ring(Ctx& ctx, const ConvLayer& L, const float* x, const float* alpha, const float* beta, int relu, int N, int H, int W, float* ring) {
+    if (!L.d2s || !L.ring_w) throw ArgError("up_ring: not a folded up-convolution");
+    if (L.cin_pad % kRingK || H < 2 || W < 2 || N > 65535) throw ArgError("up_ring: input channels in multiples of 16, a map of at least 2 x 2");
+    TimeScope ts(ctx, TSNET_T_CONV);
+    UpRingArgs a{x, alpha, alpha ? beta : nullptr, L.ring_w, ring, N, H, W, L.cin_pad, L.d2s, relu};
+    const int rp = ring_pixels(2 * H, 2 * W);
+    hipLaunchKernelGGL(up_ring_kernel, dim3((rp + kRingPx - 1) / kRingPx, (L.d2s + kRingCh - 1) / kRingCh, N), dim3(256), 0, ctx.stream, a);
+    check_launch("up_ring");
+}
+
 void launch_head(const HeadArgs& ha, int hh, int ww, int B, hipStream_t s, int cus, int force_rows = 0) {
     if (ha.C % (2 * kHead3Ch) != 0) {
         if (force_rows) throw ArgError("head: the narrow head (C not a multiple of 16) has no tile rows to force");
@@ -397,7 +417,8 @@
     check_launch("pack_weights");
 }
 
-std::vector<float> winograd_x_filters(const std::vector<float>& w) {
+template <typename T>
+std::vector<float> winograd_x_filters(const std::vector<T>& w) {
     if (w.size() % 9) throw ArgError("winograd filter transform: not a 3 x 3 kernel");
     std::vector<float> u(w.size() / 9 * 12);
     for (size_t i = 0; i < w.size() / 3; ++i) {
@@ -476,6 +497,7 @@
     float* FT = nullptr;
     float *D = nullptr, *DY1 = nullptr, *DY2 = nullptr;
     std::vector<float*> U, R;
+    float* ringbuf = nullptr;
     float* ab[4][2] = {{nullptr}};
     float* ab_side[2][2] = {{nullptr}};
     int ab_rr = 0, ab_side_rr = 0;
@@ -528,7 +550,8 @@
         conv(ctx, L, c);
         if (c.stat_S < 0) return;
         TimeScope ts(ctx, TSNET_T_STATS);
-        hipLaunchKernelGGL(in_finalize2_kernel, dim3((L.cout + kFin2Ch - 1) / kFin2Ch, N), dim3(256), 0, ctx.stream, pt, alpha, beta, L.cout, c.stat_S, HW, 1e-5f);
+        const int Cf = L.d2s ? L.d2s : L.cout, Sf = L.d2s ? 4 * c.stat_S : c.stat_S;
+        hipLaunchKernelGGL(in_finalize2_kernel, dim3((Cf + kFin2Ch - 1) / kFin2Ch, N), dim3(256), 0, ctx.stream, pt, alpha, beta, Cf, Sf, HW, 1e-5f);
         check_launch("in_finalize2");
     }
     void encode(Ctx& ctx, std::vector<ConvLayer>& L, const float* xin, const unsigned* xin_amax, int N, std::vector<float*>& raw, float* out_fea, int nblocks);
@@ -590,8 +613,15 @@
     for (size_t i = 1 + c.n_downsampling; i < img_enc.size(); ++i) to_w1(img_enc[i], h, w);
     to_w1(fuse_c1_src, h, w); to_w1(fuse_c1_tar, h, w); to_w1(fuse_c2, h, w);
     for (auto& L : dec_res) to_w1(L, h, w);
-    if (!dec_up.empty()) to_w1(dec_up[0], 2 * h, 2 * w);
-    if (dec_up.size() > 1) to_w1(dec_up[1], 4 * h, 4 * w);
+    for (size_t i = 0; i < dec_up.size(); ++i) {
+        ConvLayer& L = dec_up[i];
+        if (np != 3 || L.cin_real != L.cin_pad || !w1_eligible(L.ks, L.stride, L.pad, L.cin_pad, h << i, w << i)) continue;
+        if ((size_t)2 * conv_kpad_w1(L.cin_pad) * conv_npad(4 * L.cout) * 2 > kFoldMaxPlaneBytes) continue;
+        L.d2s = L.cout; L.cout = 4 * L.d2s; L.npad = conv_npad(L.cout); L.reflect = 2;
+        L.form = 1; L.kpad = conv_kpad_w1(L.cin_pad);
+    }
+    if (!dec_up.empty() && !dec_up[0].d2s) to_w1(dec_up[0], 2 * h, 2 * w);
+    if (dec_up.size() > 1 && !dec_up[1].d2s) to_w1(dec_up[1], 4 * h, 4 * w);
     for (auto& L : img_enc) all_layers.push_back(&L);
     for (auto& L : lbl_enc) all_layers.push_back(&L);
     all_layers.push_back(&fuse_c1_src); all_layers.push_back(&fuse_c1_tar);
@@ -617,6 +647,9 @@
     size_t o16 = 0;
     for (ConvLayer* L : all_layers) { L->w_off = o16; o16 += (size_t)planes * L->kpad * L->npad; o16 = (o16 + 127) / 128 * 128; }
     off += (o16 + 1) / 2;
+    off = (off + 63) / 64 * 64;
+    for (ConvLayer* L : all_layers)
+        if (L->d2s) { L->ring_off = off; off += (size_t)9 * L->cin_pad * L->d2s; off = (off + 63) / 64 * 64; }
     wpack_floats = off;
     HIP_TRY(hipMalloc((void**)&wpack, wpack_floats * sizeof(float)));
     HIP_TRY(hipMemsetAsync(wpack, 0, wpack_floats * sizeof(float), s));
@@ -630,7 +663,8 @@
         ConvLayer* L = all_layers[i];
         const Param& pw = params[pindex[L->wparam]];
         std::vector<float> wino;
-        if (L->form == 1) wino = winograd_x_filters(pw.host);
+        if (L->d2s) wino = winograd_x_filters(compose_up_filters(pw.host, L->d2s, L->cin_real));
+        else if (L->form == 1) wino = winograd_x_filters(pw.host);
         const std::vector<float>& wsrc = L->form == 1 ? wino : pw.host;
         float mx = 0.f;
         for (float v : wsrc) { const float av = std::fabs(v); if (av > mx) mx = av; }
@@ -640,6 +674,12 @@
         HIP_TRY(hipMemcpyAsync(stage, wsrc.data(), wsrc.size() * sizeof(float), hipMemcpyHostToDevice, s));
         HIP_TRY(hipMemcpyAsync(wpack + tab_off + i, &unscale, sizeof(float), hipMemcpyHostToDevice, s));
         pack_layer(stage, *L, planes_base + L->w_off, planes, std::ldexp(1.0f, sw), s);
+        if (L->d2s) {
+            const std::vector<float> rt = ring_weight_table(pw.host, L->d2s, L->cin_real);
+            HIP_TRY(hipMemcpyAsync(wpack + L->ring_off, rt.data(), rt.size() * sizeof(float), hipMemcpyHostToDevice, s));
+            HIP_TRY(hipStreamSynchronize(s));
+            L->ring_w = wpack + L->ring_off;
+        }
         if (!L->bparam.empty()) {
             const Param& pb = params[pindex[L->bparam]];
             HIP_TRY(hipMemcpyAsync(wpack + L->b_off, pb.host.data(), pb.host.size() * sizeof(float), hipMemcpyHostToDevice, s));
@@ -695,11 +735,14 @@
     want(&F1, NB * fe * 2); want(&F2, NB * fe * 2); want(&F1s, NB * fe * 2); want(&zbar, B * fe * 2); want(&sg, B * fe); want(&FT, B * fe * 2);
     want(&D, B * fe); want(&DY1, B * fe); want(&DY2, B * fe);
     U.assign(cfg.n_downsampling, nullptr); R.assign(cfg.n_downsampling, nullptr);
+    size_t ring_floats = 0;
     for (int i = 0; i < cfg.n_downsampling; ++i) {
         const size_t sp = (size_t)(h << (i + 1)) * (w << (i + 1));
-        want(&U[i], B * sp * (C >> i));
+        if (!dec_up[i].d2s || st16) want(&U[i], B * sp * (C >> i));
         want(&R[i], B * sp * (C >> (i + 1)));
-    }
+        if (dec_up[i].d2s) ring_floats = std::max(ring_floats, B * (size_t)ring_pixels(h << (i + 1), w << (i + 1)) * dec_up[i].d2s);
+    }
+    if (ring_floats) want(&ringbuf, ring_floats);
     for (int i = 0; i < 4; ++i) { want(&ab[i][0], NB * 2 * C); want(&ab[i][1], NB * 2 * C); }
     for (int i = 0; i < 2; ++i) { want(&ab_side[i][0], NB * 2 * C); want(&ab_side[i][1], NB * 2 * C); }
     want(&bbox_copy, NB * H * W);
@@ -871,12 +914,20 @@
     int hh = h, ww = w, cc = C;
     for (int i = 0; i < cfg.n_downsampling; ++i) {
         const float in_bound = std::sqrt((float)(hh * ww));
-        run_upsample(ctx, cur, cal, cbe, cal ? 1 : 0, B, hh, ww, cc, U[i], st16 && i > 0, st16);
+        const bool folded = dec_up[i].d2s != 0;
+        ConvCall a; a.bound = in_bound; a.N = B;
+        if (folded) {
+            run_up_ring(ctx, dec_up[i], cur, cal, cbe, cal ? 1 : 0, B, hh, ww, ringbuf);
+            a.x = cur; a.alpha = cal; a.beta = cbe; a.relu = cal ? 1 : 0; a.H = hh; a.W = ww; a.ring = ringbuf;
+        } else {
+            run_upsample(ctx, cur, cal, cbe, cal ? 1 : 0, B, hh, ww, cc, U[i], st16 && i > 0, st16);
+            a.x = U[i]; a.H = 2 * hh; a.W = 2 * ww;
+            a.x_bf16 = st16; a.y_bf16 = st16;
+        }
         hh *= 2; ww *= 2;
         cc /= 2;
         auto st = next_ab(ctx);
-        ConvCall a; a.x = U[i]; a.bound = in_bound; a.N = B; a.H = hh; a.W = ww; a.y = R[i];
-        a.x_bf16 = st16; a.y_bf16 = st16;
+        a.y = R[i];
         if (!cal) { a.in_amax = amax_dec(); a.bound_add = (float)cfg.n_blocks * sqP; }
         conv_stats(ctx, dec_up[i], a, B, hh * ww, st.first, st.second);
         cur = R[i]; cal = st.first; cbe = st.second;
@@ -1201,15 +1252,22 @@
     ConvLayer L;
     DevBufs mem;
     float* wd = nullptr; float* bd = nullptr; float* un = nullptr; unsigned short* wq = nullptr;
-    OpLayer(const float* w_oihw, const float* bias, int Cin, int Cout, int ks, int stride, int pad, int reflect, int nprod, hipStream_t s, int form = 0) {
-        L.name = "op"; L.cin_real = Cin; L.cin_pad = conv_cin_pad(Cin); L.cin_total = Cin; L.cout = Cout; L.ks = ks; L.stride = stride; L.pad = pad;
-        L.reflect = reflect; L.form = form; L.kpad = form == 1 ? conv_kpad_w1(L.cin_pad) : conv_kpad(ks, L.cin_pad); L.npad = conv_npad(Cout);
+    OpLayer(const float* w_oihw, const float* bias, int Cin, int Cout, int ks, int stride, int pad, int reflect, int nprod, hipStream_t s, int form = 0, bool fold = false) {
+        L.name = "op"; L.cin_real = Cin; L.cin_pad = conv_cin_pad(Cin); L.cin_total = Cin; L.cout = fold ? 4 * Cout : Cout; L.ks = ks; L.stride = stride; L.pad = pad;
+        L.reflect = reflect; L.form = form; L.kpad = form == 1 ? conv_kpad_w1(L.cin_pad) : conv_kpad(ks, L.cin_pad); L.npad = conv_npad(L.cout);
+        if (fold) { L.d2s = Cout; if (form != 1 || nprod != 3 || reflect != 2) throw ArgError("upconv op: the folded form is the Winograd form with clamp padding, three products"); }
         if (L.cin_pad != Cin) throw ArgError("conv2d op: Cin must be 8 or a multiple of 16 (pad channels with zeros)");
         if (form == 1 && (ks != 3 || stride != 1 || pad != 1)) throw ArgError("conv2d op: the Winograd form is for 3 x 3 / stride 1 / pad 1");
         size_t wn = (size_t)Cout * Cin * ks * ks;
         std::vector<float> hw(wn);
         HIP_TRY(hipMemcpy(hw.data(), w_oihw, wn * sizeof(float), hipMemcpyDefault));
-        if (form == 1) { hw = winograd_x_filters(hw); wn = hw.size(); }
+        if (fold) {
+            const std::vector<float> rt = ring_weight_table(hw, Cout, Cin);
+            float* rw = mem.alloc<float>(rt.size() * sizeof(float));
+            HIP_TRY(hipMemcpy(rw, rt.data(), rt.size() * sizeof(float), hipMemcpyHostToDevice));
+            L.ring_w = rw;
+            hw = winograd_x_filters(compose_up_filters(hw, Cout, Cin)); wn = hw.size();
+        } else if (form == 1) { hw = winograd_x_filters(hw); wn = hw.size(); }
         float mx = 0.f;
         for (float v : hw) mx = std::max(mx, std::fabs(v));
         const int planes = nprod == 1 ? 1 : 2;
@@ -1316,6 +1374,60 @@
     if (!x || !y) throw ArgError("null tensor");
     Ctx ctx((hipStream_t)stream, current_device_cus());
     run_upsample(ctx, x, alpha, beta, relu, N, H, W, C, y);
+    OP_END
+}
+
+int tsnet_op_upconv(const float* x, int N, int H, int W, int Cin, const float* w_oihw, const float* bias, int Cout,
+                    const float* in_alpha, const float* in_beta, int in_relu, float bound, int mode, int chunk,
+                    float* y, float* alpha_out, float* beta_out, int repeat, float* ms_out, void* stream) {
+    OP_BEGIN
+    if (!x || !w_oihw || !y || !alpha_out || !beta_out) throw ArgError("null tensor");
+    if (mode < 0 || mode > 3) throw ArgError("upconv op: mode 0 (the forward's choice), 1 (upsample + direct convolution), 2 (folded), 3 (upsample + Winograd-form convolution)");
+    if (N < 1 || H < 2 || W < 2 || Cin < 16 || (Cin & 15) || Cout < 4 || (Cout & 3)) throw ArgError("upconv op: Cin in multiples of 16, Cout of 4, a map of at least 2 x 2");
+    if (in_alpha && !in_beta) throw ArgError("upconv op: alpha without beta");
+    hipStream_t s = (hipStream_t)stream;
+    Ctx ctx(s, current_device_cus());
+    const bool can_fold = w1_eligible(3, 1, 1, Cin, H, W);
+    if (mode == 2 && !can_fold) throw ArgError("upconv op: the folded form needs a low-resolution map of whole 4 x 32 tiles");
+    if (mode == 3 && !w1_eligible(3, 1, 1, Cin, 2 * H, 2 * W)) throw ArgError("upconv op: the Winograd form needs whole 4 x 32 tiles");
+    const bool fold = mode == 2 || (mode == 0 && can_fold);
+    if (chunk && !fold && mode != 3) throw ArgError("upconv op: tiles per workgroup are conv_w1's");
+    OpLayer op(w_oihw, bias, Cin, Cout, 3, 1, 1, fold ? 2 : 1, 3, s, (fold || mode == 3) ? 1 : 0, fold);
+    const int H2 = 2 * H, W2 = 2 * W;
+    DevBufs mem;
+    double* part = mem.alloc<double>(stat_part_doubles(N, ((size_t)H2 * W2 + 63) / 64, Cout) * sizeof(double));
+    int* counters = mem.alloc<int>(kFinCounterInts * sizeof(int));
+    HIP_TRY(hipMemsetAsync(counters, 0, kFinCounterInts * sizeof(int), s));
+    float* up = fold ? nullptr : mem.alloc<float>((size_t)N * H2 * W2 * Cin * sizeof(float));
+    float* ring = fold ? mem.alloc<float>((size_t)N * ring_pixels(H2, W2) * Cout * sizeof(float)) : nullptr;
+    ConvRequest req; req.chunk = chunk;
+    auto once = [&]() {
+        ConvCall c; c.bound = bound; c.N = N; c.y = y; c.nprod = 3;
+        c.stat_part = part; c.fin_alpha = alpha_out; c.fin_beta = beta_out; c.fin_counter = counters;
+        if (fold) {
+            run_up_ring(ctx, op.L, x, in_alpha, in_beta, in_relu, N, H, W, ring);
+            c.x = x; c.alpha = in_alpha; c.beta = in_beta; c.relu = in_relu; c.H = H; c.W = W; c.ring = ring;
+        } else {
+            run_upsample(ctx, x, in_alpha, in_beta, in_relu, N, H, W, Cin, up);
+            c.x = up; c.H = H2; c.W = W2;
+        }
+        run_conv(ctx, op.L, c, req);
+        if (c.stat_S > 0) {
+            const int Cf = Cout, Sf = fold ? 4 * c.stat_S : c.stat_S;
+            hipLaunchKernelGGL(in_finalize2_kernel, dim3((Cf + kFin2Ch - 1) / kFin2Ch, N), dim3(256), 0, s, part, alpha_out, beta_out, Cf, Sf, H2 * W2, 1e-5f);
+            check_launch("in_finalize2");
+        }
+    };
+    once();
+    if (repeat > 1) {
+        EventPair ev;
+        HIP_TRY(hipEventRecord(ev.a, s));
+        for (int r = 1; r < repeat; ++r) once();
+        HIP_TRY(hipEventRecord(ev.b, s));
+        const float ms = ev.ms() / (float)(repeat - 1);
+        if (ms_out) *ms_out = ms;
+    } else if (ms_out) *ms_out = 0.f;
+    HIP_TRY(hipStreamSynchronize(s));
     OP_END
 }
 
diff --git a/wacv23_tsnet_amd/csrc/upconv_ring.hpp b/wacv23_tsnet_amd/csrc/upconv_ring.hpp
--- /dev/null
+++ b/wacv23_tsnet_amd/csrc/upconv_ring.hpp
@@ -0,0 +1,132 @@
+#pragma once
+#include <hip/hip_runtime.h>
+
+#include <vector>
+
+#include "conv_common.hpp"
+
+namespace tsnet {
+
+inline std::vector<double> compose_up_filters(const std::vector<float>& w, int O, int I) {
+    static const double A[2][3][3] = {{{.75, .25, 0.}, {.25, .75, .75}, {0., 0., .25}},
+                                      {{.25, 0., 0.}, {.75, .75, .25}, {0., .25, .75}}};
+    std::vector<double> u((size_t)4 * O * I * 9);
+    for (int ph = 0; ph < 4; ++ph)
+        for (size_t oi = 0; oi < (size_t)O * I; ++oi) {
+            const float* g = w.data() + oi * 9;
+            double* d = u.data() + ((size_t)ph * O * I + oi) * 9;
+            for (int ly = 0; ly < 3; ++ly)
+                for (int lx = 0; lx < 3; ++lx) {
+                    double s = 0.0;
+                    for (int ky = 0; ky < 3; ++ky)
+                        for (int kx = 0; kx < 3; ++kx) s += A[ph >> 1][ly][ky] * A[ph & 1][lx][kx] * (double)g[ky * 3 + kx];
+                    d[ly * 3 + lx] = s;
+                }
+        }
+    return u;
+}
+
+inline std::vector<float> ring_weight_table(const std::vector<float>& w, int O, int I) {
+    std::vector<float> t((size_t)9 * I * O);
+    for (int o = 0; o < O; ++o)
+        for (int i = 0; i < I; ++i)
+            for (int k = 0; k < 9; ++k) t[((size_t)k * I + i) * O + o] = w[((size_t)o * I + i) * 9 + k];
+    return t;
+}
+
+struct UpRingArgs {
+    const float* x;
+    const float* alpha;
+    const float* beta;
+    const float* wt;
+    float* ring;
+    int N, H, W, Cin, C, relu;
+};
+
+constexpr int kRingPx = 16, kRingCh = 64, kRingK = 16;
+
+__global__ __launch_bounds__(256) void up_ring_kernel(UpRingArgs a) {
+    __shared__ __attribute__((aligned(16))) float d[9][kRingK][kRingPx];
+    __shared__ int tap_any[9];
+    const int tid = threadIdx.x, img = blockIdx.z;
+    const int H2 = 2 * a.H, W2 = 2 * a.W, RP = ring_pixels(H2, W2);
+    const int r0 = blockIdx.x * kRingPx;
+    auto pixel_of = [&](int r, int& Y, int& X) {
+        if (r < W2) { Y = 0; X = r; }
+        else if (r < 2 * W2) { Y = H2 - 1; X = r - W2; }
+        else if (r < 2 * W2 + H2 - 2) { Y = r - 2 * W2 + 1; X = 0; }
+        else { Y = r - 2 * W2 - (H2 - 2) + 1; X = W2 - 1; }
+    };
+    auto up_at = [&](int Y, int X, int ci, float al, float be) {
+        float sy = (Y + 0.5f) * 0.5f - 0.5f; if (sy < 0.f) sy = 0.f;
+        float sx = (X + 0.5f) * 0.5f - 0.5f; if (sx < 0.f) sx = 0.f;
+        const int y0 = (int)sy, x0 = (int)sx;
+        const int y1 = y0 + (y0 < a.H - 1 ? 1 : 0), x1 = x0 + (x0 < a.W - 1 ? 1 : 0);
+        const float wy1 = sy - y0, wy0 = 1.f - wy1, wx1 = sx - x0, wx0 = 1.f - wx1;
+        auto ld = [&](int y, int x) {
+            float v = a.x[(((size_t)img * a.H + y) * a.W + x) * a.Cin + ci];
+            if (a.alpha) v = __builtin_fmaf(v, al, be);
+            if (a.relu) v = v > 0.f ? v : 0.f;
+            return v;
+        };
+        return wy0 * (wx0 * ld(y0, x0) + wx1 * ld(y0, x1)) + wy1 * (wx0 * ld(y1, x0) + wx1 * ld(y1, x1));
+    };
+    if (tid < 9) tap_any[tid] = 0;
+    __syncthreads();
+    if (tid < kRingPx && r0 + tid < RP) {
+        int Y, X;
+        pixel_of(r0 + tid, Y, X);
+        for (int t = 0; t < 9; ++t) {
+            const int sy = Y + t / 3 - 1, sx = X + t % 3 - 1;
+            if (sy < 0 || sy >= H2 || sx < 0 || sx >= W2) tap_any[t] = 1;
+        }
+    }
+    __syncthreads();
+    const int c = blockIdx.y * kRingCh + (tid & 63), pq = tid >> 6;
+    const bool cok = c < a.C;
+    float acc[4] = {0.f, 0.f, 0.f, 0.f};
+    for (int ci0 = 0; ci0 < a.Cin; ci0 += kRingK) {
+        {
+            const int ci = ci0 + (tid & (kRingK - 1)), px = tid >> 4, r = r0 + px;
+            int Y = 0, X = 0;
+            if (r < RP) pixel_of(r, Y, X);
+            float al = 1.f, be = 0.f;
+            if (a.alpha) { al = a.alpha[(size_t)img * a.Cin + ci]; be = a.beta[(size_t)img * a.Cin + ci]; }
+            for (int t = 0; t < 9; ++t) {
+                if (!tap_any[t]) continue;
+                const int sy = Y + t / 3 - 1, sx = X + t % 3 - 1;
+                float v = 0.f;
+                if (r < RP && (sy < 0 || sy >= H2 || sx < 0 || sx >= W2)) {
+                    const int ry = sy < 0 ? -sy : (sy >= H2 ? 2 * (H2 - 1) - sy : sy), rx = sx < 0 ? -sx : (sx >= W2 ? 2 * (W2 - 1) - sx : sx);
+                    const int cy = sy < 0 ? 0 : (sy >= H2 ? H2 - 1 : sy), cx = sx < 0 ? 0 : (sx >= W2 ? W2 - 1 : sx);
+                    v = up_at(ry, rx, ci, al, be) - up_at(cy, cx, ci, al, be);
+                }
+                d[t][tid & (kRingK - 1)][px] = v;
+            }
+        }
+        __syncthreads();
+        if (cok) {
+            for (int t = 0; t < 9; ++t) {
+                if (!tap_any[t]) continue;
+                const float* wp = a.wt + ((size_t)t * a.Cin + ci0) * a.C + c;
+#pragma unroll
+                for (int k = 0; k < kRingK; ++k) {
+                    const float wv = wp[(size_t)k * a.C];
+                    const float4 dv = *reinterpret_cast<const float4*>(&d[t][k][pq * 4]);
+                    acc[0] = __builtin_fmaf(wv, dv.x, acc[0]); acc[1] = __builtin_fmaf(wv, dv.y, acc[1]);
+                    acc[2] = __builtin_fmaf(wv, dv.z, acc[2]); acc[3] = __builtin_fmaf(wv, dv.w, acc[3]);
+                }
+            }
+        }
+        __syncthreads();
+    }
+    if (cok) {
+#pragma unroll
+        for (int e = 0; e < 4; ++e) {
+            const int r = r0 + pq * 4 + e;
+            if (r < RP) a.ring[((size_t)img * RP + r) * a.C + c] = acc[e];
+        }
+    }
+}
+
+}
```

After: 775.0 frames/s. -3.2%, worse.
